# sungnyun/dualhyp

Measured on AMD Instinct MI355X. Metric: corrected utterances/sec (TinyLlama-1.1B, 5+5 hyps, 512->64 tok), higher is better.
Workload: dtype bf16; 1 GPU; DualHyp inference, TinyLlama-1.1B bf16 + LoRA r16 (q,k,v,proj), batch 32/GPU synthetic 5+5-hyp prompts, 512-token prompt -> 64 generated tokens, greedy; batch_per_gpu=32, parallelism=replicas x1, batches_in_flight_per_gpu=64, schedule=merged, decode_rows_per_launch=2048

## Files before the change

### dualhyp_amd/_lib.py

```python
from __future__ import annotations

import ctypes as C
from pathlib import Path

_HERE = Path(__file__).resolve().parent
import os as _os
LIB_PATH = Path(_os.environ["DUALHYP_HIP_LIB"]) if _os.environ.get("DUALHYP_HIP_LIB") else _HERE / "lib" / "libdualhyp_hip.so"

P = C.c_void_p
I = C.c_int
I64 = C.c_int64
U64 = C.c_uint64
F = C.c_float


class LayerWeights(C.Structure):
    _fields_ = [(n, P) for n in ("norm_1", "norm_2", "attn_w", "attn_lora_a", "attn_lora_b", "proj_w",
                                 "proj_lora_a", "proj_lora_b", "fc_1", "fc_2", "mlp_proj",
                                 "attn_ws", "proj_ws", "fc_1_ws", "fc_2_ws", "mlp_proj_ws")]


class ModelDesc(C.Structure):
    _fields_ = [("n_layer", C.c_int32), ("n_head", C.c_int32), ("n_groups", C.c_int32), ("head_size", C.c_int32),
                ("n_embd", C.c_int32), ("intermediate", C.c_int32), ("vocab", C.c_int32), ("block_size", C.c_int32),
                ("norm_eps", F), ("lora_scale", F), ("wte", P), ("wte_rows", C.c_int32), ("ln_f", P),
                ("rope_cos", P), ("rope_sin", P), ("lm_head", P), ("adapter_scale", P), ("adapter_bias", P),
                ("h_layers", C.POINTER(LayerWeights)), ("lm_head_ws", P)]


SIGNATURES = {
    "dh_abi_version": (I, []),
    "dh_set_tuning": (I, [I, I]),
    "dh_last_error": (C.c_char_p, []),
    "dh_device_info": (I, [C.c_char_p, I, C.POINTER(I), C.POINTER(I64)]),
    "dh_embed_bf16": (I, [P, P, P, I, I, I, P]),
    "dh_rmsnorm_bf16": (I, [P, P, P, P, P, I, I, F, P, P]),
    "dh_qkv_rope_cache_bf16": (I, [P, P, P, P, P, P, P, P, P, P, I, I, I, I, I, P]),
    "dh_linear_bf16": (I, [P, P, P, I, I, I, I, P, P, I, P, F, I, I, P, P, P, P]),
    "dh_linear_qkv_rope_cache_bf16": (I, [P, P, I, I, P, I, P, F, P, P, P, P, P, P, P, I, I, I, I, P]),
    "dh_linear_lora_bf16": (I, [P, P, P, I, I, I, P, P, F, I, I, P, P, P]),
    "dh_linear_qkv_lora_rope_cache_bf16": (I, [P, P, I, I, P, P, F, P, P, P, P, P, P, P, I, I, I, I, P, P]),
    "dh_linear_partial_bf16": (I, [P, P, P, P, I, I, I, I, I, P]),
    "dh_linear_chain_bf16": (I, [P, P, P, P, I, I, I, I, I, P]),
    "dh_linear_partial_pairs_bf16": (I, [P, P, P, P, I, I, I, I, I, P]),
    "dh_finish_norm_bf16": (I, [P, I, I, I, I, I, P, F, P, P, P, P, F, P, P]),
    "dh_attn_decode_fused_bf16": (I, [P, I, I, I, I, I, P, F, I, I, P, P, P, P, P, P, P, I, I, I, I, P]),
    "dh_attn_prefill_bf16": (I, [P, P, P, P, P, P, P, P, P, I, I, I, I, I, I, P]),
    "dh_dropout_bf16": (I, [P, P, P, I64, F, C.c_uint64, C.c_uint32, P, P]),
    "dh_swiglu_fwd_bf16": (I, [P, P, P, I64, P]),
    "dh_linear_swiglu_train_bf16": (I, [P, P, P, P, P, P, I, I, I, P]),
    "dh_linear_mul_bf16": (I, [P, P, P, I, I, I, P, P]),
    "dh_swiglu_bwd_bf16": (I, [P, P, P, P, I, I, P]),
    "dh_rmsnorm_bwd_bf16": (I, [P, P, P, P, P, I, I, F, P]),
    "dh_qkv_rope_bwd_bf16": (I, [P, P, P, P, P, P, P, I, I, I, I, P]),
    "dh_tn_accum_f32": (I, [P, I, P, I, P, I, I, I, I, F, I, P, P]),
    "dh_tn_accum_work_bytes": (I64, [I, I, I]),
    "dh_tn_accum_seg_f32": (I, [P, I, P, I, P, I, I, I, I, I, F, I, P, P]),
    "dh_rowdot_f32": (I, [P, P, P, I64, I, P]),
    "dh_transpose_pad_bf16": (I, [P, P, P, P, P, I, I, I, I, P]),
    "dh_transpose_frag_bf16": (I, [P, P, P, I, I, I, P]),
    "dh_attn_bwd_transposes": (I, [I, I, I, I]),
    "dh_attn_bwd_bf16": (I, [P, P, P, P, P, P, P, P, P, P, P, P, P, P, P, I, I, I, I, I, I, P]),
    "dh_attn_decode_work_bytes": (I64, [I, I, I, I]),
    "dh_attn_decode_bf16": (I, [P, P, P, P, P, P, P, I, I, I, I, I, P]),
    "dh_sample_bf16": (I, [P, I, P, I, P, P, I, F, I, I64, U64, I, P]),
    "dh_sample_rows_bf16": (I, [P, I, P, I, P, P, P, P, I, I, I, F, I, I64, U64, P]),
    "dh_quant_rows_fp8": (I, [P, P, P, I, I, P]),
    "dh_rmsnorm_quant_fp8": (I, [P, P, P, P, P, I, I, F, P, P]),
    "dh_linear_fp8": (I, [P, P, P, P, P, I, I, I, I, P, P, P, P, P, P]),
    "dh_linear_fp8_ex": (I, [P, P, P, P, P, I, I, I, I, P, P, P, P, P, I, P]),
    "dh_linear_fp8_f32": (I, [P, P, P, P, P, I, I, I, P]),
    "dh_engine_create": (I, [C.POINTER(ModelDesc), I, I, I, C.POINTER(P)]),
    "dh_engine_destroy": (None, [P]),
    "dh_engine_device_bytes": (I64, [P]),
    "dh_im2col3_bf16": (I, [P, P, I, I, I, I, I, P]),
    "dh_pool_head_bf16": (I, [P, P, P, P, I, I, I, I, P]),
    "dh_pool_head_bwd_bf16": (I, [P, P, P, P, P, I, I, I, I, P]),
    "dh_col2im3_bf16": (I, [P, P, P, P, I, I, I, I, P]),
    "dh_cross_entropy_fwd": (I, [P, I, P, P, P, I, I, P]),
    "dh_cross_entropy_bwd": (I, [P, I, P, P, P, P, I, I, P]),
    "dh_engine_forward": (I, [P, P, C.POINTER(C.c_int32), C.POINTER(C.c_int32), I, P, P, P]),
    "dh_engine_forward_at": (I, [P, P, C.POINTER(C.c_int32), C.POINTER(C.c_int32), I, I, P, P, P]),
    "dh_engine_forward_slots": (I, [P, P, C.POINTER(C.c_int32), C.POINTER(C.c_int32), C.POINTER(C.c_int32), I, I, P, P, P]),
    "dh_engine_set_cpu_rsqrt_emulation": (I, [P, I, I]),
    "dh_engine_decode": (I, [P, P, I, P, P, I, I, F, I, I64, U64, I, P]),
    "dh_engine_decode_rows": (I, [P, P, I, P, P, P, I, I, P, P, I, I, F, I, I64, U64, P]),
    "dh_engine_read": (I, [P, I, I, P, I64, P]),
    "dh_engine_set_timing": (I, [P, I]),
    "dh_engine_get_timing": (I, [P, I, C.POINTER(C.c_double), C.POINTER(I64)]),
}

_lib = None


class DualHypHipError(RuntimeError):
    pass


def load() -> C.CDLL:
    global _lib
    if _lib is not None:
        return _lib
    if not LIB_PATH.exists():
        raise DualHypHipError(
            f"{LIB_PATH} not found: the HIP library is not built. Run `python __graft_entry__.py` "
            "(hipcc --offload-arch=gfx950). There is no CPU fallback for the product path.")
    lib = C.CDLL(str(LIB_PATH))
    for name, (res, args) in SIGNATURES.items():
        try:
            fn = getattr(lib, name)
        except AttributeError as e:
            raise DualHypHipError(f"libdualhyp_hip.so does not export {name}") from e
        fn.restype = res
        fn.argtypes = args
    if lib.dh_abi_version() != 6:
        raise DualHypHipError("libdualhyp_hip.so ABI version mismatch")
    _lib = lib
    return lib


def check(rc: int) -> None:
    if rc != 0:
        msg = load().dh_last_error().decode(errors="replace")
        raise DualHypHipError(msg or f"libdualhyp_hip call failed with code {rc}")
```

### dualhyp_amd/csrc/decode_fused.hip

```cpp
#include "common.h"

namespace {

constexpr int DCOLS = 16;
constexpr int MAXP = 16;

template <int HS, int PMAX, int NW>
__global__ __launch_bounds__(NW * 64, NW == 16 ? 1 : (NW == 6 ? 3 : (HS == 64 ? 4 : 2))) void attn_decode_fused_kernel(
    const float* __restrict__ qkv32, int n_part, int pairs, int n_seq, int ldq, int qkv_dim,
    const bf16_t* __restrict__ lora_b, float lora_scale, int split0, int split1,
    const bf16_t* __restrict__ cos, const bf16_t* __restrict__ sin, const int32_t* __restrict__ seq_slot,
    const int32_t* __restrict__ kv_len, bf16_t* __restrict__ k_cache, bf16_t* __restrict__ vT_cache,
    bf16_t* __restrict__ y, int n_head, int n_groups, int s_max, float scale) {
    constexpr int KS = HS / 16, DT = HS / 32, HALF = HS / 2;
    extern __shared__ __attribute__((aligned(16))) char smem[];
    const int pair = blockIdx.x, seq = pair / n_groups, g = pair % n_groups;
    const int q_per_kv = n_head / n_groups;
    const int tid = threadIdx.x, lane = tid & 63, wave = tid >> 6;
    const int lr = lane & 31, lh = lane >> 5;
    const int slot = seq_slot[seq];
    const int len = kv_len[seq], pos = len - 1;
    bf16_t* sQ = reinterpret_cast<bf16_t*>(smem);
    float* sKn = reinterpret_cast<float*>(smem + 16 * HS * 2);
    float* sVn = sKn + HS;
    float* sXa = sVn + HS;
    float* sSn = sXa + 48;
    float* sPm = sSn + 16;
    float* sPl = sPm + NW * DCOLS;
    float* sPo = sPl + NW * DCOLS;
    constexpr int NT_ = NW * 64;

    constexpr int PF = NW == 6 ? 2 : 1;
    struct VF { bf16x8 v; };
    struct Tile { bf16x8 kf[KS]; VF vf[DT][2]; };
    Tile tl[PF];
    const bf16_t* kbase = k_cache + ((size_t)slot * n_groups + g) * s_max * HS;
    const bf16_t* vbase = vT_cache + ((size_t)slot * n_groups + g) * HS * s_max;
    const int n_tiles = (pos + 31) / 32;
    auto load_tile = [&](Tile& T, int t) {
#pragma unroll
        for (int ks = 0; ks < KS; ++ks)
            T.kf[ks] = __builtin_nontemporal_load(reinterpret_cast<const bf16x8*>(kbase + kfrag_blk<HS>(t, ks) + lane * 8));
#pragma unroll
        for (int dt = 0; dt < DT; ++dt)
#pragma unroll
            for (int s2 = 0; s2 < 2; ++s2)
                T.vf[dt][s2].v = __builtin_nontemporal_load(reinterpret_cast<const bf16x8*>(vbase + vfrag_blk<HS>(t, dt, s2) + lane * 8));
    };
#pragma unroll
    for (int p = 0; p < PF; ++p)
        if (wave + NW * p < n_tiles) load_tile(tl[p], wave + NW * p);

    const float* row0 = qkv32 + (size_t)seq * ldq;
    const size_t pstride = (size_t)n_seq * ldq;
    auto psum = [&](int c) {
        float v[PMAX];
#pragma unroll
        for (int p = 0; p < PMAX; ++p) v[p] = p < n_part ? row0[p * pstride + c] : 0.f;
        float s = 0.f;
        if (pairs) {
#pragma unroll
            for (int p = 0; p < PMAX; p += 2) s += v[p] + v[p + 1];
        } else {
#pragma unroll
            for (int p = 0; p < PMAX; ++p) s += v[p];
        }
        return s;
    };
    if (lora_b != nullptr && tid < 48) sXa[tid] = rbf(psum(qkv_dim + tid));
    for (int i = tid; i < 16 * HS; i += NT_) sQ[i] = 0;
    __syncthreads();

    auto finish = [&](int c) -> float {
        float o = rbf(psum(c));
        if (lora_b != nullptr) {
            const int seg = (c >= split0) + (c >= split1);
            const uint4* b4 = reinterpret_cast<const uint4*>(lora_b + (size_t)c * 16);
            float l = 0.f;
#pragma unroll
            for (int h = 0; h < 2; ++h) {
                const uint4 bv = b4[h];
                const bf16_t* bp = reinterpret_cast<const bf16_t*>(&bv);
#pragma unroll
                for (int e = 0; e < 8; ++e) l = fmaf(sXa[seg * 16 + h * 8 + e], bf2f(bp[e]), l);
            }
            o = rbf(o + rbf(rbf(l) * lora_scale));
        }
        return o;
    };
    const int gbase = g * (q_per_kv + 2) * HS;
    bf16_t* kdst = k_cache + ((size_t)slot * n_groups + g) * s_max * HS;
    bf16_t* vdst = vT_cache + ((size_t)slot * n_groups + g) * HS * s_max;
    const int n_rope = (q_per_kv + 1) * HALF;
    for (int it = tid; it < n_rope + HS; it += NT_) {
        if (it < n_rope) {
            const int j = it / HALF, i = it % HALF;
            const float x1 = finish(gbase + j * HS + i), x2 = finish(gbase + j * HS + HALF + i);
            const bf16_t* cp = cos + (size_t)pos * HS;
            const bf16_t* sp = sin + (size_t)pos * HS;
            const bf16_t o1 = f2bf(rbf(x1 * bf2f(cp[i])) + rbf(-x2 * bf2f(sp[i])));
            const bf16_t o2 = f2bf(rbf(x2 * bf2f(cp[HALF + i])) + rbf(x1 * bf2f(sp[HALF + i])));
            if (j < q_per_kv) {
                sQ[j * HS + i] = o1;
                sQ[j * HS + HALF + i] = o2;
            } else {
                sKn[i] = bf2f(o1);
                sKn[HALF + i] = bf2f(o2);
                kdst[kfrag_off<HS>(pos, i)] = o1;
                kdst[kfrag_off<HS>(pos, HALF + i)] = o2;
            }
        } else {
            const int e = it - n_rope;
            const bf16_t v = f2bf(finish(gbase + (q_per_kv + 1) * HS + e));
            sVn[e] = bf2f(v);
            vdst[vfrag_off<HS>(pos, e)] = v;
        }
    }
    __syncthreads();

    for (int h = wave; h < q_per_kv; h += NW) {
        float p = 0.f;
        for (int e = lane; e < HS; e += 64) p += bf2f(sQ[h * HS + e]) * sKn[e];
        p = wave_sum(p);
        if (lane == 0) sSn[h] = p * scale;
    }

    bf16x8 qf[KS];
#pragma unroll
    for (int ks = 0; ks < KS; ++ks) qf[ks] = *reinterpret_cast<const bf16x8*>(sQ + (lr & 15) * HS + ks * 16 + lh * 8);
    if (lr >= 16) {
#pragma unroll
        for (int ks = 0; ks < KS; ++ks) qf[ks] = bf16x8{0, 0, 0, 0, 0, 0, 0, 0};
    }
    f32x16 o[DT];
#pragma unroll
    for (int dt = 0; dt < DT; ++dt)
#pragma unroll
        for (int r = 0; r < 16; ++r) o[dt][r] = 0.f;
    float m_run = -INFINITY, l_run = 0.f;
    auto compute_tile = [&](const Tile& T, int t) {
        const int key0 = t * 32;
        f32x16 st;
#pragma unroll
        for (int r = 0; r < 16; ++r) st[r] = 0.f;
#pragma unroll
        for (int ks = 0; ks < KS; ++ks) st = __builtin_amdgcn_mfma_f32_32x32x16_bf16(T.kf[ks], qf[ks], st, 0, 0, 0);
        float m_t = -INFINITY;
#pragma unroll
        for (int r = 0; r < 16; ++r) {
            const int key_abs = key0 + (r & 3) + 8 * (r >> 2) + 4 * lh;
            float sc = st[r] * scale;
            sc = key_abs < pos ? sc : -INFINITY;
            st[r] = sc;
            m_t = fmaxf(m_t, sc);
        }
        m_t = fmaxf(m_t, __shfl_xor(m_t, 32, 64));
        const float m_new = fmaxf(m_run, m_t);
        const float alpha = __expf(m_run - m_new);
        m_run = m_new;
        float psm = 0.f;
#pragma unroll
        for (int r = 0; r < 16; ++r) {
            const float p = __expf(st[r] - m_new);
            st[r] = p;
            psm += p;
        }
        l_run = l_run * alpha + psm;
#pragma unroll
        for (int s2 = 0; s2 < 2; ++s2) {
            union { bf16x8 v; uint32_t u[4]; } pf;
#pragma unroll
            for (int j = 0; j < 4; ++j) pf.u[j] = pack2bf(st[8 * s2 + 2 * j], st[8 * s2 + 2 * j + 1]);
#pragma unroll
            for (int dt = 0; dt < DT; ++dt) {
                if (s2 == 0) {
#pragma unroll
                    for (int r = 0; r < 16; ++r) o[dt][r] *= alpha;
                }
                o[dt] = __builtin_amdgcn_mfma_f32_32x32x16_bf16(T.vf[dt][s2].v, pf.v, o[dt], 0, 0, 0);
            }
        }
    };
    for (int base = wave; base < n_tiles; base += NW * PF) {
#pragma unroll
        for (int p = 0; p < PF; ++p) {
            if (base + NW * p < n_tiles) compute_tile(tl[p], base + NW * p);
            if (base + NW * (PF + p) < n_tiles) load_tile(tl[p], base + NW * (PF + p));
        }
    }
    const float l_tot = l_run + __shfl_xor(l_run, 32, 64);
    if (lr < q_per_kv) {
        if (lh == 0) {
            sPm[wave * DCOLS + lr] = m_run;
            sPl[wave * DCOLS + lr] = l_tot;
        }
#pragma unroll
        for (int dt = 0; dt < DT; ++dt)
#pragma unroll
            for (int r = 0; r < 16; ++r) {
                const int d = dt * 32 + (r & 3) + 8 * (r >> 2) + 4 * lh;
                sPo[(wave * HS + d) * DCOLS + lr] = o[dt][r];
            }
    }
    __syncthreads();
    for (int it = tid; it < q_per_kv * HS; it += NT_) {
        const int h = it / HS, d = it % HS;
        const float sn = sSn[h];
        float M = sn;
#pragma unroll
        for (int w = 0; w < NW; ++w) M = fmaxf(M, sPm[w * DCOLS + h]);
        const float pn = __expf(sn - M);
        float L = pn, O = rbf(pn) * sVn[d];
#pragma unroll
        for (int w = 0; w < NW; ++w) {
            const float mw = sPm[w * DCOLS + h];
            const float f = (mw == -INFINITY) ? 0.f : __expf(mw - M);
            L += sPl[w * DCOLS + h] * f;
            O += sPo[(w * HS + d) * DCOLS + h] * f;
        }
        y[(size_t)seq * n_head * HS + (g * q_per_kv + h) * HS + d] = f2bf(O / L);
    }
}

#ifndef DH_ATTN_WAVES64
#define DH_ATTN_WAVES64 8
#endif
template <int HS>
constexpr int attn_fused_waves() { return HS == 64 ? DH_ATTN_WAVES64 : 8; }
template <int HS>
constexpr size_t attn_fused_lds() {
    constexpr int NW = attn_fused_waves<HS>();
    return 16 * HS * 2 + (HS + HS + 48 + 16 + NW * DCOLS + NW * DCOLS + NW * HS * DCOLS) * sizeof(float);
}

template <int MAXC>
__global__ __launch_bounds__(256) void finish_norm_kernel(const float* __restrict__ h32, int n_part, int pairs, int rows, int ldh,
                                                          const bf16_t* __restrict__ lora_b, float lora_scale,
                                                          const bf16_t* __restrict__ x_resid,
                                                          const bf16_t* __restrict__ w_norm, bf16_t* __restrict__ x_out,
                                                          bf16_t* __restrict__ xn_out, int d, float eps,
                                                          const uint8_t* __restrict__ row_tail) {
    __shared__ float sXa[16];
    __shared__ float sRed[4];
    const int row = blockIdx.x, tid = threadIdx.x, lane = tid & 63, wave = tid >> 6;
    const float* hrow = h32 + (size_t)row * ldh;
    const size_t pstride = (size_t)rows * ldh;
    if (lora_b != nullptr && tid < 16) {
        float pv[MAXP];
#pragma unroll
        for (int p = 0; p < MAXP; ++p) pv[p] = p < n_part ? hrow[p * pstride + d + tid] : 0.f;
        float s = 0.f;
        if (pairs) {
#pragma unroll
            for (int p = 0; p < MAXP; p += 2) s += pv[p] + pv[p + 1];
        } else {
#pragma unroll
            for (int p = 0; p < MAXP; ++p) s += pv[p];
        }
        sXa[tid] = rbf(s);
    }
    __syncthreads();
    float v[MAXC][8];
    float ss = 0.f;
#pragma unroll
    for (int i = 0; i < MAXC; ++i) {
        const int c0 = (tid + i * 256) * 8;
        if (c0 < d) {
            float acc[8];
#pragma unroll
            for (int e = 0; e < 8; ++e) acc[e] = 0.f;
            for (int p0 = 0; p0 < n_part; p0 += 4) {
                float4 a0[4], a1[4];
#pragma unroll
                for (int q = 0; q < 4; ++q) {
                    const int p = p0 + q < n_part ? p0 + q : p0;
                    a0[q] = *reinterpret_cast<const float4*>(hrow + p * pstride + c0);
                    a1[q] = *reinterpret_cast<const float4*>(hrow + p * pstride + c0 + 4);
                }
                if (pairs) {
#pragma unroll
                    for (int q = 0; q < 4; q += 2) {
                        if (p0 + q < n_part) {
                            const bool two = p0 + q + 1 < n_part;
                            const float4 b0 = two ? a0[q + 1] : float4{0.f, 0.f, 0.f, 0.f}, b1 = two ? a1[q + 1] : float4{0.f, 0.f, 0.f, 0.f};
                            acc[0] += a0[q].x + b0.x; acc[1] += a0[q].y + b0.y; acc[2] += a0[q].z + b0.z; acc[3] += a0[q].w + b0.w;
                            acc[4] += a1[q].x + b1.x; acc[5] += a1[q].y + b1.y; acc[6] += a1[q].z + b1.z; acc[7] += a1[q].w + b1.w;
                        }
                    }
                } else {
#pragma unroll
                for (int q = 0; q < 4; ++q) {
                    if (p0 + q < n_part) {
                        acc[0] += a0[q].x; acc[1] += a0[q].y; acc[2] += a0[q].z; acc[3] += a0[q].w;
                        acc[4] += a1[q].x; acc[5] += a1[q].y; acc[6] += a1[q].z; acc[7] += a1[q].w;
                    }
                }
                }
            }
            const uint4 xr = *reinterpret_cast<const uint4*>(x_resid + (size_t)row * d + c0);
            const bf16_t* xp = reinterpret_cast<const bf16_t*>(&xr);
            uint4 xo;
            bf16_t* xop = reinterpret_cast<bf16_t*>(&xo);
#pragma unroll
            for (int e = 0; e < 8; ++e) {
                float o = rbf(acc[e]);
                if (lora_b != nullptr) {
                    const uint4* b4 = reinterpret_cast<const uint4*>(lora_b + (size_t)(c0 + e) * 16);
                    float l = 0.f;
#pragma unroll
                    for (int h = 0; h < 2; ++h) {
                        const uint4 bv = b4[h];
                        const bf16_t* bp = reinterpret_cast<const bf16_t*>(&bv);
#pragma unroll
                        for (int k = 0; k < 8; ++k) l = fmaf(sXa[h * 8 + k], bf2f(bp[k]), l);
                    }
                    o = rbf(o + rbf(rbf(l) * lora_scale));
                }
                xop[e] = f2bf(bf2f(xp[e]) + o);
                v[i][e] = bf2f(xop[e]);
                ss += rbf(v[i][e] * v[i][e]);
            }
            *reinterpret_cast<uint4*>(x_out + (size_t)row * d + c0) = xo;
        }
    }
    ss = wave_sum(ss);
    if (lane == 0) sRed[wave] = ss;
    __syncthreads();
    ss = sRed[0] + sRed[1] + sRed[2] + sRed[3];
    const float ms = rbf(ss / (float)d);
    const float t = rbf(ms + eps);
    const bool tail = row_tail != nullptr && row_tail[row] != 0;
    const float r = tail ? rbf(1.0f / rbf(sqrtf(t))) : rbf(1.0f / sqrtf(t));
#pragma unroll
    for (int i = 0; i < MAXC; ++i) {
        const int c0 = (tid + i * 256) * 8;
        if (c0 < d) {
            const uint4 wu = *reinterpret_cast<const uint4*>(w_norm + c0);
            const bf16_t* wp = reinterpret_cast<const bf16_t*>(&wu);
            uint4 o;
            bf16_t* op = reinterpret_cast<bf16_t*>(&o);
#pragma unroll
            for (int e = 0; e < 8; ++e) op[e] = f2bf(bf2f(wp[e]) * rbf(v[i][e] * r));
            *reinterpret_cast<uint4*>(xn_out + (size_t)row * d + c0) = o;
        }
    }
}

}

extern "C" int dh_attn_decode_fused_bf16(const float* qkv32, int n_part, int pairs, int n_seq, int qkv_dim, int n_ext,
                                         const dh_bf16* lora_b, float lora_scale, int split0, int split1,
                                         const dh_bf16* cos, const dh_bf16* sin, const int32_t* seq_slot,
                                         const int32_t* kv_len, dh_bf16* k_cache, dh_bf16* vT_cache, dh_bf16* y,
                                         int n_head, int n_groups, int hs, int s_max, void* stream) {
    DH_CHECK(qkv32 && cos && sin && seq_slot && kv_len && k_cache && vT_cache && y, "dh_attn_decode_fused_bf16: null argument");
    DH_CHECK(n_groups > 0 && n_head % n_groups == 0 && n_head / n_groups <= DCOLS, "dh_attn_decode_fused_bf16: bad head counts");
    DH_CHECK(hs == 64 || hs == 96 || hs == 128, "dh_attn_decode_fused_bf16: head_size %d unsupported", hs);
    DH_CHECK(s_max % 64 == 0 && n_part >= 1 && n_part <= MAXP, "dh_attn_decode_fused_bf16: bad s_max / n_part");
    DH_CHECK(qkv_dim == (n_head + 2 * n_groups) * hs, "dh_attn_decode_fused_bf16: qkv_dim mismatch");
    DH_CHECK(lora_b == nullptr || n_ext >= 48, "dh_attn_decode_fused_bf16: LoRA needs the 48 x·A^T columns");
    if (n_seq <= 0) return 0;
    const float scale = 1.0f / sqrtf((float)hs);
    hipStream_t s = (hipStream_t)stream;
    dim3 grid(n_seq * n_groups);
#define ATT_LAUNCH(HSV, PM)                                                                                           \
    hipLaunchKernelGGL((attn_decode_fused_kernel<HSV, PM, attn_fused_waves<HSV>()>), grid, dim3(64 * attn_fused_waves<HSV>()), attn_fused_lds<HSV>(), s, qkv32, n_part, pairs, n_seq,  \
                       qkv_dim + n_ext, qkv_dim, lora_b, lora_scale, split0, split1, cos, sin, seq_slot, kv_len, k_cache,  \
                       vT_cache, y, n_head, n_groups, s_max, scale)
    if (hs == 64) {
        DH_MAX_LDS_ONCE((attn_decode_fused_kernel<64, 2, attn_fused_waves<64>()>), attn_fused_lds<64>());
        DH_MAX_LDS_ONCE((attn_decode_fused_kernel<64, 8, attn_fused_waves<64>()>), attn_fused_lds<64>());
        DH_MAX_LDS_ONCE((attn_decode_fused_kernel<64, 16, attn_fused_waves<64>()>), attn_fused_lds<64>());
        if (n_part <= 2) ATT_LAUNCH(64, 2);
        else if (n_part <= 8) ATT_LAUNCH(64, 8);
        else ATT_LAUNCH(64, 16);
    } else if (hs == 96) {
        DH_MAX_LDS_ONCE((attn_decode_fused_kernel<96, 2, 8>), attn_fused_lds<96>());
        DH_MAX_LDS_ONCE((attn_decode_fused_kernel<96, 8, 8>), attn_fused_lds<96>());
        DH_MAX_LDS_ONCE((attn_decode_fused_kernel<96, 16, 8>), attn_fused_lds<96>());
        if (n_part <= 2) ATT_LAUNCH(96, 2);
        else if (n_part <= 8) ATT_LAUNCH(96, 8);
        else ATT_LAUNCH(96, 16);
    } else {
        DH_MAX_LDS_ONCE((attn_decode_fused_kernel<128, 2, 8>), attn_fused_lds<128>());
        DH_MAX_LDS_ONCE((attn_decode_fused_kernel<128, 8, 8>), attn_fused_lds<128>());
        DH_MAX_LDS_ONCE((attn_decode_fused_kernel<128, 16, 8>), attn_fused_lds<128>());
        if (n_part <= 2) ATT_LAUNCH(128, 2);
        else if (n_part <= 8) ATT_LAUNCH(128, 8);
        else ATT_LAUNCH(128, 16);
    }
#undef ATT_LAUNCH
    DH_LAUNCH_CHECK();
    return 0;
}

extern "C" int dh_finish_norm_bf16(const float* h32, int n_part, int pairs, int rows, int d, int n_ext, const dh_bf16* lora_b,
                                   float lora_scale, const dh_bf16* x_resid, const dh_bf16* w_norm, dh_bf16* x_out,
                                   dh_bf16* xn_out, float eps, const uint8_t* row_tail, void* stream) {
    DH_CHECK(h32 && x_resid && w_norm && x_out && xn_out, "dh_finish_norm_bf16: null argument");
    DH_CHECK(d % 8 == 0 && d <= 8192 && n_part >= 1 && n_part <= MAXP, "dh_finish_norm_bf16: unsupported d=%d", d);
    DH_CHECK(lora_b == nullptr || n_ext >= 16, "dh_finish_norm_bf16: LoRA needs the 16 x·A^T columns");
    DH_CHECK((d + n_ext) % 4 == 0, "dh_finish_norm_bf16: row stride must be a multiple of 4 floats");
    if (rows <= 0) return 0;
    hipStream_t s = (hipStream_t)stream;
    dim3 grid(rows), block(256);
    const int ldh = d + n_ext;
#define LAUNCH(MAXC) hipLaunchKernelGGL((finish_norm_kernel<MAXC>), grid, block, 0, s, h32, n_part, pairs, rows, ldh, lora_b, \
                                        lora_scale, x_resid, w_norm, x_out, xn_out, d, eps, row_tail)
    if (d <= 2048) { LAUNCH(1); }
    else if (d <= 4096) { LAUNCH(2); }
    else { LAUNCH(4); }
#undef LAUNCH
    DH_LAUNCH_CHECK();
    return 0;
}
```

### dualhyp_amd/csrc/engine.hip

```cpp
#include <vector>

#include "common.h"
#include "gemm.h"

int dh_sample_impl(const dh_bf16* logits, int vocab, int64_t* tokens, int tok_ld, int32_t* length, int32_t* done,
                   int n_seq, float temperature, int top_k, int64_t eos_id, uint64_t seed, int step,
                   const int32_t* step_dev, void* stream);
int dh_sample_rows_impl(const dh_bf16* logits, int vocab, int64_t* tokens, int tok_ld, int32_t* length, int32_t* done,
                        const int32_t* limit, const int32_t* row_seq, int n_rows, int n_seq, int max_new, float temperature,
                        int top_k, int64_t eos_id, uint64_t seed, void* stream);

namespace {

struct Timing {
    bool on = false;
    std::vector<std::pair<hipEvent_t, hipEvent_t>> ev[4];
    std::vector<hipEvent_t> pool;
};

}

constexpr int MAX_DECODE_ROWS = 2048;
int g_decode_tiled_rows = 0;
int g_short_kps = 8;
int g_fuse_qkv_rope = 1;
int g_prune_last_layer = 1;

struct dh_engine {
    dh_model_desc d;
    std::vector<dh_layer_weights> layers;
    int max_batch = 0, s_max = 0, max_tokens = 0;
    int qkv_dim = 0, kv_dim = 0;
    bf16_t *kc = nullptr, *vtc = nullptr;
    bf16_t *x = nullptr, *xn = nullptr, *qkv = nullptr, *qrot = nullptr, *att = nullptr, *xa = nullptr,
           *act = nullptr, *xlast = nullptr, *logits = nullptr;
    int32_t *tok_slot = nullptr, *tok_pos = nullptr, *seq_meta = nullptr;
    int32_t *last_row = nullptr, *step_dev = nullptr;
    int32_t* slot_list = nullptr;
    int32_t* last_meta = nullptr;
    bf16_t *att_last = nullptr, *xn_last = nullptr, *act_last = nullptr;
    uint8_t *row_tail = nullptr, *last_tail = nullptr, *ones = nullptr;
    int rsqrt_vec = 0, rsqrt_whole = 0;
    int64_t* dec_ids = nullptr;
    void* dec_work = nullptr;
    float* part32 = nullptr;
    bool fp8 = false;
    uint8_t* xq = nullptr;
    float* xscale = nullptr;
    int32_t* h_stage = nullptr;
    size_t cache_layer_elems = 0;
    int64_t dev_bytes = 0;
    hipStream_t gstream = nullptr;
    hipEvent_t ev_in = nullptr, ev_out = nullptr, ev_stage = nullptr;
    struct GKey {
        int64_t* tokens; int tok_ld; int32_t *length, *done; int n_seq, top_k; float temp; int64_t eos; uint64_t seed; int rsqrt_vec, tiled_rows;
        const int32_t *limit, *row_seq, *row_slot; int n_all, max_new;
        bool operator==(const GKey& k) const {
            return tokens == k.tokens && tok_ld == k.tok_ld && length == k.length && done == k.done && n_seq == k.n_seq &&
                   top_k == k.top_k && temp == k.temp && eos == k.eos && seed == k.seed && rsqrt_vec == k.rsqrt_vec &&
                   tiled_rows == k.tiled_rows && limit == k.limit && row_seq == k.row_seq && row_slot == k.row_slot &&
                   n_all == k.n_all && max_new == k.max_new;
        }
    };
    struct GEntry { GKey key; hipGraphExec_t exec; uint64_t used; };
    std::vector<GEntry> graphs;
    uint64_t graph_clock = 0;
    int last_ntok = 0;
    int slot_base = 0;
    const int32_t* seq_slot = nullptr;
    bool capturing = false;
    bool phase_decode = false;
    bool decode_tiled = false;
    Timing tm;
};

namespace {

template <typename T>
int dmalloc(dh_engine* e, T** p, size_t n) {
    DH_HIP(hipMalloc((void**)p, n * sizeof(T)));
    e->dev_bytes += (int64_t)(n * sizeof(T));
    return 0;
}

__global__ void decode_prep_kernel(const int64_t* __restrict__ tokens, int tok_ld, const int32_t* __restrict__ length,
                                   int64_t* __restrict__ ids, int32_t* __restrict__ tok_slot,
                                   int32_t* __restrict__ tok_pos, int32_t* __restrict__ kv_len, int32_t* step_dev,
                                   int n_seq, int s_max) {
    const int i = blockIdx.x * blockDim.x + threadIdx.x;
    if (i < n_seq) {
        int n = length[i];
        n = n < 1 ? 1 : (n > s_max ? s_max : n);
        ids[i] = tokens[(size_t)i * tok_ld + n - 1];
        tok_slot[i] = i;
        tok_pos[i] = n - 1;
        kv_len[i] = n;
    }
    if (i == 0) *step_dev += 1;
}

__global__ void decode_prep_rows_kernel(const int64_t* __restrict__ tokens, int tok_ld, const int32_t* __restrict__ length,
                                        const int32_t* __restrict__ row_seq, const int32_t* __restrict__ row_slot,
                                        int64_t* __restrict__ ids, int32_t* __restrict__ tok_slot, int32_t* __restrict__ tok_pos,
                                        int32_t* __restrict__ kv_len, int n_rows, int n_all, int max_batch, int s_max) {
    const int r = blockIdx.x * blockDim.x + threadIdx.x;
    if (r < n_rows) {
        int u = row_seq[r], slot = row_slot[r];
        u = u < 0 || u >= n_all ? 0 : u;
        slot = slot < 0 || slot >= max_batch ? 0 : slot;
        int n = length[u];
        const int cap = s_max < tok_ld ? s_max : tok_ld;
        n = n < 1 ? 1 : (n > cap ? cap : n);
        ids[r] = tokens[(size_t)u * tok_ld + n - 1];
        tok_slot[r] = slot;
        tok_pos[r] = n - 1;
        kv_len[r] = n;
    }
}

__global__ void set_i32_kernel(int32_t* p, int32_t v) { *p = v; }
__global__ void iota_i32_kernel(int32_t* p, int n) {
    const int i = blockIdx.x * blockDim.x + threadIdx.x;
    if (i < n) p[i] = i;
}

__global__ void gather_rows_kernel(const bf16_t* __restrict__ src, const int32_t* __restrict__ rows,
                                   bf16_t* __restrict__ dst, int n, int d) {
    const int wave = (blockIdx.x * blockDim.x + threadIdx.x) >> 6, lane = threadIdx.x & 63;
    if (wave >= n) return;
    const uint4* s = reinterpret_cast<const uint4*>(src + (size_t)rows[wave] * d);
    uint4* t = reinterpret_cast<uint4*>(dst + (size_t)wave * d);
    for (int c = lane; c < d / 8; c += 64) t[c] = s[c];
}

struct TimeScope {
    dh_engine* e; int which; hipStream_t s; hipEvent_t a = nullptr, b = nullptr;
    TimeScope(dh_engine* e_, int w, hipStream_t s_) : e(e_), which(w), s(s_) {
        if (!e->tm.on || e->capturing) return;
        hipEventCreate(&a); hipEventCreate(&b);
        hipEventRecord(a, s);
    }
    ~TimeScope() {
        if (!a) return;
        hipEventRecord(b, s);
        e->tm.ev[which].push_back({a, b});
    }
};

int linear(dh_engine* e, const bf16_t* x, const bf16_t* w, bf16_t* y, int M, int N, int K, int epi,
           const bf16_t* w2, const bf16_t* xa, int xa_ld, const bf16_t* lb, int s0, int s1, const bf16_t* va,
           const bf16_t* vb, const bf16_t* resid, hipStream_t s, bool timed) {
    const int kernel = e->phase_decode && !e->decode_tiled ? 2 : 1;
    if (timed) {
        TimeScope t(e, e->phase_decode ? 1 : 0, s);
        return dh_linear_impl(x, w, y, M, N, K, epi, w2, xa, xa_ld, lb, e->d.lora_scale, s0, s1, va, vb, resid, kernel, s);
    }
    return dh_linear_impl(x, w, y, M, N, K, epi, w2, xa, xa_ld, lb, e->d.lora_scale, s0, s1, va, vb, resid, kernel, s);
}

int run_layers(dh_engine* e, const int64_t* ids, int n_tok, int n_seq, int max_q_len, bool decode,
               const uint8_t* tail_flags, hipStream_t s, bool prune_last = false) {
    const uint8_t* rt = e->rsqrt_vec > 0 ? tail_flags : nullptr;
    e->phase_decode = decode;
    const dh_model_desc& D = e->d;
    const int d = D.n_embd, I = D.intermediate, hs = D.head_size, H = D.n_head, G = D.n_groups;
    const int32_t* seq_slot = e->seq_slot;
    int32_t* q_start = e->seq_meta + e->max_batch;
    int32_t* q_len = e->seq_meta + 2 * e->max_batch;
    int32_t* kv_pos0 = e->seq_meta + 3 * e->max_batch;
    int rc;
    if ((rc = dh_embed_bf16(ids, D.wte, e->x, n_tok, d, D.wte_rows, s))) return rc;
    for (int l = 0; l < D.n_layer; ++l) {
        const dh_layer_weights& W = e->layers[l];
        bf16_t* kc = e->kc + (size_t)l * e->cache_layer_elems;
        bf16_t* vtc = e->vtc + (size_t)l * e->cache_layer_elems;
        if ((rc = dh_rmsnorm_bf16(e->x, nullptr, W.norm_1, e->xn, nullptr, n_tok, d, D.norm_eps, rt, s))) return rc;
        const bool fuse_qkv = !decode && g_fuse_qkv_rope && hs != 96 && dh_linear_is_big(n_tok, e->qkv_dim, DH_EPI_LORA);
        if (W.attn_lora_a && !fuse_qkv)
            if ((rc = linear(e, e->xn, W.attn_lora_a, e->xa, n_tok, 48, d, DH_EPI_PLAIN, nullptr, nullptr, 0, nullptr, 0, 0,
                             nullptr, nullptr, nullptr, s, false))) return rc;
        if (fuse_qkv) {
            TimeScope t(e, 0, s);
            if (W.attn_lora_a) {
                if ((rc = dh_linear_qkv_lora_rope_cache_bf16(e->xn, W.attn_w, n_tok, d, W.attn_lora_a, W.attn_lora_b, D.lora_scale,
                                                             D.rope_cos, D.rope_sin, e->tok_slot, e->tok_pos, e->qrot, kc, vtc, H, G,
                                                             hs, e->s_max, e->xa, s))) return rc;
            } else if ((rc = dh_linear_qkv_rope_cache_bf16(e->xn, W.attn_w, n_tok, d, nullptr, 48, nullptr, D.lora_scale, D.rope_cos,
                                                           D.rope_sin, e->tok_slot, e->tok_pos, e->qrot, kc, vtc, H, G, hs,
                                                           e->s_max, s))) return rc;
        } else {
        if (W.attn_lora_a) {
            if ((rc = linear(e, e->xn, W.attn_w, e->qkv, n_tok, e->qkv_dim, d, DH_EPI_LORA, nullptr, e->xa, 48,
                             W.attn_lora_b, d, d + e->kv_dim, nullptr, nullptr, nullptr, s, true))) return rc;
        } else {
            if ((rc = linear(e, e->xn, W.attn_w, e->qkv, n_tok, e->qkv_dim, d, DH_EPI_PLAIN, nullptr, nullptr, 0, nullptr,
                             0, 0, nullptr, nullptr, nullptr, s, true))) return rc;
        }
        if ((rc = dh_qkv_rope_cache_bf16(e->qkv, D.rope_cos, D.rope_sin, e->tok_slot, e->tok_pos, e->qrot, kc, vtc, nullptr,
                                         nullptr, n_tok, H, G, hs, e->s_max, s))) return rc;
        }
        if (prune_last && l == D.n_layer - 1) {
            const uint8_t* rtl = e->rsqrt_vec > 0 ? e->last_tail : nullptr;
            {
                TimeScope t(e, 2, s);
                if ((rc = dh_attn_prefill_bf16(e->qrot, kc, vtc, seq_slot, e->last_row, e->last_meta, e->last_meta + e->max_batch,
                                               e->att, nullptr, n_seq, 1, H, G, hs, e->s_max, s))) return rc;
            }
            hipLaunchKernelGGL(gather_rows_kernel, dim3(cdiv(n_seq, 4)), dim3(256), 0, s, e->att, e->last_row, e->att_last, n_seq, d);
            hipLaunchKernelGGL(gather_rows_kernel, dim3(cdiv(n_seq, 4)), dim3(256), 0, s, e->x, e->last_row, e->xlast, n_seq, d);
            DH_LAUNCH_CHECK();
            if (W.proj_lora_a) {
                if ((rc = dh_linear_lora_impl(e->att_last, W.proj_w, e->xlast, n_seq, d, d, W.proj_lora_a, W.proj_lora_b, D.lora_scale, d, d,
                                              e->xlast, e->xa, 1, s))) return rc;
            } else {
                if ((rc = linear(e, e->att_last, W.proj_w, e->xlast, n_seq, d, d, DH_EPI_PLAIN, nullptr, nullptr, 0, nullptr, 0, 0,
                                 nullptr, nullptr, e->xlast, s, false))) return rc;
            }
            if ((rc = dh_rmsnorm_bf16(e->xlast, nullptr, W.norm_2, e->xn_last, nullptr, n_seq, d, D.norm_eps, rtl, s))) return rc;
            if ((rc = linear(e, e->xn_last, W.fc_1, e->act_last, n_seq, I, d, DH_EPI_SWIGLU, W.fc_2, nullptr, 0, nullptr, 0, 0, nullptr,
                             nullptr, nullptr, s, false))) return rc;
            if ((rc = linear(e, e->act_last, W.mlp_proj, e->xlast, n_seq, d, I, DH_EPI_PLAIN, nullptr, nullptr, 0, nullptr, 0, 0, nullptr,
                             nullptr, e->xlast, s, false))) return rc;
            break;
        }
        if (decode) {
            TimeScope t(e, 3, s);
            if ((rc = dh_attn_decode_bf16(e->qrot, kc, vtc, seq_slot, kv_pos0, e->att, e->dec_work, n_seq, H, G, hs,
                                          e->s_max, s))) return rc;
        } else {
            TimeScope t(e, 2, s);
            if ((rc = dh_attn_prefill_bf16(e->qrot, kc, vtc, seq_slot, q_start, q_len, kv_pos0, e->att, nullptr, n_seq,
                                           max_q_len, H, G, hs, e->s_max, s))) return rc;
        }
        if (W.proj_lora_a) {
            TimeScope t(e, e->phase_decode ? 1 : 0, s);
            if ((rc = dh_linear_lora_impl(e->att, W.proj_w, e->x, n_tok, d, d, W.proj_lora_a, W.proj_lora_b, D.lora_scale, d, d, e->x,
                                          e->xa, e->phase_decode && !e->decode_tiled ? 2 : 1, s))) return rc;
        } else {
            if ((rc = linear(e, e->att, W.proj_w, e->x, n_tok, d, d, DH_EPI_PLAIN, nullptr, nullptr, 0, nullptr, 0, 0,
                             nullptr, nullptr, e->x, s, true))) return rc;
        }
        if ((rc = dh_rmsnorm_bf16(e->x, nullptr, W.norm_2, e->xn, nullptr, n_tok, d, D.norm_eps, rt, s))) return rc;
        if ((rc = linear(e, e->xn, W.fc_1, e->act, n_tok, I, d, DH_EPI_SWIGLU, W.fc_2, nullptr, 0, nullptr, 0, 0, nullptr,
                         nullptr, nullptr, s, true))) return rc;
        if ((rc = linear(e, e->act, W.mlp_proj, e->x, n_tok, d, I, DH_EPI_PLAIN, nullptr, nullptr, 0, nullptr, 0, 0, nullptr,
                         nullptr, e->x, s, true))) return rc;
    }
    return 0;
}

inline int fp8_kernel(bool decode, int rows) { return decode && rows <= 128 ? 2 : 1; }

int run_layers_fp8(dh_engine* e, const int64_t* ids, int n_tok, int n_seq, int max_q_len, bool decode,
                   const uint8_t* tail_flags, hipStream_t s, bool prune_last = false) {
    const uint8_t* rt = e->rsqrt_vec > 0 ? tail_flags : nullptr;
    e->phase_decode = decode;
    const dh_model_desc& D = e->d;
    const int d = D.n_embd, I = D.intermediate, hs = D.head_size, H = D.n_head, G = D.n_groups;
    const int32_t* seq_slot = e->seq_slot;
    int32_t* q_start = e->seq_meta + e->max_batch;
    int32_t* q_len = e->seq_meta + 2 * e->max_batch;
    int32_t* kv_pos0 = e->seq_meta + 3 * e->max_batch;
    int rc;
    auto lin = [&](const bf16_t* w, const float* ws, bf16_t* y, int N, int K, int epi, const bf16_t* w2, const float* w2s,
                   const bf16_t* res) {
        return dh_linear_fp8_ex(e->xq, e->xscale, reinterpret_cast<const uint8_t*>(w), ws, y, n_tok, N, K, epi,
                                reinterpret_cast<const uint8_t*>(w2), w2s, nullptr, nullptr, res, fp8_kernel(decode, n_tok), s);
    };
    if ((rc = dh_embed_bf16(ids, D.wte, e->x, n_tok, d, D.wte_rows, s))) return rc;
    for (int l = 0; l < D.n_layer; ++l) {
        const dh_layer_weights& W = e->layers[l];
        bf16_t* kc = e->kc + (size_t)l * e->cache_layer_elems;
        bf16_t* vtc = e->vtc + (size_t)l * e->cache_layer_elems;
        if ((rc = dh_rmsnorm_quant_fp8(e->x, W.norm_1, nullptr, e->xq, e->xscale, n_tok, d, D.norm_eps, rt, s))) return rc;
        if (decode && n_tok <= 128) {
            {
                TimeScope t(e, 1, s);
                if ((rc = dh_linear_fp8_f32(e->xq, e->xscale, reinterpret_cast<const uint8_t*>(W.attn_w), W.attn_ws, e->part32,
                                            n_tok, e->qkv_dim, d, s))) return rc;
            }
            TimeScope t(e, 3, s);
            if ((rc = dh_attn_decode_fused_bf16(e->part32, 1, 0, n_seq, e->qkv_dim, 0, nullptr, 0.f, e->qkv_dim, e->qkv_dim,
                                                D.rope_cos, D.rope_sin, seq_slot, kv_pos0, kc, vtc, e->att, H, G, hs,
                                                e->s_max, s))) return rc;
        } else {
        {
            TimeScope t(e, decode ? 1 : 0, s);
            if ((rc = lin(W.attn_w, W.attn_ws, e->qkv, e->qkv_dim, d, DH_EPI_PLAIN, nullptr, nullptr, nullptr))) return rc;
        }
        if ((rc = dh_qkv_rope_cache_bf16(e->qkv, D.rope_cos, D.rope_sin, e->tok_slot, e->tok_pos, e->qrot, kc, vtc, nullptr,
                                         nullptr, n_tok, H, G, hs, e->s_max, s))) return rc;
        if (prune_last && l == D.n_layer - 1) {
            const uint8_t* rtl = e->rsqrt_vec > 0 ? e->last_tail : nullptr;
            auto lin_last = [&](const bf16_t* w, const float* ws, bf16_t* y, int N, int K, int epi, const bf16_t* w2, const float* w2s,
                                const bf16_t* res) {
                return dh_linear_fp8_ex(e->xq, e->xscale, reinterpret_cast<const uint8_t*>(w), ws, y, n_seq, N, K, epi,
                                        reinterpret_cast<const uint8_t*>(w2), w2s, nullptr, nullptr, res, fp8_kernel(false, n_seq), s);
            };
            {
                TimeScope t(e, 2, s);
                if ((rc = dh_attn_prefill_bf16(e->qrot, kc, vtc, seq_slot, e->last_row, e->last_meta, e->last_meta + e->max_batch,
                                               e->att, nullptr, n_seq, 1, H, G, hs, e->s_max, s))) return rc;
            }
            hipLaunchKernelGGL(gather_rows_kernel, dim3(cdiv(n_seq, 4)), dim3(256), 0, s, e->att, e->last_row, e->att_last, n_seq, d);
            hipLaunchKernelGGL(gather_rows_kernel, dim3(cdiv(n_seq, 4)), dim3(256), 0, s, e->x, e->last_row, e->xlast, n_seq, d);
            DH_LAUNCH_CHECK();
            if ((rc = dh_quant_rows_fp8(e->att_last, e->xq, e->xscale, n_seq, d, s))) return rc;
            if ((rc = lin_last(W.proj_w, W.proj_ws, e->xlast, d, d, DH_EPI_PLAIN, nullptr, nullptr, e->xlast))) return rc;
            if ((rc = dh_rmsnorm_quant_fp8(e->xlast, W.norm_2, nullptr, e->xq, e->xscale, n_seq, d, D.norm_eps, rtl, s))) return rc;
            if ((rc = lin_last(W.fc_1, W.fc_1_ws, e->act_last, I, d, DH_EPI_SWIGLU, W.fc_2, W.fc_2_ws, nullptr))) return rc;
            if ((rc = dh_quant_rows_fp8(e->act_last, e->xq, e->xscale, n_seq, I, s))) return rc;
            if ((rc = lin_last(W.mlp_proj, W.mlp_proj_ws, e->xlast, d, I, DH_EPI_PLAIN, nullptr, nullptr, e->xlast))) return rc;
            break;
        }
        if (decode) {
            TimeScope t(e, 3, s);
            if ((rc = dh_attn_decode_bf16(e->qrot, kc, vtc, seq_slot, kv_pos0, e->att, e->dec_work, n_seq, H, G, hs,
                                          e->s_max, s))) return rc;
        } else {
            TimeScope t(e, 2, s);
            if ((rc = dh_attn_prefill_bf16(e->qrot, kc, vtc, seq_slot, q_start, q_len, kv_pos0, e->att, nullptr, n_seq,
                                           max_q_len, H, G, hs, e->s_max, s))) return rc;
        }
        }
        if ((rc = dh_quant_rows_fp8(e->att, e->xq, e->xscale, n_tok, d, s))) return rc;
        {
            TimeScope t(e, decode ? 1 : 0, s);
            if ((rc = lin(W.proj_w, W.proj_ws, e->x, d, d, DH_EPI_PLAIN, nullptr, nullptr, e->x))) return rc;
        }
        if ((rc = dh_rmsnorm_quant_fp8(e->x, W.norm_2, nullptr, e->xq, e->xscale, n_tok, d, D.norm_eps, rt, s))) return rc;
        {
            TimeScope t(e, decode ? 1 : 0, s);
            if ((rc = lin(W.fc_1, W.fc_1_ws, e->act, I, d, DH_EPI_SWIGLU, W.fc_2, W.fc_2_ws, nullptr))) return rc;
        }
        if ((rc = dh_quant_rows_fp8(e->act, e->xq, e->xscale, n_tok, I, s))) return rc;
        {
            TimeScope t(e, decode ? 1 : 0, s);
            if ((rc = lin(W.mlp_proj, W.mlp_proj_ws, e->x, d, I, DH_EPI_PLAIN, nullptr, nullptr, e->x))) return rc;
        }
    }
    return 0;
}

int head_fp8(dh_engine* e, const bf16_t* xrows, int rows, bf16_t* logits, const uint8_t* rt, hipStream_t s) {
    const dh_model_desc& D = e->d;
    int rc;
    if ((rc = dh_rmsnorm_quant_fp8(xrows, D.ln_f, e->xn, e->xq, e->xscale, rows, D.n_embd, D.norm_eps,
                                   e->rsqrt_vec > 0 ? rt : nullptr, s))) return rc;
    TimeScope t(e, e->phase_decode ? 1 : 0, s);
    return dh_linear_fp8_ex(e->xq, e->xscale, reinterpret_cast<const uint8_t*>(D.lm_head), D.lm_head_ws, logits, rows, D.vocab,
                            D.n_embd, DH_EPI_ADAPTER, nullptr, nullptr, D.adapter_scale, D.adapter_bias, nullptr,
                            fp8_kernel(e->phase_decode, rows), s);
}

int pick_ksplit(int tiles, int nks) {
    (void)tiles;
    if (nks <= 128) return g_short_kps == 16 && nks % 16 == 0 ? nks / 16 : (nks + 7) / 8;
    if (nks <= 256) return (nks + 15) / 16;
    int ks = 1;
    while (ks < 4 && nks / (16 * ks) >= 2) ks *= 2;
    return ks;
}

int run_layers_decode(dh_engine* e, const int64_t* ids, int n_seq, const uint8_t* tail_flags, hipStream_t s) {
    const dh_model_desc& D = e->d;
    const int d = D.n_embd, I = D.intermediate, hs = D.head_size, H = D.n_head, G = D.n_groups;
    const uint8_t* rt = e->rsqrt_vec > 0 ? tail_flags : nullptr;
    const int32_t* seq_slot = e->seq_slot;
    const int32_t* kv_len = e->seq_meta + 3 * e->max_batch;
    e->phase_decode = true;
    int rc;
    if ((rc = dh_embed_bf16(ids, D.wte, e->x, n_seq, d, D.wte_rows, s))) return rc;
    if ((rc = dh_rmsnorm_bf16(e->x, nullptr, e->layers[0].norm_1, e->xn, nullptr, n_seq, d, D.norm_eps, rt, s))) return rc;
    for (int l = 0; l < D.n_layer; ++l) {
        const dh_layer_weights& W = e->layers[l];
        bf16_t* kc = e->kc + (size_t)l * e->cache_layer_elems;
        bf16_t* vtc = e->vtc + (size_t)l * e->cache_layer_elems;
        auto partial = [&](const bf16_t* xin, const bf16_t* w, const bf16_t* wext, int N, int ext, int K, int ks, int& np, int& pairs) {
            if (dh_chain_ok(n_seq, N, ext, K, ks)) { np = 1; pairs = 0; return dh_linear_chain_bf16(xin, w, wext, e->part32, n_seq, N, ext, K, ks, s); }
            if (dh_pairs_ok(n_seq, N, ext, K, ks)) { np = (ks + 1) / 2; pairs = 0; return dh_linear_partial_pairs_bf16(xin, w, wext, e->part32, n_seq, N, ext, K, ks, s); }
            np = ks; pairs = 1;
            return dh_linear_partial_bf16(xin, w, wext, e->part32, n_seq, N, ext, K, ks, s);
        };
        int np, pairs;
        const int ext1 = W.attn_lora_a ? 48 : 0;
        if ((rc = partial(e->xn, W.attn_w, W.attn_lora_a, e->qkv_dim, ext1, d, pick_ksplit((e->qkv_dim + ext1) / 16, d / 32), np, pairs))) return rc;
        if ((rc = dh_attn_decode_fused_bf16(e->part32, np, pairs, n_seq, e->qkv_dim, ext1, W.attn_lora_b, D.lora_scale, d,
                                            d + e->kv_dim, D.rope_cos, D.rope_sin, seq_slot, kv_len, kc, vtc, e->att, H, G,
                                            hs, e->s_max, s))) return rc;
        const int ext2 = W.proj_lora_a ? 16 : 0;
        if ((rc = partial(e->att, W.proj_w, W.proj_lora_a, d, ext2, d, pick_ksplit((d + ext2) / 16, d / 32), np, pairs))) return rc;
        if ((rc = dh_finish_norm_bf16(e->part32, np, pairs, n_seq, d, ext2, W.proj_lora_b, D.lora_scale, e->x, W.norm_2, e->x,
                                      e->xn, D.norm_eps, rt, s))) return rc;
        if ((rc = linear(e, e->xn, W.fc_1, e->act, n_seq, I, d, DH_EPI_SWIGLU, W.fc_2, nullptr, 0, nullptr, 0, 0, nullptr,
                         nullptr, nullptr, s, false))) return rc;
        if ((rc = partial(e->act, W.mlp_proj, nullptr, d, 0, I, pick_ksplit(d / 16, I / 32), np, pairs))) return rc;
        const bf16_t* next_norm = l + 1 < D.n_layer ? e->layers[l + 1].norm_1 : D.ln_f;
        if ((rc = dh_finish_norm_bf16(e->part32, np, pairs, n_seq, d, 0, nullptr, 0.f, e->x, next_norm, e->x, e->xn,
                                      D.norm_eps, rt, s))) return rc;
    }
    return 0;
}

int head_normed(dh_engine* e, int rows, bf16_t* logits, hipStream_t s) {
    const dh_model_desc& D = e->d;
    return linear(e, e->xn, D.lm_head, logits, rows, D.vocab, D.n_embd, DH_EPI_ADAPTER, nullptr, nullptr, 0, nullptr, 0, 0,
                  D.adapter_scale, D.adapter_bias, nullptr, s, true);
}

int head(dh_engine* e, const bf16_t* xrows, int rows, bf16_t* logits, const uint8_t* rt, hipStream_t s) {
    const dh_model_desc& D = e->d;
    int rc;
    if ((rc = dh_rmsnorm_bf16(xrows, nullptr, D.ln_f, e->xn, nullptr, rows, D.n_embd, D.norm_eps,
                              e->rsqrt_vec > 0 ? rt : nullptr, s))) return rc;
    return linear(e, e->xn, D.lm_head, logits, rows, D.vocab, D.n_embd, DH_EPI_ADAPTER, nullptr, nullptr, 0, nullptr, 0, 0,
                  D.adapter_scale, D.adapter_bias, nullptr, s, true);
}

int decode_step(dh_engine* e, int64_t* tokens, int tok_ld, int32_t* length, int32_t* done, int n_seq, float temperature,
                int top_k, int64_t eos_id, uint64_t seed, hipStream_t s);
int engine_init(dh_engine* e, const dh_model_desc* desc, int max_batch, int s_max, int max_tokens);

}

extern "C" int dh_engine_create(const dh_model_desc* desc, int max_batch, int s_max, int max_tokens, dh_engine** out) {
    DH_CHECK(desc && out, "dh_engine_create: null argument");
    DH_CHECK(desc->head_size == 64 || desc->head_size == 96 || desc->head_size == 128, "dh_engine_create: head_size %d unsupported", desc->head_size);
    DH_CHECK(desc->n_head % desc->n_groups == 0, "dh_engine_create: n_head %% n_groups != 0");
    DH_CHECK(desc->n_embd == desc->n_head * desc->head_size, "dh_engine_create: n_embd != n_head*head_size");
    DH_CHECK(desc->n_embd % 64 == 0 && desc->intermediate % 64 == 0 && desc->vocab % 8 == 0, "dh_engine_create: dims must be multiples of 64");
    DH_CHECK(s_max > 0 && s_max % 64 == 0 && s_max <= (desc->block_size + 63) / 64 * 64, "dh_engine_create: s_max=%d must be a multiple of 64 and <= block_size rounded up", s_max);
    DH_CHECK(max_batch > 0 && max_tokens >= max_batch, "dh_engine_create: bad batch/token capacity");
    DH_CHECK(desc->rope_cos && desc->rope_sin && desc->wte && desc->ln_f && desc->lm_head && desc->h_layers, "dh_engine_create: null weight pointer");
    dh_engine* e = new dh_engine();
    const int rc = engine_init(e, desc, max_batch, s_max, max_tokens);
    if (rc) { dh_engine_destroy(e); return rc; }
    *out = e;
    return 0;
}

namespace {

int engine_init(dh_engine* e, const dh_model_desc* desc, int max_batch, int s_max, int max_tokens) {
    e->d = *desc;
    e->layers.assign(desc->h_layers, desc->h_layers + desc->n_layer);
    e->d.h_layers = nullptr;
    e->max_batch = max_batch; e->s_max = s_max; e->max_tokens = max_tokens;
    const int d = desc->n_embd, hs = desc->head_size, G = desc->n_groups, H = desc->n_head;
    e->kv_dim = G * hs;
    e->qkv_dim = (H + 2 * G) * hs;
    e->fp8 = e->layers[0].attn_ws != nullptr;
    if (e->fp8) {
        for (const auto& L : e->layers)
            DH_CHECK(L.attn_ws && L.proj_ws && L.fc_1_ws && L.fc_2_ws && L.mlp_proj_ws && !L.attn_lora_a && !L.proj_lora_a,
                     "dh_engine_create: fp8 mode needs every channel-scale pointer and merged LoRA (no lora_a/lora_b)");
        DH_CHECK(desc->lm_head_ws != nullptr, "dh_engine_create: fp8 mode needs lm_head_ws");
        DH_CHECK(d % 128 == 0 && desc->intermediate % 128 == 0, "dh_engine_create: fp8 mode needs n_embd and intermediate %% 128 == 0");
    }
    e->cache_layer_elems = (size_t)max_batch * G * s_max * hs;
    {
        size_t free_b = 0, total_b = 0;
        DH_HIP(hipMemGetInfo(&free_b, &total_b));
        const size_t kv_bytes = 2 * e->cache_layer_elems * desc->n_layer * sizeof(bf16_t);
        DH_CHECK(kv_bytes <= free_b,
                 "dh_engine_create: the KV cache of %d sequences x %d positions x %d layers needs %.1f GiB and %.1f GiB are free: "
                 "lower the decode batch (--decode_batch)", max_batch, s_max, desc->n_layer, kv_bytes / 1073741824.0,
                 free_b / 1073741824.0);
    }
    const size_t T = max_tokens;
    int rc = 0;
    rc |= dmalloc(e, &e->kc, e->cache_layer_elems * desc->n_layer);
    rc |= dmalloc(e, &e->vtc, e->cache_layer_elems * desc->n_layer);
    rc |= dmalloc(e, &e->x, T * d);
    rc |= dmalloc(e, &e->xn, T * d);
    rc |= dmalloc(e, &e->qkv, T * e->qkv_dim);
    rc |= dmalloc(e, &e->qrot, T * d);
    rc |= dmalloc(e, &e->att, T * d);
    rc |= dmalloc(e, &e->xa, T * 48);
    rc |= dmalloc(e, &e->act, T * desc->intermediate);
    rc |= dmalloc(e, &e->xlast, (size_t)max_batch * d);
    rc |= dmalloc(e, &e->logits, (size_t)max_batch * desc->vocab);
    rc |= dmalloc(e, &e->tok_slot, T);
    rc |= dmalloc(e, &e->tok_pos, T);
    rc |= dmalloc(e, &e->seq_meta, (size_t)4 * max_batch);
    rc |= dmalloc(e, &e->last_row, (size_t)max_batch);
    rc |= dmalloc(e, &e->last_meta, (size_t)2 * max_batch);
    rc |= dmalloc(e, &e->att_last, (size_t)max_batch * d);
    rc |= dmalloc(e, &e->xn_last, (size_t)max_batch * d);
    rc |= dmalloc(e, &e->act_last, (size_t)max_batch * desc->intermediate);
    rc |= dmalloc(e, &e->step_dev, 1);
    rc |= dmalloc(e, &e->slot_list, (size_t)max_batch);
    rc |= dmalloc(e, &e->dec_ids, (size_t)max_batch);
    rc |= dmalloc(e, &e->part32, (size_t)16 * (max_batch < 32 ? 32 : (max_batch < MAX_DECODE_ROWS ? max_batch : MAX_DECODE_ROWS)) * (e->qkv_dim + 48));
    if (e->fp8) {
        rc |= dmalloc(e, &e->xq, T * (size_t)(desc->intermediate > d ? desc->intermediate : d));
        rc |= dmalloc(e, &e->xscale, T);
    }
    rc |= dmalloc(e, &e->row_tail, T);
    rc |= dmalloc(e, &e->last_tail, (size_t)max_batch);
    rc |= dmalloc(e, &e->ones, (size_t)max_batch);
    const int64_t wb = dh_attn_decode_work_bytes(max_batch, H, hs, s_max);
    if (!rc) { hipError_t he = hipMalloc(&e->dec_work, wb); if (he != hipSuccess) rc = 2; e->dev_bytes += wb; }
    if (rc) { dh_set_error("dh_engine_create: device allocation failed (%s)", dh_last_error()); return 2; }
    DH_HIP(hipMemset(e->kc, 0, e->cache_layer_elems * desc->n_layer * sizeof(bf16_t)));
    DH_HIP(hipMemset(e->vtc, 0, e->cache_layer_elems * desc->n_layer * sizeof(bf16_t)));
    DH_HIP(hipMemset(e->step_dev, 0, sizeof(int32_t)));
    DH_HIP(hipMemset(e->ones, 1, (size_t)max_batch));
    DH_HIP(hipHostMalloc((void**)&e->h_stage, (3 * T + 8 * (size_t)max_batch) * sizeof(int32_t)));
    DH_HIP(hipStreamCreateWithFlags(&e->gstream, hipStreamNonBlocking));
    DH_HIP(hipEventCreateWithFlags(&e->ev_in, hipEventDisableTiming));
    DH_HIP(hipEventCreateWithFlags(&e->ev_out, hipEventDisableTiming));
    DH_HIP(hipEventCreateWithFlags(&e->ev_stage, hipEventDisableTiming));
    hipLaunchKernelGGL(iota_i32_kernel, dim3(cdiv(max_batch, 64)), dim3(64), 0, 0, e->seq_meta, max_batch);
    DH_HIP(hipDeviceSynchronize());
    return 0;
}

}

extern "C" void dh_engine_destroy(dh_engine* e) {
    if (!e) return;
    for (auto& g : e->graphs) hipGraphExecDestroy(g.exec);
    void* ptrs[] = {e->kc, e->vtc, e->x, e->xn, e->qkv, e->qrot, e->att, e->xa, e->act, e->xlast, e->logits,
                    e->tok_slot, e->tok_pos, e->seq_meta, e->last_row, e->last_meta, e->att_last, e->xn_last, e->act_last, e->step_dev, e->slot_list, e->dec_ids, e->dec_work,
                    e->row_tail, e->last_tail, e->ones, e->part32, e->xq, e->xscale};
    for (void* p : ptrs)
        if (p) hipFree(p);
    if (e->h_stage) hipHostFree(e->h_stage);
    if (e->gstream) hipStreamDestroy(e->gstream);
    if (e->ev_in) hipEventDestroy(e->ev_in);
    if (e->ev_out) hipEventDestroy(e->ev_out);
    if (e->ev_stage) hipEventDestroy(e->ev_stage);
    for (auto& v : e->tm.ev)
        for (auto& p : v) { hipEventDestroy(p.first); hipEventDestroy(p.second); }
    delete e;
}

extern "C" int64_t dh_engine_device_bytes(const dh_engine* e) { return e ? e->dev_bytes : 0; }
extern "C" int dh_engine_read(dh_engine* e, int what, int layer, void* dst, int64_t n_bytes, void* stream) {
    DH_CHECK(e && dst && n_bytes >= 0, "dh_engine_read: bad argument");
    const void* src = nullptr;
    int64_t avail = 0;
    const int64_t cache_bytes = (int64_t)e->cache_layer_elems * sizeof(bf16_t);
    switch (what) {
        case 0: src = e->xn; avail = (int64_t)e->max_tokens * e->d.n_embd * 2; break;
        case 3: src = e->x; avail = (int64_t)e->max_tokens * e->d.n_embd * 2; break;
        case 1: case 2:
            DH_CHECK(layer >= 0 && layer < e->d.n_layer, "dh_engine_read: layer %d out of range", layer);
            src = (what == 1 ? e->kc : e->vtc) + (size_t)layer * e->cache_layer_elems;
            avail = cache_bytes;
            break;
        default: DH_CHECK(false, "dh_engine_read: unknown selector %d", what);
    }
    DH_CHECK(n_bytes <= avail, "dh_engine_read: %lld bytes requested, %lld available", (long long)n_bytes, (long long)avail);
    DH_HIP(hipMemcpyAsync(dst, src, n_bytes, hipMemcpyDeviceToDevice, (hipStream_t)stream));
    return 0;
}

extern "C" int dh_engine_forward(dh_engine* e, const int64_t* ids, const int32_t* h_seq_len, const int32_t* h_pos0,
                                 int n_seq, dh_bf16* logits_all, dh_bf16* logits_last, void* stream) {
    return dh_engine_forward_at(e, ids, h_seq_len, h_pos0, n_seq, 0, logits_all, logits_last, stream);
}

namespace {
int forward_impl(dh_engine* e, const int64_t* ids, const int32_t* h_seq_len, const int32_t* h_pos0, const int32_t* h_slots,
                 int n_seq, int slot_base, bool prompt_phase, dh_bf16* logits_all, dh_bf16* logits_last, void* stream);
}

extern "C" int dh_engine_forward_at(dh_engine* e, const int64_t* ids, const int32_t* h_seq_len, const int32_t* h_pos0,
                                    int n_seq, int slot_base, dh_bf16* logits_all, dh_bf16* logits_last, void* stream) {
    DH_CHECK(e && ids && h_seq_len && h_pos0, "dh_engine_forward: null argument");
    DH_CHECK(n_seq > 0 && slot_base >= 0 && slot_base + n_seq <= e->max_batch,
             "dh_engine_forward: sequences [%d, %d) exceed max_batch=%d", slot_base, slot_base + n_seq, e->max_batch);
    return forward_impl(e, ids, h_seq_len, h_pos0, nullptr, n_seq, slot_base, false, logits_all, logits_last, stream);
}

extern "C" int dh_engine_forward_slots(dh_engine* e, const int64_t* ids, const int32_t* h_seq_len, const int32_t* h_pos0,
                                       const int32_t* h_slot, int n_seq, int prompt_phase, dh_bf16* logits_all, dh_bf16* logits_last,
                                       void* stream) {
    DH_CHECK(e && ids && h_seq_len && h_pos0 && h_slot, "dh_engine_forward_slots: null argument");
    DH_CHECK(n_seq > 0 && n_seq <= e->max_batch, "dh_engine_forward_slots: n_seq=%d exceeds max_batch=%d", n_seq, e->max_batch);
    std::vector<char> taken(e->max_batch, 0);
    for (int i = 0; i < n_seq; ++i) {
        DH_CHECK(h_slot[i] >= 0 && h_slot[i] < e->max_batch, "dh_engine_forward_slots: sequence %d names slot %d of %d", i, h_slot[i], e->max_batch);
        DH_CHECK(!taken[h_slot[i]], "dh_engine_forward_slots: slot %d is named twice", h_slot[i]);
        taken[h_slot[i]] = 1;
    }
    return forward_impl(e, ids, h_seq_len, h_pos0, h_slot, n_seq, 0, prompt_phase != 0, logits_all, logits_last, stream);
}

namespace {

int forward_impl(dh_engine* e, const int64_t* ids, const int32_t* h_seq_len, const int32_t* h_pos0, const int32_t* h_slots,
                 int n_seq, int slot_base, bool prompt_phase, dh_bf16* logits_all, dh_bf16* logits_last, void* stream) {
    e->slot_base = slot_base;
    e->seq_slot = h_slots ? e->slot_list : e->seq_meta + slot_base;
    hipStream_t s = (hipStream_t)stream;
    int n_tok = 0, max_q = 0;
    for (int i = 0; i < n_seq; ++i) {
        DH_CHECK(h_seq_len[i] > 0 && h_pos0[i] >= 0, "dh_engine_forward: sequence %d has length %d at position %d", i, h_seq_len[i], h_pos0[i]);
        DH_CHECK(h_pos0[i] + h_seq_len[i] <= e->s_max, "Cannot forward sequence %d: %d tokens at position %d exceed the KV cache length %d",
                 i, h_seq_len[i], h_pos0[i], e->s_max);
        n_tok += h_seq_len[i];
        max_q = h_seq_len[i] > max_q ? h_seq_len[i] : max_q;
    }
    const bool step = max_q == 1 && !prompt_phase;
    DH_CHECK(n_tok <= e->max_tokens, "dh_engine_forward: %d tokens exceed the workspace capacity %d", n_tok, e->max_tokens);
    const int B = e->max_batch;
    int32_t* hs_ = e->h_stage;
    DH_HIP(hipEventSynchronize(e->ev_stage));
    int32_t *h_slot = hs_, *h_pos = hs_ + e->max_tokens, *h_meta = hs_ + 2 * (size_t)e->max_tokens;
    int t = 0;
    for (int i = 0; i < n_seq; ++i) {
        const int slot = h_slots ? h_slots[i] : slot_base + i;
        h_meta[i] = slot;
        h_meta[B + i] = t;
        h_meta[2 * B + i] = h_seq_len[i];
        h_meta[3 * B + i] = step ? h_pos0[i] + 1 : h_pos0[i];
        for (int j = 0; j < h_seq_len[i]; ++j, ++t) { h_slot[t] = slot; h_pos[t] = h_pos0[i] + j; }
        h_meta[4 * B + i] = t - 1;
    }
    uint8_t* h_tail = reinterpret_cast<uint8_t*>(hs_ + 2 * (size_t)e->max_tokens + 5 * (size_t)B);
    uint8_t* h_last_tail = h_tail + e->max_tokens;
    if (e->rsqrt_vec > 0) {
        const int V = e->rsqrt_vec;
        int r = 0;
        for (int i = 0; i < n_seq; ++i) {
            for (int j = 0; j < h_seq_len[i]; ++j, ++r)
                h_tail[r] = e->rsqrt_whole ? (r >= n_tok / V * V) : (j >= h_seq_len[i] / V * V);
            h_last_tail[i] = h_tail[r - 1];
        }
        DH_HIP(hipMemcpyAsync(e->row_tail, h_tail, n_tok, hipMemcpyHostToDevice, s));
        DH_HIP(hipMemcpyAsync(e->last_tail, h_last_tail, n_seq, hipMemcpyHostToDevice, s));
    }
    DH_HIP(hipMemcpyAsync(e->tok_slot, h_slot, n_tok * sizeof(int32_t), hipMemcpyHostToDevice, s));
    DH_HIP(hipMemcpyAsync(e->tok_pos, h_pos, n_tok * sizeof(int32_t), hipMemcpyHostToDevice, s));
    if (h_slots) DH_HIP(hipMemcpyAsync(e->slot_list, h_meta, n_seq * sizeof(int32_t), hipMemcpyHostToDevice, s));
    DH_HIP(hipMemcpyAsync(e->seq_meta + B, h_meta + B, 3 * B * sizeof(int32_t), hipMemcpyHostToDevice, s));
    DH_HIP(hipMemcpyAsync(e->last_row, h_meta + 4 * B, B * sizeof(int32_t), hipMemcpyHostToDevice, s));
    const bool prune_last = g_prune_last_layer && max_q > 1 && logits_all == nullptr && logits_last != nullptr;
    if (prune_last) {
        int32_t* h_lm = hs_ + 3 * (size_t)e->max_tokens + 6 * (size_t)B;
        for (int i = 0; i < n_seq; ++i) { h_lm[i] = 1; h_lm[B + i] = h_pos0[i] + h_seq_len[i] - 1; }
        DH_HIP(hipMemcpyAsync(e->last_meta, h_lm, 2 * B * sizeof(int32_t), hipMemcpyHostToDevice, s));
    }
    DH_HIP(hipEventRecord(e->ev_stage, s));
    int rc;
    e->decode_tiled = step && g_decode_tiled_rows > 0 && n_seq >= g_decode_tiled_rows;
    if (e->fp8) {
        if ((rc = run_layers_fp8(e, ids, n_tok, n_seq, max_q, step, e->row_tail, s, prune_last))) return rc;
        e->last_ntok = n_tok;
        if (prune_last) return head_fp8(e, e->xlast, n_seq, logits_last, e->last_tail, s);
        if (logits_all && (rc = head_fp8(e, e->x, n_tok, logits_all, e->row_tail, s))) return rc;
        if (logits_last) {
            hipLaunchKernelGGL(gather_rows_kernel, dim3(cdiv(n_seq, 4)), dim3(256), 0, s, e->x, e->last_row, e->xlast, n_seq,
                               e->d.n_embd);
            DH_LAUNCH_CHECK();
            if ((rc = head_fp8(e, e->xlast, n_seq, logits_last, e->last_tail, s))) return rc;
        }
        return 0;
    }
    const bool fast = step && n_seq <= MAX_DECODE_ROWS && e->d.n_embd % 16 == 0 && !e->decode_tiled;
    if (fast) {
        if ((rc = run_layers_decode(e, ids, n_seq, e->row_tail, s))) return rc;
        e->last_ntok = n_tok;
        if (logits_all && (rc = head_normed(e, n_seq, logits_all, s))) return rc;
        if (logits_last && (rc = head_normed(e, n_seq, logits_last, s))) return rc;
        return 0;
    }
    if ((rc = run_layers(e, ids, n_tok, n_seq, max_q, step, e->row_tail, s, prune_last))) return rc;
    e->last_ntok = n_tok;
    if (prune_last) return head(e, e->xlast, n_seq, logits_last, e->last_tail, s);
    if (logits_all) {
        if ((rc = head(e, e->x, n_tok, logits_all, e->row_tail, s))) return rc;
    }
    if (logits_last) {
        hipLaunchKernelGGL(gather_rows_kernel, dim3(cdiv(n_seq, 4)), dim3(256), 0, s, e->x, e->last_row, e->xlast, n_seq,
                           e->d.n_embd);
        DH_LAUNCH_CHECK();
        if (logits_all) {
        }
        if ((rc = head(e, e->xlast, n_seq, logits_last, e->last_tail, s))) return rc;
    }
    return 0;
}

int decode_forward(dh_engine* e, int n_seq, hipStream_t s) {
    int rc;
    e->decode_tiled = g_decode_tiled_rows > 0 && n_seq >= g_decode_tiled_rows;
    if (e->fp8) {
        if ((rc = run_layers_fp8(e, e->dec_ids, n_seq, n_seq, 1, true, e->ones, s))) return rc;
        if ((rc = head_fp8(e, e->x, n_seq, e->logits, e->ones, s))) return rc;
    } else if (n_seq <= MAX_DECODE_ROWS && !e->decode_tiled) {
        if ((rc = run_layers_decode(e, e->dec_ids, n_seq, e->ones, s))) return rc;
        if ((rc = head_normed(e, n_seq, e->logits, s))) return rc;
    } else {
        if ((rc = run_layers(e, e->dec_ids, n_seq, n_seq, 1, true, e->ones, s))) return rc;
        if ((rc = head(e, e->x, n_seq, e->logits, e->ones, s))) return rc;
    }
    return 0;
}

int decode_step(dh_engine* e, int64_t* tokens, int tok_ld, int32_t* length, int32_t* done, int n_seq, float temperature,
                int top_k, int64_t eos_id, uint64_t seed, hipStream_t s) {
    int32_t* kv_len = e->seq_meta + 3 * e->max_batch;
    hipLaunchKernelGGL(decode_prep_kernel, dim3(cdiv(n_seq, 64)), dim3(64), 0, s, tokens, tok_ld, length, e->dec_ids,
                       e->tok_slot, e->tok_pos, kv_len, e->step_dev, n_seq, e->s_max);
    DH_LAUNCH_CHECK();
    int rc;
    if ((rc = decode_forward(e, n_seq, s))) return rc;
    return dh_sample_impl(e->logits, e->d.vocab, tokens, tok_ld, length, done, n_seq, temperature, top_k, eos_id,
                          seed, 0, e->step_dev, s);
}

int decode_rows_step(dh_engine* e, const dh_engine::GKey& k, hipStream_t s) {
    int32_t* kv_len = e->seq_meta + 3 * e->max_batch;
    hipLaunchKernelGGL(decode_prep_rows_kernel, dim3(cdiv(k.n_seq, 64)), dim3(64), 0, s, k.tokens, k.tok_ld, k.length, k.row_seq,
                       k.row_slot, e->dec_ids, e->tok_slot, e->tok_pos, kv_len, k.n_seq, k.n_all, e->max_batch, e->s_max);
    DH_LAUNCH_CHECK();
    int rc;
    if ((rc = decode_forward(e, k.n_seq, s))) return rc;
    return dh_sample_rows_impl(e->logits, e->d.vocab, k.tokens, k.tok_ld, k.length, k.done, k.limit, k.row_seq, k.n_seq, k.n_all,
                               k.max_new, k.temp, k.top_k, k.eos, k.seed, s);
}

int launch_steps(dh_engine* e, const dh_engine::GKey& key, int n_steps, hipStream_t s) {
    const bool rows = key.row_seq != nullptr;
    hipGraphExec_t gexec = nullptr;
    for (auto& g : e->graphs) {
        if (g.key == key) {
            gexec = g.exec;
            g.used = ++e->graph_clock;
            break;
        }
    }
    DH_HIP(hipEventRecord(e->ev_in, s));
    DH_HIP(hipStreamWaitEvent(e->gstream, e->ev_in, 0));
    if (!gexec) {
        hipGraph_t graph = nullptr;
        DH_HIP(hipStreamBeginCapture(e->gstream, hipStreamCaptureModeThreadLocal));
        e->capturing = true;
        int rc = rows ? decode_rows_step(e, key, e->gstream)
                      : decode_step(e, key.tokens, key.tok_ld, key.length, key.done, key.n_seq, key.temp, key.top_k, key.eos, key.seed, e->gstream);
        e->capturing = false;
        hipError_t ce = hipStreamEndCapture(e->gstream, &graph);
        if (rc) { if (graph) hipGraphDestroy(graph); return rc; }
        DH_CHECK(ce == hipSuccess && graph, "dh_engine_decode: graph capture failed: %s", hipGetErrorString(ce));
        hipError_t ie = hipGraphInstantiate(&gexec, graph, nullptr, nullptr, 0);
        hipGraphDestroy(graph);
        DH_CHECK(ie == hipSuccess, "dh_engine_decode: hipGraphInstantiate failed: %s", hipGetErrorString(ie));
        if (e->graphs.size() >= 8) {
            size_t lru = 0;
            for (size_t i = 1; i < e->graphs.size(); ++i)
                if (e->graphs[i].used < e->graphs[lru].used) lru = i;
            DH_HIP(hipStreamSynchronize(e->gstream));
            hipGraphExecDestroy(e->graphs[lru].exec);
            e->graphs.erase(e->graphs.begin() + lru);
        }
        e->graphs.push_back({key, gexec, ++e->graph_clock});
    }
    for (int i = 0; i < n_steps; ++i) DH_HIP(hipGraphLaunch(gexec, e->gstream));
    DH_HIP(hipEventRecord(e->ev_out, e->gstream));
    DH_HIP(hipStreamWaitEvent(s, e->ev_out, 0));
    return 0;
}

}

extern "C" int dh_engine_decode(dh_engine* e, int64_t* tokens, int tok_ld, int32_t* length, int32_t* done, int n_seq,
                                int n_steps, float temperature, int top_k, int64_t eos_id, uint64_t seed,
                                int first_step, void* stream) {
    DH_CHECK(e && tokens && length && done, "dh_engine_decode: null argument");
    DH_CHECK(n_seq > 0 && n_seq <= e->max_batch, "dh_engine_decode: n_seq=%d exceeds max_batch=%d", n_seq, e->max_batch);
    DH_CHECK(temperature > 0.f && top_k >= 0, "dh_engine_decode: bad sampling parameters");
    if (n_steps <= 0) return 0;
    e->slot_base = 0;
    e->seq_slot = e->seq_meta;
    hipStream_t s = (hipStream_t)stream;
    hipLaunchKernelGGL(set_i32_kernel, dim3(1), dim3(1), 0, s, e->step_dev, (int32_t)first_step);
    DH_LAUNCH_CHECK();
    const dh_engine::GKey key{tokens, tok_ld, length, done, n_seq, top_k, temperature, eos_id, seed, e->rsqrt_vec, g_decode_tiled_rows,
                              nullptr, nullptr, nullptr, 0, 0};
    return launch_steps(e, key, n_steps, s);
}

extern "C" int dh_engine_decode_rows(dh_engine* e, int64_t* tokens, int tok_ld, int32_t* length, int32_t* done, const int32_t* limit,
                                     int n_seq, int max_new_tokens, const int32_t* row_seq, const int32_t* row_slot, int n_rows,
                                     int n_steps, float temperature, int top_k, int64_t eos_id, uint64_t seed, void* stream) {
    DH_CHECK(e && tokens && length && done && limit && row_seq && row_slot, "dh_engine_decode_rows: null argument");
    DH_CHECK(n_rows > 0 && n_rows <= e->max_batch, "dh_engine_decode_rows: n_rows=%d exceeds max_batch=%d", n_rows, e->max_batch);
    DH_CHECK(n_seq > 0 && tok_ld > 0 && max_new_tokens > 0, "dh_engine_decode_rows: bad shape");
    DH_CHECK(temperature > 0.f && top_k >= 0, "dh_engine_decode_rows: bad sampling parameters");
    if (n_steps <= 0) return 0;
    e->slot_base = 0;
    e->seq_slot = row_slot;
    const dh_engine::GKey key{tokens, tok_ld, length, done, n_rows, top_k, temperature, eos_id, seed, e->rsqrt_vec, g_decode_tiled_rows,
                              limit, row_seq, row_slot, n_seq, max_new_tokens};
    return launch_steps(e, key, n_steps, (hipStream_t)stream);
}

extern "C" int dh_engine_set_cpu_rsqrt_emulation(dh_engine* e, int vec_width, int whole_call) {
    DH_CHECK(e && vec_width >= 0, "dh_engine_set_cpu_rsqrt_emulation: bad argument");
    e->rsqrt_vec = vec_width;
    e->rsqrt_whole = whole_call != 0;
    return 0;
}

extern "C" int dh_engine_set_timing(dh_engine* e, int on) {
    DH_CHECK(e, "dh_engine_set_timing: null engine");
    e->tm.on = on != 0;
    for (auto& v : e->tm.ev) {
        for (auto& p : v) { hipEventDestroy(p.first); hipEventDestroy(p.second); }
        v.clear();
    }
    return 0;
}

extern "C" int dh_engine_get_timing(dh_engine* e, int which, double* h_ms, int64_t* h_launches) {
    DH_CHECK(e && which >= 0 && which < 4 && h_ms && h_launches, "dh_engine_get_timing: bad argument");
    DH_HIP(hipDeviceSynchronize());
    double tot = 0;
    for (auto& p : e->tm.ev[which]) {
        float ms = 0;
        DH_HIP(hipEventElapsedTime(&ms, p.first, p.second));
        tot += ms;
    }
    *h_ms = tot;
    *h_launches = (int64_t)e->tm.ev[which].size();
    return 0;
}
```

### dualhyp_amd/csrc/gemm.h

```cpp
#pragma once
#include "common.h"

struct GemmArgs {
    const bf16_t* x;
    const bf16_t* w;
    const bf16_t* w2;
    bf16_t* y;
    const bf16_t* xa;
    const bf16_t* lora_a;
    const bf16_t* lora_b;
    const bf16_t* vec_a;
    const bf16_t* vec_b;
    const bf16_t* resid;
    int M, N, K;
    int xa_ld, split0, split1;
    float lora_scale;
    int nb_n, nb_m;
    int gm;
    int fast_epi;
    int resid_mul;
    const bf16_t* rope_cos;
    const bf16_t* rope_sin;
    const int32_t* tok_slot;
    const int32_t* tok_pos;
    bf16_t* q_out;
    bf16_t* k_cache;
    bf16_t* vT_cache;
    int n_head, n_groups, hs, s_max;
};

constexpr int DH_EPI_QKV = 4;



int dh_linear_skinny(const GemmArgs& a, int epilogue, hipStream_t s);
bool dh_linear_skinny_n_ok(int M, int N, int K, const void* x, const void* w, const void* y);
int dh_linear_skinny_n(const dh_bf16* x, const dh_bf16* w, dh_bf16* y, int M, int N, int K, hipStream_t s);
bool dh_linear_k64_ok(int M, int N, int K, const void* x, const void* w, const void* y, const void* mul);
int dh_linear_k64(const dh_bf16* x, const dh_bf16* w, const dh_bf16* mul, dh_bf16* y, int M, int N, hipStream_t s);
bool dh_linear_256_xa_ok(const GemmArgs& a, int epilogue);

bool dh_linear_mid_ok(const GemmArgs& a, int epilogue);
int dh_linear_mid(const GemmArgs& a, int epilogue, hipStream_t s);
extern int g_mid;

bool dh_linear_dt_ok(const GemmArgs& a, int epilogue, int seg);
int dh_linear_dt(const GemmArgs& a, int epilogue, int seg, hipStream_t s);
bool dh_chain_ok(int M, int n_main, int n_ext, int K, int ksplit);
bool dh_pairs_ok(int M, int n_main, int n_ext, int K, int ksplit);
int dh_pairs_tiled(const bf16_t* x, const bf16_t* w, const bf16_t* w_ext, float* y32, int M, int n_main, int n_ext, int K,
                   int kps, hipStream_t s);
int dh_chain_tiled(const bf16_t* x, const bf16_t* w, const bf16_t* w_ext, float* y32, int M, int n_main, int n_ext, int K,
                   int kps, hipStream_t s);
extern int g_dt_min_rows, g_chain_min_rows;

bool dh_linear_is_big(int M, int N, int epilogue);

int dh_linear_256(GemmArgs a, int epilogue, hipStream_t s);
extern int g_linear_phase;
extern int g_gemm_gm;
extern int g_gemm_variant;

int dh_linear_lora_impl(const dh_bf16* x, const dh_bf16* w, dh_bf16* y, int M, int N, int K, const dh_bf16* lora_a, const dh_bf16* lora_b,
                        float lora_scale, int split0, int split1, const dh_bf16* resid, dh_bf16* xa_work, int kernel, hipStream_t s);
int dh_linear_impl(const dh_bf16* x, const dh_bf16* w, dh_bf16* y, int M, int N, int K, int epilogue,
                   const dh_bf16* w2, const dh_bf16* xa, int xa_ld, const dh_bf16* lora_b, float lora_scale,
                   int split0, int split1, const dh_bf16* vec_a, const dh_bf16* vec_b, const dh_bf16* resid,
                   int kernel, hipStream_t s);
```

### dualhyp_amd/csrc/gemm_skinny.hip

```cpp
#include "common.h"
#include "gemm.h"

namespace {

constexpr int ROWS = 16;
constexpr int NW = 8;
constexpr int CH = 8;

template <int EPI, bool RESID>
__global__ __launch_bounds__(512, 2) void gemm_skinny_kernel(GemmArgs a) {
    __shared__ __attribute__((aligned(16))) float part[NW][32][ROWS];
    __shared__ __attribute__((aligned(16))) float part2[EPI == DH_EPI_SWIGLU ? NW : 1][32][ROWS];
    const int tid = threadIdx.x, lane = tid & 63, wave = tid >> 6;
    const int n0 = blockIdx.x * ROWS;
    const int lrow = lane & 15, kg = lane >> 4;
    constexpr bool SW = EPI == DH_EPI_SWIGLU;
    constexpr int CHK = SW ? CH / 2 : CH;
    const int kw = wave, kstride = NW;
    int n = n0 + lrow;
    n = n < a.N ? n : a.N - 1;
    const bf16_t* wrow = a.w + (size_t)n * a.K + kg * 8;
    const bf16_t* wrow2 = SW ? a.w2 + (size_t)n * a.K + kg * 8 : nullptr;
    int m_lo = lrow, m_hi = 16 + lrow;
    m_lo = m_lo < a.M ? m_lo : a.M - 1;
    m_hi = m_hi < a.M ? m_hi : a.M - 1;
    const bf16_t* xlo = a.x + (size_t)m_lo * a.K + kg * 8;
    const bf16_t* xhi = a.x + (size_t)m_hi * a.K + kg * 8;

    f32x4 acc_lo = {0.f, 0.f, 0.f, 0.f}, acc_hi = {0.f, 0.f, 0.f, 0.f};
    f32x4 acc2_lo = {0.f, 0.f, 0.f, 0.f}, acc2_hi = {0.f, 0.f, 0.f, 0.f};
    const int nks = a.K / 32;
    for (int ks0 = kw; ks0 < nks; ks0 += kstride * CHK) {
        bf16x8 wf[CHK], wf2[CHK], xl[CHK], xh[CHK];
#pragma unroll
        for (int c = 0; c < CHK; ++c) {
            const int ks = ks0 + c * kstride;
            if (ks < nks) {
                wf[c] = __builtin_nontemporal_load(reinterpret_cast<const bf16x8*>(wrow + ks * 32));
                if (SW) wf2[c] = __builtin_nontemporal_load(reinterpret_cast<const bf16x8*>(wrow2 + ks * 32));
                xl[c] = *reinterpret_cast<const bf16x8*>(xlo + ks * 32);
                xh[c] = *reinterpret_cast<const bf16x8*>(xhi + ks * 32);
            }
        }
#pragma unroll
        for (int c = 0; c < CHK; ++c) {
            const int ks = ks0 + c * kstride;
            if (ks < nks) {
                acc_lo = __builtin_amdgcn_mfma_f32_16x16x32_bf16(wf[c], xl[c], acc_lo, 0, 0, 0);
                acc_hi = __builtin_amdgcn_mfma_f32_16x16x32_bf16(wf[c], xh[c], acc_hi, 0, 0, 0);
                if (SW) {
                    acc2_lo = __builtin_amdgcn_mfma_f32_16x16x32_bf16(wf2[c], xl[c], acc2_lo, 0, 0, 0);
                    acc2_hi = __builtin_amdgcn_mfma_f32_16x16x32_bf16(wf2[c], xh[c], acc2_hi, 0, 0, 0);
                }
            }
        }
    }
    *reinterpret_cast<f32x4*>(&part[wave][lrow][kg * 4]) = acc_lo;
    *reinterpret_cast<f32x4*>(&part[wave][16 + lrow][kg * 4]) = acc_hi;
    if (SW) {
        *reinterpret_cast<f32x4*>(&part2[wave][lrow][kg * 4]) = acc2_lo;
        *reinterpret_cast<f32x4*>(&part2[wave][16 + lrow][kg * 4]) = acc2_hi;
    }
    __syncthreads();

    const int tn = tid & 15, tm = tid >> 4;
    const int nn = n0 + tn;
    if (tm >= a.M || nn >= a.N) return;
    const float* p = &part[0][0][0] + tm * ROWS + tn;
    float o;
    if (EPI == DH_EPI_SWIGLU) {
        float g = 0.f, u = 0.f;
        const float* p2 = &part2[0][0][0] + tm * ROWS + tn;
#pragma unroll
        for (int w = 0; w < NW; ++w) {
            g += p[w * 32 * ROWS];
            u += p2[w * 32 * ROWS];
        }
        g = rbf(g);
        u = rbf(u);
        o = rbf(silu_fast(g)) * u;
    } else {
        float s = 0.f;
#pragma unroll
        for (int w = 0; w < NW; ++w) s += p[w * 32 * ROWS];
        o = rbf(s);
        if (EPI == DH_EPI_LORA) {
            const int seg = (nn >= a.split0) + (nn >= a.split1);
            const uint4* xa4 = reinterpret_cast<const uint4*>(a.xa + (size_t)tm * a.xa_ld + seg * 16);
            const uint4* lb4 = reinterpret_cast<const uint4*>(a.lora_b + (size_t)nn * 16);
            float l = 0.f;
#pragma unroll
            for (int h = 0; h < 2; ++h) {
                const uint4 xv = xa4[h], bv = lb4[h];
                const bf16_t* xp = reinterpret_cast<const bf16_t*>(&xv);
                const bf16_t* bp = reinterpret_cast<const bf16_t*>(&bv);
#pragma unroll
                for (int e = 0; e < 8; ++e) l = fmaf(bf2f(xp[e]), bf2f(bp[e]), l);
            }
            o = rbf(o + rbf(rbf(l) * a.lora_scale));
        }
        if (EPI == DH_EPI_ADAPTER) o = rbf(bf2f(a.vec_a[nn]) * rbf(o + bf2f(a.vec_b[nn])));
        if (RESID) o = bf2f(a.resid[(size_t)tm * a.N + nn]) + o;
    }
    a.y[(size_t)tm * a.N + nn] = f2bf(o);
}

__global__ __launch_bounds__(512, 1) void swiglu_skinny2_kernel(GemmArgs a) {
    extern __shared__ __attribute__((aligned(16))) float part2x[];
    const int tid = threadIdx.x, lane = tid & 63, wave = tid >> 6;
    const int n0 = blockIdx.x * 32;
    const int lrow = lane & 15, kg = lane >> 4;
    int na = n0 + lrow, nb = n0 + 16 + lrow;
    na = na < a.N ? na : a.N - 1;
    nb = nb < a.N ? nb : a.N - 1;
    const bf16_t* w1a = a.w + (size_t)na * a.K + kg * 8;
    const bf16_t* w1b = a.w + (size_t)nb * a.K + kg * 8;
    const bf16_t* w2a = a.w2 + (size_t)na * a.K + kg * 8;
    const bf16_t* w2b = a.w2 + (size_t)nb * a.K + kg * 8;
    int m_lo = lrow, m_hi = 16 + lrow;
    m_lo = m_lo < a.M ? m_lo : a.M - 1;
    m_hi = m_hi < a.M ? m_hi : a.M - 1;
    const bf16_t* xlo = a.x + (size_t)m_lo * a.K + kg * 8;
    const bf16_t* xhi = a.x + (size_t)m_hi * a.K + kg * 8;
    f32x4 acc[2][2][2];
#pragma unroll
    for (int f = 0; f < 2; ++f)
#pragma unroll
        for (int t = 0; t < 2; ++t)
#pragma unroll
            for (int h = 0; h < 2; ++h) acc[f][t][h] = f32x4{0.f, 0.f, 0.f, 0.f};
    constexpr int C2 = 4;
    const int nks = a.K / 32;
    for (int ks0 = wave; ks0 < nks; ks0 += NW * C2) {
        bf16x8 f1a[C2], f1b[C2], f2a[C2], f2b[C2], xl[C2], xh[C2];
#pragma unroll
        for (int c = 0; c < C2; ++c) {
            const int ks = ks0 + c * NW;
            if (ks < nks) {
                f1a[c] = __builtin_nontemporal_load(reinterpret_cast<const bf16x8*>(w1a + ks * 32));
                f1b[c] = __builtin_nontemporal_load(reinterpret_cast<const bf16x8*>(w1b + ks * 32));
                f2a[c] = __builtin_nontemporal_load(reinterpret_cast<const bf16x8*>(w2a + ks * 32));
                f2b[c] = __builtin_nontemporal_load(reinterpret_cast<const bf16x8*>(w2b + ks * 32));
                xl[c] = *reinterpret_cast<const bf16x8*>(xlo + ks * 32);
                xh[c] = *reinterpret_cast<const bf16x8*>(xhi + ks * 32);
            }
        }
#pragma unroll
        for (int c = 0; c < C2; ++c) {
            const int ks = ks0 + c * NW;
            if (ks < nks) {
                acc[0][0][0] = __builtin_amdgcn_mfma_f32_16x16x32_bf16(f1a[c], xl[c], acc[0][0][0], 0, 0, 0);
                acc[0][0][1] = __builtin_amdgcn_mfma_f32_16x16x32_bf16(f1a[c], xh[c], acc[0][0][1], 0, 0, 0);
                acc[0][1][0] = __builtin_amdgcn_mfma_f32_16x16x32_bf16(f1b[c], xl[c], acc[0][1][0], 0, 0, 0);
                acc[0][1][1] = __builtin_amdgcn_mfma_f32_16x16x32_bf16(f1b[c], xh[c], acc[0][1][1], 0, 0, 0);
                acc[1][0][0] = __builtin_amdgcn_mfma_f32_16x16x32_bf16(f2a[c], xl[c], acc[1][0][0], 0, 0, 0);
                acc[1][0][1] = __builtin_amdgcn_mfma_f32_16x16x32_bf16(f2a[c], xh[c], acc[1][0][1], 0, 0, 0);
                acc[1][1][0] = __builtin_amdgcn_mfma_f32_16x16x32_bf16(f2b[c], xl[c], acc[1][1][0], 0, 0, 0);
                acc[1][1][1] = __builtin_amdgcn_mfma_f32_16x16x32_bf16(f2b[c], xh[c], acc[1][1][1], 0, 0, 0);
            }
        }
    }
#pragma unroll
    for (int f = 0; f < 2; ++f)
#pragma unroll
        for (int t = 0; t < 2; ++t)
#pragma unroll
            for (int h = 0; h < 2; ++h)
                *reinterpret_cast<f32x4*>(&part2x[(((f * NW + wave) * 32) + 16 * h + lrow) * 32 + 16 * t + kg * 4]) = acc[f][t][h];
    __syncthreads();
    for (int it = tid; it < 32 * 32; it += 512) {
        const int tn = it & 31, tm = it >> 5, nn = n0 + tn;
        if (tm >= a.M || nn >= a.N) continue;
        float g = 0.f, u = 0.f;
#pragma unroll
        for (int w = 0; w < NW; ++w) {
            g += part2x[((0 * NW + w) * 32 + tm) * 32 + tn];
            u += part2x[((1 * NW + w) * 32 + tm) * 32 + tn];
        }
        g = rbf(g);
        u = rbf(u);
        a.y[(size_t)tm * a.N + nn] = f2bf(rbf(silu_fast(g)) * u);
    }
}

int g_swiglu2 = 1;

__global__ __launch_bounds__(512, 2) void gemm_skinny_partial_kernel(const bf16_t* __restrict__ x,
                                                                   const bf16_t* __restrict__ w,
                                                                   const bf16_t* __restrict__ w_ext,
                                                                   float* __restrict__ y32, int M, int m_total,
                                                                   int n_main, int N, int K) {
    __shared__ __attribute__((aligned(16))) float part[NW][32][ROWS];
    const int tid = threadIdx.x, lane = tid & 63, wave = tid >> 6;
    const int n0 = blockIdx.x * ROWS, ksplit = gridDim.y;
    const int lrow = lane & 15, kg = lane >> 4;
    int n = n0 + lrow;
    n = n < N ? n : N - 1;
    const bf16_t* wrow = (n < n_main ? w + (size_t)n * K : w_ext + (size_t)(n - n_main) * K) + kg * 8;
    int m_lo = lrow, m_hi = 16 + lrow;
    m_lo = m_lo < M ? m_lo : M - 1;
    m_hi = m_hi < M ? m_hi : M - 1;
    const bf16_t* xlo = x + (size_t)m_lo * K + kg * 8;
    const bf16_t* xhi = x + (size_t)m_hi * K + kg * 8;
    f32x4 acc_lo = {0.f, 0.f, 0.f, 0.f}, acc_hi = {0.f, 0.f, 0.f, 0.f};
    const int nks = K / 32, kstride = NW * ksplit;
    for (int ks0 = blockIdx.y * NW + wave; ks0 < nks; ks0 += kstride * CH) {
        bf16x8 wf[CH], xl[CH], xh[CH];
#pragma unroll
        for (int c = 0; c < CH; ++c) {
            const int ks = ks0 + c * kstride;
            if (ks < nks) {
                wf[c] = __builtin_nontemporal_load(reinterpret_cast<const bf16x8*>(wrow + ks * 32));
                xl[c] = *reinterpret_cast<const bf16x8*>(xlo + ks * 32);
                xh[c] = *reinterpret_cast<const bf16x8*>(xhi + ks * 32);
            }
        }
#pragma unroll
        for (int c = 0; c < CH; ++c) {
            const int ks = ks0 + c * kstride;
            if (ks < nks) {
                acc_lo = __builtin_amdgcn_mfma_f32_16x16x32_bf16(wf[c], xl[c], acc_lo, 0, 0, 0);
                acc_hi = __builtin_amdgcn_mfma_f32_16x16x32_bf16(wf[c], xh[c], acc_hi, 0, 0, 0);
            }
        }
    }
    *reinterpret_cast<f32x4*>(&part[wave][lrow][kg * 4]) = acc_lo;
    *reinterpret_cast<f32x4*>(&part[wave][16 + lrow][kg * 4]) = acc_hi;
    __syncthreads();
    const int tn = tid & 15, tm = tid >> 4, nn = n0 + tn;
    if (tm >= M || nn >= N) return;
    const float* p = &part[0][0][0] + tm * ROWS + tn;
    float s = 0.f;
#pragma unroll
    for (int wv = 0; wv < NW; ++wv) s += p[wv * 32 * ROWS];
    y32[((size_t)blockIdx.y * m_total + tm) * N + nn] = s;
}

#ifdef DH_ROWS_NT_STORE
#define PSTORE(p, v) __builtin_nontemporal_store(v, reinterpret_cast<f32x4*>(p))
#else
#define PSTORE(p, v) (*reinterpret_cast<f32x4*>(p) = (v))
#endif
#ifdef DH_ROWS_STAMPS
__device__ unsigned long long g_rows_stamps[1024 * 8];
#define ROWS_STAMP(i) do { if (threadIdx.x == 0) { const int _b = blockIdx.x + gridDim.x * (blockIdx.y + gridDim.y * blockIdx.z); \
    if (_b < 1024) g_rows_stamps[_b * 8 + (i)] = __builtin_amdgcn_s_memrealtime(); } } while (0)
extern "C" int dh_debug_rows_stamps(unsigned long long* out) {
    return hipMemcpyFromSymbol(out, HIP_SYMBOL(g_rows_stamps), sizeof(g_rows_stamps)) == hipSuccess ? 0 : 1;
}
#else
#define ROWS_STAMP(i)
#endif

template <int KPS, int NG, int NGL, int CT>
__global__ __launch_bounds__(512, NG == 1 ? 2 : 1) void gemm_skinny_rows_kernel(const bf16_t* __restrict__ x,
                                                                              const bf16_t* __restrict__ w,
                                                                              const bf16_t* __restrict__ w_ext,
                                                                              float* __restrict__ y32, int M, int n_main,
                                                                              int N, int K) {
    constexpr int RB = KPS * 64;
    constexpr int RND = NGL * 32 * RB;
    constexpr int LPR = RB / 16;
    constexpr int XI = RND / 1024 / 8;
    constexpr int NR = (NG + NGL - 1) / NGL;
    static_assert(KPS % 2 == 0 && RND % 8192 == 0, "a line holds two k-steps; a round is a whole number of requests per wave");
    extern __shared__ __attribute__((aligned(16))) char sx[];
    const int tid = threadIdx.x, lane = tid & 63, wave = tid >> 6;
    const int lrow = lane & 15, kg = lane >> 4;
    const int n0 = blockIdx.x * (128 * CT) + wave * (16 * CT);
    const int m0 = blockIdx.z * (NG * 32);
    const int ks_begin = blockIdx.y * KPS;
    ROWS_STAMP(0);
    i32x4 raw[CT][KPS / 2][2];
#pragma unroll
    for (int ct = 0; ct < CT; ++ct)
#pragma unroll
        for (int h = 0; h < 2; ++h) {
            int n = n0 + ct * 16 + h * 8 + (lane >> 3);
            n = n < N ? n : N - 1;
            const bf16_t* wrow = (n < n_main ? w + (size_t)n * K : w_ext + (size_t)(n - n_main) * K) + ks_begin * 32 + (lane & 7) * 8;
#pragma unroll
            for (int c2 = 0; c2 < KPS / 2; ++c2) raw[ct][c2][h] = __builtin_nontemporal_load(reinterpret_cast<const i32x4*>(wrow + c2 * 64));
        }
    const int xrow_in = lane / LPR, xpos = lane % LPR;
    auto issue_x = [&](int r) __attribute__((always_inline)) {
        char* buf = sx + (r & 1) * RND;
#pragma unroll
        for (int i = 0; i < XI; ++i) {
            const int q = wave + 8 * i;
            const int row = q * (64 / LPR) + xrow_in;
            int m = m0 + r * (NGL * 32) + row;
            m = m < M ? m : M - 1;
            const int chunk = xpos ^ (row & 15);
            glds16(x + (size_t)m * K + ks_begin * 32 + chunk * 8, buf + q * 1024);
        }
    };
    const int rounds = min(NR, (M - m0 + NGL * 32 - 1) / (NGL * 32));
    issue_x(0);
    bf16x8 wf[CT][KPS];
    {
        const int fidx = frag_src_lane(lane) * 4;
#pragma unroll
        for (int ct = 0; ct < CT; ++ct)
#pragma unroll
            for (int c2 = 0; c2 < KPS / 2; ++c2) lines_to_frags(raw[ct][c2][0], raw[ct][c2][1], fidx, wf[ct][2 * c2], wf[ct][2 * c2 + 1]);
    }
    ROWS_STAMP(1);
    asm volatile("s_waitcnt vmcnt(0)" ::: "memory");
    __builtin_amdgcn_s_barrier();
    ROWS_STAMP(2);
    float* out = y32 + (size_t)blockIdx.y * M * N;
#pragma unroll
    for (int r = 0; r < NR; ++r) {
        if (r >= rounds) break;
        if (r + 1 < rounds) issue_x(r + 1);
        const char* buf = sx + (r & 1) * RND;
        f32x4 acc_lo[NGL][CT], acc_hi[NGL][CT];
#pragma unroll
        for (int g = 0; g < NGL; ++g) {
#pragma unroll
            for (int ct = 0; ct < CT; ++ct) acc_lo[g][ct] = acc_hi[g][ct] = f32x4{0.f, 0.f, 0.f, 0.f};
            if (r * NGL + g < NG && m0 + (r * NGL + g) * 32 < M) {
#pragma unroll
                for (int c = 0; c < KPS; ++c) {
                    const int co = ((c * 4 + kg) ^ lrow) << 4;
                    const bf16x8 xl = *reinterpret_cast<const bf16x8*>(buf + (g * 32 + lrow) * RB + co);
                    const bf16x8 xh = *reinterpret_cast<const bf16x8*>(buf + (g * 32 + 16 + lrow) * RB + co);
#pragma unroll
                    for (int ct = 0; ct < CT; ++ct) {
                        acc_lo[g][ct] = __builtin_amdgcn_mfma_f32_16x16x32_bf16(wf[ct][c], xl, acc_lo[g][ct], 0, 0, 0);
                        acc_hi[g][ct] = __builtin_amdgcn_mfma_f32_16x16x32_bf16(wf[ct][c], xh, acc_hi[g][ct], 0, 0, 0);
                    }
                }
            }
        }
        if (r + 1 < rounds) {
            asm volatile("s_waitcnt vmcnt(0)" ::: "memory");
            __builtin_amdgcn_s_barrier();
        }
        ROWS_STAMP(r == 0 ? 3 : 5);
#pragma unroll
        for (int g = 0; g < NGL; ++g) {
            const int mg = m0 + (r * NGL + g) * 32;
            if (r * NGL + g >= NG || mg >= M) break;
            if (CT >= 2 && n0 + 16 * CT <= N) {
                const int lidx = line_src_lane(lane) * 4;
#pragma unroll
                for (int cp = 0; cp + 1 < CT; cp += 2) {
                    float* o = out + n0 + cp * 16 + (lane & 7) * 4;
#pragma unroll
                    for (int h = 0; h < 2; ++h) {
                        f32x4 r0, r1;
                        tiles_to_lines(h ? acc_hi[g][cp] : acc_lo[g][cp], h ? acc_hi[g][cp + 1] : acc_lo[g][cp + 1], lidx, r0, r1);
                        const int m_a = mg + h * 16 + (lane >> 3), m_b = m_a + 8;
                        if (m_a < M) PSTORE(o + (size_t)m_a * N, r0);
                        if (m_b < M) PSTORE(o + (size_t)m_b * N, r1);
                    }
                }
            } else {
#pragma unroll
                for (int ct = 0; ct < CT; ++ct) {
                    const int nn = n0 + ct * 16 + kg * 4;
                    if (nn < N) {
                        if (mg + lrow < M) *reinterpret_cast<f32x4*>(out + (size_t)(mg + lrow) * N + nn) = acc_lo[g][ct];
                        if (mg + 16 + lrow < M) *reinterpret_cast<f32x4*>(out + (size_t)(mg + 16 + lrow) * N + nn) = acc_hi[g][ct];
                    }
                }
            }
        }
    }
    ROWS_STAMP(6);
}

int g_rows_ng = 0;
int g_rows_ct = 0;

template <int KPS, int NG, int CT>
int launch_rows(const bf16_t* x, const bf16_t* w, const bf16_t* w_ext, float* y32, int M, int n_main, int N, int K,
                int ksplit, hipStream_t s) {
    constexpr int NGL = NG == 1 ? 1 : (KPS == 8 ? (NG >= 4 ? 4 : 2) : 2);
    constexpr int lds = 2 * NGL * 32 * KPS * 64;
    static_assert(lds <= 160 * 1024, "x rounds do not fit in LDS");
    if (lds > 48 * 1024) DH_MAX_LDS_ONCE((gemm_skinny_rows_kernel<KPS, NG, NGL, CT>), lds);
    dim3 grid(cdiv(N, 128 * CT), ksplit, cdiv(M, NG * 32)), block(512);
    hipLaunchKernelGGL((gemm_skinny_rows_kernel<KPS, NG, NGL, CT>), grid, block, lds, s, x, w, w_ext, y32, M, n_main, N, K);
    DH_LAUNCH_CHECK();
    return 0;
}

template <int KPS>
int launch_rows_ng(const bf16_t* x, const bf16_t* w, const bf16_t* w_ext, float* y32, int M, int n_main, int N, int K,
                   int ksplit, hipStream_t s) {
    if (M <= 32) return launch_rows<KPS, 1, 1>(x, w, w_ext, y32, M, n_main, N, K, ksplit, s);
    if (M <= 64) return launch_rows<KPS, 2, 1>(x, w, w_ext, y32, M, n_main, N, K, ksplit, s);
    if (M <= 128) return launch_rows<KPS, 4, 1>(x, w, w_ext, y32, M, n_main, N, K, ksplit, s);
    constexpr int CTMAX = KPS == 8 ? 4 : 2;
    const int ct = g_rows_ct ? g_rows_ct : (M <= 256 ? 1 : 2);
    if (ct >= 4 && CTMAX >= 4) return launch_rows<KPS, 8, CTMAX>(x, w, w_ext, y32, M, n_main, N, K, ksplit, s);
    if (ct >= 2) {
        auto cost = [&](int ng) {
            const int blocks = cdiv(N, 256) * ksplit * cdiv(M, ng * 32);
            return cdiv(blocks, 256) * (5 + 2 * ng);
        };
        const bool ten = g_rows_ng ? g_rows_ng == 10 : cost(10) < cost(8);
        if (ten) return launch_rows<KPS, 10, 2>(x, w, w_ext, y32, M, n_main, N, K, ksplit, s);
        return launch_rows<KPS, 8, 2>(x, w, w_ext, y32, M, n_main, N, K, ksplit, s);
    }
    return launch_rows<KPS, 8, 1>(x, w, w_ext, y32, M, n_main, N, K, ksplit, s);
}

int g_skinny_variant = 1;

template <int EPI>
int launch(const GemmArgs& a, hipStream_t s) {
    dim3 grid(cdiv(a.N, ROWS)), block(512);
    if (a.resid)
        hipLaunchKernelGGL((gemm_skinny_kernel<EPI, true>), grid, block, 0, s, a);
    else
        hipLaunchKernelGGL((gemm_skinny_kernel<EPI, false>), grid, block, 0, s, a);
    DH_LAUNCH_CHECK();
    return 0;
}

template <int NT>
__global__ __launch_bounds__(256, 2) void gemm_skinny_n_kernel(const bf16_t* __restrict__ x, const bf16_t* __restrict__ w,
                                                               bf16_t* __restrict__ y, int M, int K, int ldy) {
    constexpr int RB = 64, NST = 4, XB = RB * 128, WB = NT * 16 * 128, STAGE = XB + WB;
    constexpr int WPW = (2 * NT + 3) / 4, NPW = 2 + WPW;
    extern __shared__ __attribute__((aligned(16))) char sn_smem[];
    const int lane = threadIdx.x & 63, wave = __builtin_amdgcn_readfirstlane(threadIdx.x >> 6);
    const int m0 = blockIdx.x * RB;
    uint32_t xo[2], wo[WPW];
    int wp[WPW];
#pragma unroll
    for (int i = 0; i < 2; ++i) {
        const int r = 8 * (2 * wave + i) + (lane >> 3);
        const int row = min(m0 + r, M - 1);
        xo[i] = ((uint32_t)row * (uint32_t)K + (uint32_t)(((lane & 7) ^ ((r >> 1) & 7)) * 8)) * 2u;
    }
#pragma unroll
    for (int i = 0; i < WPW; ++i) {
        wp[i] = min(wave + 4 * i, 2 * NT - 1);
        const int r = 8 * wp[i] + (lane >> 3);
        wo[i] = ((uint32_t)r * (uint32_t)K + (uint32_t)(((lane & 7) ^ ((r >> 1) & 7)) * 8)) * 2u;
    }
    auto issue = [&](int st) __attribute__((always_inline)) {
        char* base = sn_smem + (st % NST) * STAGE;
        const bf16_t* xs = x + (size_t)st * 64;
        const bf16_t* ws = w + (size_t)st * 64;
#pragma unroll
        for (int i = 0; i < 2; ++i) glds16_saddr(xs, xo[i], base + (2 * wave + i) * 1024);
#pragma unroll
        for (int i = 0; i < WPW; ++i) glds16_saddr(ws, wo[i], base + XB + wp[i] * 1024);
    };
    const int nst = K / 64;
    f32x4 acc[NT];
#pragma unroll
    for (int t = 0; t < NT; ++t) acc[t] = f32x4{0.f, 0.f, 0.f, 0.f};
    const int frow = lane & 15, kg = lane >> 4;
    const int xr = 16 * wave + frow;
#pragma unroll 1
    for (int st = 0; st < NST - 1 && st < nst; ++st) issue(st);
#pragma unroll 1
    for (int st = 0; st < nst; ++st) {
        if (st + NST - 2 < nst) asm volatile("s_waitcnt vmcnt(%0)" ::"n"((NST - 2) * NPW) : "memory");
        else asm volatile("s_waitcnt vmcnt(0)" ::: "memory");
        __syncthreads();
        if (st + NST - 1 < nst) issue(st + NST - 1);
        const char* base = sn_smem + (st % NST) * STAGE;
#pragma unroll
        for (int kh = 0; kh < 2; ++kh) {
            const int c = 4 * kh + kg;
            const bf16x8 bf = *reinterpret_cast<const bf16x8*>(base + xr * 128 + ((c ^ ((xr >> 1) & 7)) << 4));
#pragma unroll
            for (int t = 0; t < NT; ++t) {
                const int wr = 16 * t + frow;
                const bf16x8 af = *reinterpret_cast<const bf16x8*>(base + XB + wr * 128 + ((c ^ ((wr >> 1) & 7)) << 4));
                acc[t] = __builtin_amdgcn_mfma_f32_16x16x32_bf16(af, bf, acc[t], 0, 0, 0);
            }
        }
    }
    const int m = m0 + xr;
    if (m < M) {
#pragma unroll
        for (int t = 0; t < NT; ++t)
            *reinterpret_cast<uint2*>(y + (size_t)m * ldy + 16 * t + 4 * kg) = make_uint2(pack2bf(acc[t][0], acc[t][1]), pack2bf(acc[t][2], acc[t][3]));
    }
}

template <bool MUL>
__global__ __launch_bounds__(256, 4) void gemm_k64_kernel(const bf16_t* __restrict__ x, const bf16_t* __restrict__ w,
                                                          const bf16_t* __restrict__ mul, bf16_t* __restrict__ y, int M, int N) {
    constexpr int RB = 64, CB = 256, XB = RB * 128, WB = CB * 128;
    __shared__ __attribute__((aligned(16))) char k64_smem[XB + WB];
    const int lane = threadIdx.x & 63, wave = __builtin_amdgcn_readfirstlane(threadIdx.x >> 6);
    const int m0 = blockIdx.y * RB, n0 = blockIdx.x * CB;
#pragma unroll
    for (int i = 0; i < 2; ++i) {
        const int r = 8 * (2 * wave + i) + (lane >> 3);
        const int row = min(m0 + r, M - 1);
        glds16_saddr(x, ((uint32_t)row * 64u + (uint32_t)(((lane & 7) ^ ((r >> 1) & 7)) * 8)) * 2u, k64_smem + (2 * wave + i) * 1024);
    }
#pragma unroll
    for (int i = 0; i < 8; ++i) {
        const int r = 8 * (8 * wave + i) + (lane >> 3);
        const int row = min(n0 + r, N - 1);
        glds16_saddr(w, ((uint32_t)row * 64u + (uint32_t)(((lane & 7) ^ ((r >> 1) & 7)) * 8)) * 2u, k64_smem + XB + (8 * wave + i) * 1024);
    }
    asm volatile("s_waitcnt vmcnt(0)" ::: "memory");
    __syncthreads();
    const int frow = lane & 15, kg = lane >> 4;
    const int xr = 16 * wave + frow, m = m0 + xr;
    bf16x8 bf[2];
#pragma unroll
    for (int kh = 0; kh < 2; ++kh) bf[kh] = *reinterpret_cast<const bf16x8*>(k64_smem + xr * 128 + (((4 * kh + kg) ^ ((xr >> 1) & 7)) << 4));
    const bool m_ok = m < M;
    const int cpair = (kg & 1) * 16 + (kg >> 1) * 8;
#pragma unroll
    for (int tp = 0; tp < CB / 32; ++tp) {
        f32x4 acc[2];
#pragma unroll
        for (int h = 0; h < 2; ++h) {
            const int wr = 32 * tp + 16 * h + frow;
            acc[h] = f32x4{0.f, 0.f, 0.f, 0.f};
#pragma unroll
            for (int kh = 0; kh < 2; ++kh) {
                const bf16x8 af = *reinterpret_cast<const bf16x8*>(k64_smem + XB + wr * 128 + (((4 * kh + kg) ^ ((wr >> 1) & 7)) << 4));
                acc[h] = __builtin_amdgcn_mfma_f32_16x16x32_bf16(af, bf[kh], acc[h], 0, 0, 0);
            }
        }
        const uint2 ta = make_uint2(pack2bf(acc[0][0], acc[0][1]), pack2bf(acc[0][2], acc[0][3]));
        const uint2 tb = make_uint2(pack2bf(acc[1][0], acc[1][1]), pack2bf(acc[1][2], acc[1][3]));
        const auto rx = __builtin_amdgcn_permlane16_swap(ta.x, tb.x, false, false);
        const auto ry = __builtin_amdgcn_permlane16_swap(ta.y, tb.y, false, false);
        uint4 out = make_uint4(rx[0], ry[0], rx[1], ry[1]);
        const int n = n0 + 32 * tp + cpair;
        if (m_ok && n + 8 <= N) {
            if (MUL) {
                const uint4 mv = *reinterpret_cast<const uint4*>(mul + (size_t)m * N + n);
                auto mul2 = [](uint32_t y2, uint32_t r2) __attribute__((always_inline)) -> uint32_t {
                    return pack2bf(bf2f((bf16_t)(r2 & 0xffffu)) * bf2f((bf16_t)(y2 & 0xffffu)), bf2f((bf16_t)(r2 >> 16)) * bf2f((bf16_t)(y2 >> 16)));
                };
                out = make_uint4(mul2(out.x, mv.x), mul2(out.y, mv.y), mul2(out.z, mv.z), mul2(out.w, mv.w));
            }
            *reinterpret_cast<uint4*>(y + (size_t)m * N + n) = out;
        }
    }
}

}

extern "C" int dh_linear_partial_bf16(const dh_bf16* x, const dh_bf16* w, const dh_bf16* w_ext, float* y32, int M,
                                      int n_main, int n_ext, int K, int ksplit, void* stream) {
    DH_CHECK(x && w && y32 && M >= 1 && M <= 4096, "dh_linear_partial_bf16: need 1 <= M <= 4096 (got %d)", M);
    DH_CHECK(K % 32 == 0 && n_main % ROWS == 0 && n_ext % ROWS == 0 && n_main > 0 && n_ext >= 0,
             "dh_linear_partial_bf16: K %% 32 and row counts %% 16 must be 0");
    DH_CHECK(n_ext == 0 || w_ext, "dh_linear_partial_bf16: null w_ext");
    DH_CHECK(ksplit >= 1 && ksplit <= 16, "dh_linear_partial_bf16: ksplit must be 1..16");
    const int N = n_main + n_ext;
    const int nks = K / 32;
    const int kps = (nks + ksplit - 1) / ksplit;
    hipStream_t s = (hipStream_t)stream;
    if (g_skinny_variant == 1 && (kps == 8 || kps == 16) && ksplit * kps == nks && N % 4 == 0) {
        if (kps == 8) return launch_rows_ng<8>(x, w, w_ext ? w_ext : w, y32, M, n_main, N, K, ksplit, s);
        return launch_rows_ng<16>(x, w, w_ext ? w_ext : w, y32, M, n_main, N, K, ksplit, s);
    }
    DH_CHECK(ksplit <= 8, "dh_linear_partial_bf16: ksplit must be 1..8 for this shape");
    for (int m0 = 0; m0 < M; m0 += 32) {
        const int mm = M - m0 < 32 ? M - m0 : 32;
        hipLaunchKernelGGL(gemm_skinny_partial_kernel, dim3(N / ROWS, ksplit), dim3(512), 0, s, x + (size_t)m0 * K, w,
                           w_ext ? w_ext : w, y32 + (size_t)m0 * N, mm, M, n_main, N, K);
    }
    DH_LAUNCH_CHECK();
    return 0;
}

bool dh_chain_ok(int M, int n_main, int n_ext, int K, int ksplit) {
    const int nks = K / 32, kps = (nks + ksplit - 1) / ksplit, N = n_main + n_ext;
    return g_skinny_variant == 1 && M >= g_chain_min_rows && K % 64 == 0 && (kps == 8 || kps == 16) && (ksplit - 1) * kps < nks &&
           N % 4 == 0 && n_main % ROWS == 0 && n_ext % ROWS == 0;
}

int g_pairs_min_rows = 288;
bool dh_pairs_ok(int M, int n_main, int n_ext, int K, int ksplit) {
    const int nks = K / 32, kps = (nks + ksplit - 1) / ksplit, N = n_main + n_ext;
    return g_skinny_variant == 1 && M >= g_pairs_min_rows && K % 64 == 0 && (kps == 8 || kps == 16) && ksplit * kps == nks &&
           N % 4 == 0 && n_main % ROWS == 0 && n_ext % ROWS == 0;
}

extern "C" int dh_linear_partial_pairs_bf16(const dh_bf16* x, const dh_bf16* w, const dh_bf16* w_ext, float* y32, int M,
                                            int n_main, int n_ext, int K, int ksplit, void* stream) {
    DH_CHECK(x && w && y32 && M >= 1 && ksplit >= 1 && ksplit <= 16 && (n_ext == 0 || w_ext), "dh_linear_partial_pairs_bf16: bad argument");
    const int nks = K / 32, kps = (nks + ksplit - 1) / ksplit;
    DH_CHECK(K % 64 == 0 && (kps == 8 || kps == 16) && ksplit * kps == nks && (n_main + n_ext) % 4 == 0 && n_main % ROWS == 0 &&
             n_ext % ROWS == 0, "dh_linear_partial_pairs_bf16: unsupported shape N=%d+%d K=%d ksplit=%d (K %% 64 == 0, whole K-slices of 8 or 16 k-steps)",
             n_main, n_ext, K, ksplit);
    return dh_pairs_tiled(x, w, w_ext, y32, M, n_main, n_ext, K, kps, (hipStream_t)stream);
}

extern "C" int dh_linear_chain_bf16(const dh_bf16* x, const dh_bf16* w, const dh_bf16* w_ext, float* y32, int M, int n_main,
                                    int n_ext, int K, int ksplit, void* stream) {
    DH_CHECK(x && w && y32 && M >= 1 && ksplit >= 1 && (n_ext == 0 || w_ext), "dh_linear_chain_bf16: bad argument");
    DH_CHECK(dh_chain_ok(M, n_main, n_ext, K, ksplit),
             "dh_linear_chain_bf16: unsupported shape M=%d N=%d+%d K=%d ksplit=%d (needs >= %d rows, K %% 64 == 0, K-slices of 8 or 16 k-steps)",
             M, n_main, n_ext, K, ksplit, g_chain_min_rows);
    const int kps = (K / 32 + ksplit - 1) / ksplit;
    return dh_chain_tiled(x, w, w_ext, y32, M, n_main, n_ext, K, kps, (hipStream_t)stream);
}

int g_skinny_n = 1;
bool dh_linear_skinny_n_ok(int M, int N, int K, const void* x, const void* w, const void* y) {
    return g_skinny_n && N >= 16 && N <= 64 && N % 16 == 0 && M >= 512 && K >= 64 && K % 64 == 0 && (size_t)M * K * 2 < (1ull << 32) &&
           (((uintptr_t)x | (uintptr_t)w) & 15) == 0 && ((uintptr_t)y & 7) == 0;
}
int dh_linear_skinny_n(const dh_bf16* x, const dh_bf16* w, dh_bf16* y, int M, int N, int K, hipStream_t s) {
    const dim3 grid(cdiv(M, 64)), block(256);
    const int nt = N / 16, lds = 4 * (64 * 128 + nt * 16 * 128);
    switch (nt) {
        case 1: hipLaunchKernelGGL((gemm_skinny_n_kernel<1>), grid, block, lds, s, x, w, y, M, K, N); break;
        case 2: hipLaunchKernelGGL((gemm_skinny_n_kernel<2>), grid, block, lds, s, x, w, y, M, K, N); break;
        case 3: hipLaunchKernelGGL((gemm_skinny_n_kernel<3>), grid, block, lds, s, x, w, y, M, K, N); break;
        default: hipLaunchKernelGGL((gemm_skinny_n_kernel<4>), grid, block, lds, s, x, w, y, M, K, N); break;
    }
    DH_LAUNCH_CHECK();
    return 0;
}

bool dh_linear_k64_ok(int M, int N, int K, const void* x, const void* w, const void* y, const void* mul) {
    return g_skinny_n && K == 64 && N >= 256 && N % 8 == 0 && M >= 512 && (size_t)M * 128 < (1ull << 32) && (size_t)N * 128 < (1ull << 32) &&
           (((uintptr_t)x | (uintptr_t)w | (uintptr_t)y | (uintptr_t)mul) & 15) == 0;
}
int dh_linear_k64(const dh_bf16* x, const dh_bf16* w, const dh_bf16* mul, dh_bf16* y, int M, int N, hipStream_t s) {
    const dim3 grid(cdiv(N, 256), cdiv(M, 64)), block(256);
    if (mul) hipLaunchKernelGGL((gemm_k64_kernel<true>), grid, block, 0, s, x, w, mul, y, M, N);
    else hipLaunchKernelGGL((gemm_k64_kernel<false>), grid, block, 0, s, x, w, mul, y, M, N);
    DH_LAUNCH_CHECK();
    return 0;
}

extern "C" int dh_set_tuning(int key, int value) {
    if (key == 0) { g_skinny_variant = value; return 0; }
    if (key == 1) { g_gemm_variant = value; return 0; }
    if (key == 2) { g_swiglu2 = value; return 0; }
    if (key == 3) { g_mid = value; return 0; }
    if (key == 4) { g_linear_phase = value; return 0; }
    if (key == 5 && value >= 0) { g_gemm_gm = value; return 0; }
    if (key == 6 && value >= 1) { g_dt_min_rows = value; return 0; }
    if (key == 7 && value >= 1) { g_chain_min_rows = value; return 0; }
    if (key == 8) { extern int g_dt_stages; g_dt_stages = value; return 0; }
    if (key == 9) { extern int g_gemm128_stages; g_gemm128_stages = value; return 0; }
    if (key == 10 && value >= 0) { extern int g_decode_tiled_rows; g_decode_tiled_rows = value; return 0; }
    if (key == 11 && value >= 0) { g_rows_ct = value; return 0; }
    if (key == 12) { extern int g_fuse_qkv_rope; g_fuse_qkv_rope = value; return 0; }
    if (key == 14 && (value == 0 || value == 8 || value == 10)) { g_rows_ng = value; return 0; }
    if (key == 16 && (value == 8 || value == 16)) { extern int g_short_kps; g_short_kps = value; return 0; }
    if (key == 15) { extern int g_dt_wide; g_dt_wide = value; return 0; }
    if (key == 13) { extern int g_mid_wlds; g_mid_wlds = value; return 0; }
    if (key == 17 && (value == 0 || value == 2 || value == 4)) { extern int g_pairs_wn; g_pairs_wn = value; return 0; }
    if (key == 18 && value >= 1) { g_pairs_min_rows = value; return 0; }
    if (key == 21) { extern int g_pairs_wt; g_pairs_wt = value != 0; return 0; }
    if (key == 19 && (value == 0 || value == 128 || value == 256)) { extern int g_fp8_tile; g_fp8_tile = value; return 0; }
    if (key == 20 && value >= 0 && value <= 64) { extern int g_fp8_gm; g_fp8_gm = value; return 0; }
    if (key == 22 && value >= 0 && value <= 2) { extern int g_w4_persist; g_w4_persist = value; return 0; }
    if (key == 23) { extern int g_prune_last_layer; g_prune_last_layer = value != 0; return 0; }
    if (key == 24) { extern int g_w4_fast_epi; g_w4_fast_epi = value; return 0; }
    if (key == 25) { extern int g_w4_persist_qkv; g_w4_persist_qkv = value != 0; return 0; }
    if (key == 26) { extern int g_tn_mfma; g_tn_mfma = value != 0; return 0; }
    if (key == 31) { g_skinny_n = value != 0; return 0; }
    if (key == 30) { extern int g_w4_persist_lora; g_w4_persist_lora = value != 0; return 0; }
    if (key == 29) { extern int g_attn_bwd_dkdv_img; g_attn_bwd_dkdv_img = value != 0; return 0; }
    if (key == 28) { extern int g_tail_split; g_tail_split = value != 0; return 0; }
    if (key == 27) { extern int g_attn_bwd_dq_group; g_attn_bwd_dq_group = value != 0; return 0; }
    dh_set_error("dh_set_tuning: unknown key %d", key);
    return 1;
}

int dh_linear_skinny(const GemmArgs& a, int epilogue, hipStream_t s) {
    if (epilogue == DH_EPI_SWIGLU && g_swiglu2 && a.N % 32 == 0) {
        DH_MAX_LDS_ONCE(swiglu_skinny2_kernel, 64 * 1024);
        hipLaunchKernelGGL(swiglu_skinny2_kernel, dim3(a.N / 32), dim3(512), 64 * 1024, s, a);
        DH_LAUNCH_CHECK();
        return 0;
    }
    switch (epilogue) {
        case DH_EPI_PLAIN: return launch<DH_EPI_PLAIN>(a, s);
        case DH_EPI_LORA: return launch<DH_EPI_LORA>(a, s);
        case DH_EPI_SWIGLU: return launch<DH_EPI_SWIGLU>(a, s);
        case DH_EPI_ADAPTER: return launch<DH_EPI_ADAPTER>(a, s);
    }
    dh_set_error("dh_linear_bf16: unknown epilogue %d", epilogue);
    return 1;
}
```

### dualhyp_amd/ops.py

```python
from __future__ import annotations

import os
from typing import Sequence, Optional, Tuple

import torch

from . import _lib
from ._lib import check

EPI_PLAIN, EPI_LORA, EPI_SWIGLU, EPI_ADAPTER = 0, 1, 2, 3


def _p(t: Optional[torch.Tensor]):
    return None if t is None else t.data_ptr()


def _stream() -> int:
    return torch.cuda.current_stream().cuda_stream


def _dev(t: torch.Tensor, dtype=torch.bfloat16, name="tensor") -> torch.Tensor:
    if not t.is_cuda:
        raise _lib.DualHypHipError(f"{name} must live on the GPU: the HIP path has no CPU fallback")
    if t.dtype != dtype:
        raise TypeError(f"{name} must be {dtype}, got {t.dtype}")
    return t if t.is_contiguous() else t.contiguous()


class _Keep(list):

    def __call__(self, t: Optional[torch.Tensor], dtype=torch.bfloat16, name: str = "tensor"):
        if t is None:
            return None
        t = _dev(t, dtype, name)
        self.append(t)
        return t.data_ptr()


def embed(ids: torch.Tensor, wte: torch.Tensor) -> torch.Tensor:
    ids = _dev(ids.reshape(-1), torch.int64, "ids")
    wte = _dev(wte, name="wte")
    out = torch.empty((ids.numel(), wte.size(1)), dtype=torch.bfloat16, device=wte.device)
    check(_lib.load().dh_embed_bf16(_p(ids), _p(wte), _p(out), ids.numel(), wte.size(1), wte.size(0), _stream()))
    return out


def rmsnorm(x: torch.Tensor, w: torch.Tensor, eps: float, resid: Optional[torch.Tensor] = None,
            return_sum: bool = False, row_tail: Optional[torch.Tensor] = None):
    x = _dev(x, name="x")
    w = _dev(w, name="weight")
    d = x.size(-1)
    rows = x.numel() // d
    out = torch.empty_like(x)
    s = torch.empty_like(x) if (resid is not None and return_sum) else None
    if resid is not None:
        resid = _dev(resid, name="resid")
    if row_tail is not None:
        row_tail = _dev(row_tail.reshape(-1), torch.uint8, "row_tail")
        assert row_tail.numel() == rows
    check(_lib.load().dh_rmsnorm_bf16(_p(x), _p(resid), _p(w), _p(out), _p(s), rows, d, float(eps), _p(row_tail),
                                      _stream()))
    return (out, s) if return_sum else out


def linear(x: torch.Tensor, w: torch.Tensor, *, epilogue: int = EPI_PLAIN, w2: Optional[torch.Tensor] = None,
           xa: Optional[torch.Tensor] = None, lora_b: Optional[torch.Tensor] = None, lora_scale: float = 1.0,
           splits: Optional[Tuple[int, int]] = None, scale: Optional[torch.Tensor] = None,
           bias: Optional[torch.Tensor] = None, resid: Optional[torch.Tensor] = None,
           out: Optional[torch.Tensor] = None) -> torch.Tensor:
    x = _dev(x, name="x")
    w = _dev(w, name="w")
    K = x.size(-1)
    M = x.numel() // K
    N = w.size(0)
    assert w.size(1) == K, f"weight is {tuple(w.shape)}, input feature size {K}"
    y = out if out is not None else torch.empty((*x.shape[:-1], N), dtype=torch.bfloat16, device=x.device)
    s0, s1 = splits if splits is not None else (N, N)
    xa_ld = 0
    if xa is not None:
        xa = _dev(xa, name="xa")
        xa_ld = xa.size(-1)
    for t, nm in ((w2, "w2"), (lora_b, "lora_b"), (scale, "scale"), (bias, "bias"), (resid, "resid")):
        if t is not None:
            _dev(t, name=nm)
            assert t.is_contiguous(), f"{nm} must be contiguous"
    check(_lib.load().dh_linear_bf16(_p(x), _p(w), _p(y), M, N, K, epilogue, _p(w2), _p(xa), xa_ld, _p(lora_b),
                                     float(lora_scale), s0, s1, _p(scale), _p(bias), _p(resid), _stream()))
    return y


def qkv_rope_cache(qkv: torch.Tensor, cos: torch.Tensor, sin: torch.Tensor, tok_slot: torch.Tensor,
                   tok_pos: torch.Tensor, k_cache: torch.Tensor, vT_cache: torch.Tensor, n_head: int,
                   n_groups: int, k_out: Optional[torch.Tensor] = None, v_out: Optional[torch.Tensor] = None) -> torch.Tensor:
    k = _Keep()
    qkv = _dev(qkv, name="qkv")
    hs = k_cache.size(-1)
    s_max = k_cache.size(-2)
    n_tok = qkv.numel() // ((n_head + 2 * n_groups) * hs)
    q = torch.empty((n_tok, n_head, hs), dtype=torch.bfloat16, device=qkv.device)
    check(_lib.load().dh_qkv_rope_cache_bf16(_p(qkv), k(cos), k(sin), k(tok_slot, torch.int32),
                                             k(tok_pos, torch.int32), _p(q), _p(k_cache), _p(vT_cache), _p(k_out),
                                             _p(v_out), n_tok, n_head, n_groups, hs, s_max, _stream()))
    return q


def linear_qkv_rope_cache(x: torch.Tensor, w: torch.Tensor, cos: torch.Tensor, sin: torch.Tensor, tok_slot: torch.Tensor,
                          tok_pos: torch.Tensor, k_cache: torch.Tensor, vT_cache: torch.Tensor, n_head: int, n_groups: int,
                          xa: Optional[torch.Tensor] = None, lora_b: Optional[torch.Tensor] = None,
                          lora_scale: float = 1.0) -> torch.Tensor:
    k = _Keep()
    x = _dev(x, name="x")
    K = x.size(-1)
    M = x.numel() // K
    hs, s_max = k_cache.size(-1), k_cache.size(-2)
    q = torch.empty((M, n_head, hs), dtype=torch.bfloat16, device=x.device)
    check(_lib.load().dh_linear_qkv_rope_cache_bf16(_p(x), k(w, name="w"), M, K, k(xa, name="xa"), 0 if xa is None else xa.size(-1),
                                                    k(lora_b, name="lora_b"), float(lora_scale), k(cos), k(sin),
                                                    k(tok_slot, torch.int32), k(tok_pos, torch.int32), _p(q), _p(k_cache),
                                                    _p(vT_cache), n_head, n_groups, hs, s_max, _stream()))
    return q


def linear_lora(x: torch.Tensor, w: torch.Tensor, lora_a: torch.Tensor, lora_b: torch.Tensor, *, lora_scale: float = 1.0,
                splits: Optional[Tuple[int, int]] = None, resid: Optional[torch.Tensor] = None) -> torch.Tensor:
    x, w, lora_a, lora_b = _dev(x, name="x"), _dev(w, name="w"), _dev(lora_a, name="lora_a"), _dev(lora_b, name="lora_b")
    K = x.size(-1)
    M, N = x.numel() // K, w.size(0)
    s0, s1 = splits if splits is not None else (N, N)
    nseg = 1 + (s0 < N) + (s1 < N)
    assert lora_a.shape == (16 * nseg, K) and lora_b.shape == (N, 16), (lora_a.shape, lora_b.shape)
    if resid is not None:
        _dev(resid, name="resid")
    y = torch.empty((*x.shape[:-1], N), dtype=torch.bfloat16, device=x.device)
    work = torch.empty((M, 16 * nseg), dtype=torch.bfloat16, device=x.device)
    check(_lib.load().dh_linear_lora_bf16(_p(x), _p(w), _p(y), M, N, K, _p(lora_a), _p(lora_b), float(lora_scale), s0, s1, _p(resid),
                                          _p(work), _stream()))
    return y


def linear_qkv_lora_rope_cache(x: torch.Tensor, w: torch.Tensor, lora_a: torch.Tensor, lora_b: torch.Tensor, cos: torch.Tensor,
                               sin: torch.Tensor, tok_slot: torch.Tensor, tok_pos: torch.Tensor, k_cache: torch.Tensor,
                               vT_cache: torch.Tensor, n_head: int, n_groups: int, *, lora_scale: float = 1.0) -> torch.Tensor:
    k = _Keep()
    M, K = x.shape
    hs = k_cache.size(-1)
    q = torch.empty((M, n_head, hs), dtype=torch.bfloat16, device=x.device)
    work = torch.empty((M, 48), dtype=torch.bfloat16, device=x.device)
    i32 = torch.int32
    check(_lib.load().dh_linear_qkv_lora_rope_cache_bf16(k(x), k(w), M, K, k(lora_a), k(lora_b), float(lora_scale), k(cos), k(sin),
                                                         k(tok_slot, i32), k(tok_pos, i32), _p(q), _p(k_cache), _p(vT_cache), n_head,
                                                         n_groups, hs, k_cache.size(2), _p(work), _stream()))
    return q


def attn_prefill(q: torch.Tensor, k_cache: torch.Tensor, vT_cache: torch.Tensor, seq_slot: torch.Tensor,
                 q_start: torch.Tensor, q_len: torch.Tensor, kv_pos0: torch.Tensor, max_q_len: int,
                 lse: Optional[torch.Tensor] = None) -> torch.Tensor:
    k = _Keep()
    n_tok, n_head, hs = q.shape
    n_groups, s_max = k_cache.size(1), k_cache.size(2)
    y = torch.empty((n_tok, n_head * hs), dtype=torch.bfloat16, device=q.device)
    i32 = torch.int32
    check(_lib.load().dh_attn_prefill_bf16(k(q), _p(k_cache), _p(vT_cache), k(seq_slot, i32),
                                           k(q_start, i32), k(q_len, i32), k(kv_pos0, i32), _p(y), _p(lse),
                                           seq_slot.numel(), int(max_q_len), n_head, n_groups, hs, s_max, _stream()))
    return y


def attn_decode(q: torch.Tensor, k_cache: torch.Tensor, vT_cache: torch.Tensor, seq_slot: torch.Tensor,
                kv_len: torch.Tensor) -> torch.Tensor:
    k = _Keep()
    n_seq, n_head, hs = q.shape
    n_groups, s_max = k_cache.size(1), k_cache.size(2)
    lib = _lib.load()
    work = torch.empty(lib.dh_attn_decode_work_bytes(n_seq, n_head, hs, s_max), dtype=torch.uint8, device=q.device)
    y = torch.empty((n_seq, n_head * hs), dtype=torch.bfloat16, device=q.device)
    i32 = torch.int32
    check(lib.dh_attn_decode_bf16(k(q), _p(k_cache), _p(vT_cache), k(seq_slot, i32),
                                  k(kv_len, i32), _p(y), _p(work), n_seq, n_head, n_groups, hs, s_max, _stream()))
    return y


def sample(logits: torch.Tensor, tokens: torch.Tensor, length: torch.Tensor, done: torch.Tensor, *,
           temperature: float = 1.0, top_k: Optional[int] = None, eos_id: Optional[int] = None, seed: int = 0,
           step: int = 0) -> None:
    k = _Keep()
    logits = _dev(logits, name="logits")
    n_seq, vocab = logits.shape
    assert tokens.dtype == torch.int64 and tokens.is_contiguous() and tokens.size(0) == n_seq
    check(_lib.load().dh_sample_bf16(_p(logits), vocab, _p(tokens), tokens.size(1), k(length, torch.int32),
                                     k(done, torch.int32), n_seq, float(temperature),
                                     0 if top_k is None else int(top_k), -1 if eos_id is None else int(eos_id),
                                     int(seed) & ((1 << 64) - 1), int(step), _stream()))


def sample_rows(logits: torch.Tensor, tokens: torch.Tensor, length: torch.Tensor, done: torch.Tensor, limit: torch.Tensor,
                row_seq: torch.Tensor, max_new_tokens: int, *, temperature: float = 1.0, top_k: Optional[int] = None,
                eos_id: Optional[int] = None, seed: int = 0) -> None:
    k = _Keep()
    logits = _dev(logits, name="logits")
    n_rows, vocab = logits.shape
    n_seq = tokens.size(0)
    assert tokens.dtype == torch.int64 and tokens.is_contiguous() and row_seq.numel() == n_rows
    assert length.numel() == done.numel() == limit.numel() == n_seq
    check(_lib.load().dh_sample_rows_bf16(_p(logits), vocab, _p(tokens), tokens.size(1), k(length, torch.int32),
                                          k(done, torch.int32), k(limit, torch.int32), k(row_seq, torch.int32), n_rows, n_seq,
                                          int(max_new_tokens), float(temperature), 0 if top_k is None else int(top_k),
                                          -1 if eos_id is None else int(eos_id), int(seed) & ((1 << 64) - 1), _stream()))


def quant_rows_fp8(x: torch.Tensor) -> Tuple[torch.Tensor, torch.Tensor]:
    x = _dev(x, name="x")
    K = x.size(-1)
    rows = x.numel() // K
    q = torch.empty((rows, K), dtype=torch.uint8, device=x.device)
    s = torch.empty(rows, dtype=torch.float32, device=x.device)
    check(_lib.load().dh_quant_rows_fp8(_p(x), _p(q), _p(s), rows, K, _stream()))
    return q, s


def rmsnorm_quant_fp8(x: torch.Tensor, w: torch.Tensor, eps: float, row_tail: Optional[torch.Tensor] = None):
    k = _Keep()
    x = _dev(x, name="x")
    d = x.size(-1)
    rows = x.numel() // d
    xn = torch.empty_like(x)
    q = torch.empty((rows, d), dtype=torch.uint8, device=x.device)
    s = torch.empty(rows, dtype=torch.float32, device=x.device)
    check(_lib.load().dh_rmsnorm_quant_fp8(_p(x), k(w, name="weight"), _p(xn), _p(q), _p(s), rows, d, float(eps),
                                           k(row_tail, torch.uint8, "row_tail"), _stream()))
    return xn, q, s


def linear_fp8(xq: torch.Tensor, x_scale: torch.Tensor, wq: torch.Tensor, w_scale: torch.Tensor, *, epilogue: int = EPI_PLAIN,
               w2q: Optional[torch.Tensor] = None, w2_scale: Optional[torch.Tensor] = None, scale: Optional[torch.Tensor] = None,
               bias: Optional[torch.Tensor] = None, resid: Optional[torch.Tensor] = None, kernel: int = 0) -> torch.Tensor:
    k = _Keep()
    M, K = xq.shape
    N = wq.size(0)
    assert wq.size(1) == K and xq.dtype == torch.uint8 and wq.dtype == torch.uint8
    y = torch.empty((M, N), dtype=torch.bfloat16, device=xq.device)
    check(_lib.load().dh_linear_fp8_ex(k(xq, torch.uint8, "xq"), k(x_scale, torch.float32, "x_scale"), k(wq, torch.uint8, "wq"),
                                       k(w_scale, torch.float32, "w_scale"), _p(y), M, N, K, epilogue, k(w2q, torch.uint8, "w2q"),
                                       k(w2_scale, torch.float32, "w2_scale"), k(scale, name="scale"), k(bias, name="bias"),
                                       k(resid, name="resid"), int(kernel), _stream()))
    return y


def im2col3(x: torch.Tensor, ld: int, relu: bool = False) -> torch.Tensor:
    x = _dev(x, name="x")
    B, T, Cc = x.shape
    out = torch.empty((B * T, ld), dtype=torch.bfloat16, device=x.device)
    check(_lib.load().dh_im2col3_bf16(_p(x), _p(out), B, T, Cc, ld, int(relu), _stream()))
    return out


def pool_head(h: torch.Tensor, w: torch.Tensor, bias: torch.Tensor, pool: int) -> torch.Tensor:
    k = _Keep()
    h = _dev(h, name="h")
    B, T, H = h.shape
    out = torch.empty((B, (T + pool - 1) // pool, 3), dtype=torch.bfloat16, device=h.device)
    check(_lib.load().dh_pool_head_bf16(_p(h), k(w, name="w"), k(bias, name="bias"), _p(out), B, T, H, int(pool),
                                        _stream()))
    return out


def pool_head_bwd(h: torch.Tensor, w: torch.Tensor, dlogits: torch.Tensor, pool: int) -> Tuple[torch.Tensor, torch.Tensor]:
    k = _Keep()
    h = _dev(h, name="h")
    B, T, H = h.shape
    P = (T + pool - 1) // pool
    assert dlogits.shape == (B, P, 3)
    dh = torch.empty_like(h)
    pooled = torch.empty((B * P, H), dtype=torch.bfloat16, device=h.device)
    check(_lib.load().dh_pool_head_bwd_bf16(_p(h), k(w, name="w"), k(dlogits, torch.float32, "dlogits"), _p(dh), _p(pooled),
                                            B, T, H, int(pool), _stream()))
    return dh, pooled


def col2im3(dcol: torch.Tensor, B: int, T: int, C: int, pre: Optional[torch.Tensor] = None,
            mask: Optional[torch.Tensor] = None) -> torch.Tensor:
    k = _Keep()
    dcol = _dev(dcol, name="dcol")
    assert dcol.dim() == 2 and dcol.size(0) == B * T and dcol.size(1) >= 3 * C
    dx = torch.empty((B, T, C), dtype=torch.bfloat16, device=dcol.device)
    check(_lib.load().dh_col2im3_bf16(_p(dcol), k(pre, name="pre"), k(mask, name="mask"), _p(dx), B, T, C, dcol.size(1), _stream()))
    return dx


def cross_entropy_fwd(logits: torch.Tensor, targets: torch.Tensor) -> Tuple[torch.Tensor, torch.Tensor]:
    assert logits.dtype in (torch.bfloat16, torch.float32), f"logits must be bf16 or fp32, got {logits.dtype}"
    lg = _dev(logits.reshape(-1, logits.size(-1)), logits.dtype, "logits")
    tg = _dev(targets.reshape(-1), torch.int64, "targets")
    assert tg.numel() == lg.size(0), f"{tg.numel()} targets for {lg.size(0)} rows"
    loss = torch.empty(lg.size(0), dtype=torch.float32, device=lg.device)
    lse = torch.empty_like(loss)
    check(_lib.load().dh_cross_entropy_fwd(_p(lg), int(lg.dtype == torch.float32), _p(tg), _p(loss), _p(lse), lg.size(0),
                                           lg.size(1), _stream()))
    return loss, lse


def cross_entropy_bwd(logits: torch.Tensor, targets: torch.Tensor, lse: torch.Tensor, grad_row: torch.Tensor) -> torch.Tensor:
    k = _Keep()
    lg = _dev(logits.reshape(-1, logits.size(-1)), logits.dtype, "logits")
    tg = _dev(targets.reshape(-1), torch.int64, "targets")
    out = torch.empty_like(lg)
    check(_lib.load().dh_cross_entropy_bwd(_p(lg), int(lg.dtype == torch.float32), _p(tg), k(lse, torch.float32, "lse"),
                                           k(grad_row, torch.float32, "grad_row"), _p(out), lg.size(0), lg.size(1),
                                           _stream()))
    return out.view(logits.shape)


def linear_partial(x: torch.Tensor, w: torch.Tensor, w_ext: Optional[torch.Tensor] = None, ksplit: int = 1) -> torch.Tensor:
    x, w = _dev(x, name="x"), _dev(w, name="w")
    K = x.size(-1)
    M = x.numel() // K
    n_ext = 0 if w_ext is None else _dev(w_ext, name="w_ext").size(0)
    y = torch.empty((ksplit, M, w.size(0) + n_ext), dtype=torch.float32, device=x.device)
    check(_lib.load().dh_linear_partial_bf16(_p(x), _p(w), _p(w_ext), _p(y), M, w.size(0), n_ext, K, ksplit, _stream()))
    return y


def linear_partial_pairs(x: torch.Tensor, w: torch.Tensor, w_ext: Optional[torch.Tensor] = None, ksplit: int = 1) -> torch.Tensor:
    x, w = _dev(x, name="x"), _dev(w, name="w")
    K = x.size(-1)
    M = x.numel() // K
    n_ext = 0 if w_ext is None else _dev(w_ext, name="w_ext").size(0)
    y = torch.empty(((ksplit + 1) // 2, M, w.size(0) + n_ext), dtype=torch.float32, device=x.device)
    check(_lib.load().dh_linear_partial_pairs_bf16(_p(x), _p(w), _p(w_ext), _p(y), M, w.size(0), n_ext, K, ksplit, _stream()))
    return y


def combine_partials(parts: torch.Tensor, pairs: bool = True) -> torch.Tensor:
    if pairs:
        n = parts.size(0)
        parts = torch.stack([parts[i] + parts[i + 1] if i + 1 < n else parts[i] for i in range(0, n, 2)])
    out = parts[0].clone()
    for p in parts[1:]:
        out = out + p
    return out


def linear_chain(x: torch.Tensor, w: torch.Tensor, w_ext: Optional[torch.Tensor] = None, ksplit: int = 1) -> torch.Tensor:
    x, w = _dev(x, name="x"), _dev(w, name="w")
    K = x.size(-1)
    M = x.numel() // K
    n_ext = 0 if w_ext is None else _dev(w_ext, name="w_ext").size(0)
    y = torch.empty((M, w.size(0) + n_ext), dtype=torch.float32, device=x.device)
    check(_lib.load().dh_linear_chain_bf16(_p(x), _p(w), _p(w_ext), _p(y), M, w.size(0), n_ext, K, ksplit, _stream()))
    return y


def finish_norm(h32: torch.Tensor, d: int, x_resid: torch.Tensor, w_norm: torch.Tensor, eps: float,
                lora_b: Optional[torch.Tensor] = None, lora_scale: float = 1.0,
                row_tail: Optional[torch.Tensor] = None, pairs: bool = True) -> Tuple[torch.Tensor, torch.Tensor]:
    k = _Keep()
    n_part, rows, ld = h32.shape
    x_resid = _dev(x_resid, name="x_resid")
    x_out, xn_out = torch.empty_like(x_resid), torch.empty_like(x_resid)
    check(_lib.load().dh_finish_norm_bf16(_p(h32), n_part, int(pairs), rows, d, ld - d, _p(lora_b), float(lora_scale), _p(x_resid),
                                          k(w_norm), _p(x_out), _p(xn_out), float(eps), _p(row_tail), _stream()))
    return x_out, xn_out


def attn_decode_fused(qkv32: torch.Tensor, qkv_dim: int, lora_b: Optional[torch.Tensor], lora_scale: float,
                      splits: Tuple[int, int], cos: torch.Tensor, sin: torch.Tensor, seq_slot: torch.Tensor,
                      kv_len: torch.Tensor, k_cache: torch.Tensor, vT_cache: torch.Tensor, n_head: int,
                      pairs: bool = True) -> torch.Tensor:
    k = _Keep()
    n_part, n_seq, ld = qkv32.shape
    n_groups, s_max, hs = k_cache.size(1), k_cache.size(2), k_cache.size(3)
    y = torch.empty((n_seq, n_head * hs), dtype=torch.bfloat16, device=qkv32.device)
    i32 = torch.int32
    check(_lib.load().dh_attn_decode_fused_bf16(_p(qkv32), n_part, int(pairs), n_seq, qkv_dim, ld - qkv_dim, _p(lora_b),
                                                float(lora_scale), splits[0], splits[1], k(cos), k(sin),
                                                k(seq_slot, i32), k(kv_len, i32), _p(k_cache), _p(vT_cache),
                                                _p(y), n_head, n_groups, hs, s_max, _stream()))
    return y


def kcache_to_plain(kc: torch.Tensor) -> torch.Tensor:
    B, G, S, hs = kc.shape
    v = kc.reshape(B, G, S // 32, hs // 16, 2, 32, 8)
    return v.permute(0, 1, 2, 5, 3, 4, 6).reshape(B, G, S, hs)


def vcache_to_plain(vt: torch.Tensor) -> torch.Tensor:
    B, G, hs, S = vt.shape
    v = vt.reshape(B, G, S // 32, hs // 32, 2, 2, 32, 2, 4)
    return v.permute(0, 1, 3, 6, 2, 4, 7, 5, 8).reshape(B, G, hs, S)


def dropout(x: torch.Tensor, p: float, seed: int, call_id: int, step: Optional[torch.Tensor] = None):
    x = _dev(x, name="x")
    y, m = torch.empty_like(x), torch.empty_like(x)
    check(_lib.load().dh_dropout_bf16(_p(x), _p(y), _p(m), x.numel(), float(p), int(seed) & (2 ** 64 - 1), int(call_id) & 0xffffffff,
                                      _p(step) if step is not None else None, _stream()))
    return y, m


def swiglu_fwd(g: torch.Tensor, u: torch.Tensor) -> torch.Tensor:
    k = _Keep()
    act = torch.empty_like(g)
    check(_lib.load().dh_swiglu_fwd_bf16(k(g), k(u), _p(act), g.numel(), _stream()))
    return act


def linear_swiglu_train(x: torch.Tensor, w1: torch.Tensor, w2: torch.Tensor):
    k = _Keep()
    M, K = x.shape
    I = w1.size(0)
    act = torch.empty((M, I), dtype=torch.bfloat16, device=x.device)
    g, u = torch.empty_like(act), torch.empty_like(act)
    check(_lib.load().dh_linear_swiglu_train_bf16(k(x), k(w1), k(w2), _p(act), _p(g), _p(u), M, I, K, _stream()))
    return act, g, u


def linear_mul(x: torch.Tensor, w: torch.Tensor, mul: torch.Tensor) -> torch.Tensor:
    M, K = x.shape
    N = w.size(0)
    if (M >= 256 and N >= 256 and -(-M // 256) * -(-N // 256) >= 128 and mul.is_contiguous() and mul.shape == (M, N)
            and not os.environ.get("DUALHYP_NO_LINEAR_MUL")):
        k = _Keep()
        y = torch.empty((M, N), dtype=torch.bfloat16, device=x.device)
        check(_lib.load().dh_linear_mul_bf16(k(x), k(w), _p(y), M, N, K, k(mul), _stream()))
        return y
    return linear(x, w) * mul


def swiglu_bwd(dact: torch.Tensor, g: torch.Tensor, u: torch.Tensor) -> torch.Tensor:
    k = _Keep()
    rows, I = g.shape
    out = torch.empty((rows, 2 * I), dtype=torch.bfloat16, device=g.device)
    check(_lib.load().dh_swiglu_bwd_bf16(k(dact), k(g), k(u), _p(out), rows, I, _stream()))
    return out


def rmsnorm_bwd(dy: torch.Tensor, x: torch.Tensor, w: torch.Tensor, eps: float, dres: Optional[torch.Tensor] = None) -> torch.Tensor:
    k = _Keep()
    d = x.size(-1)
    dx = torch.empty_like(x)
    check(_lib.load().dh_rmsnorm_bwd_bf16(k(dy), k(x), k(w), k(dres, name="dres"), _p(dx), x.numel() // d, d,
                                          float(eps), _stream()))
    return dx


def qkv_rope_bwd(dq: torch.Tensor, dk: torch.Tensor, dv: torch.Tensor, cos: torch.Tensor, sin: torch.Tensor,
                 tok_pos: torch.Tensor) -> torch.Tensor:
    k = _Keep()
    n_tok, n_head, hs = dq.shape
    n_groups = dk.size(1)
    out = torch.empty((n_tok, (n_head + 2 * n_groups) * hs), dtype=torch.bfloat16, device=dq.device)
    check(_lib.load().dh_qkv_rope_bwd_bf16(k(dq), k(dk), k(dv), k(cos), k(sin),
                                           k(tok_pos, torch.int32), _p(out), n_tok, n_head, n_groups, hs, _stream()))
    return out


def tn_accum(a: torch.Tensor, b: torch.Tensor, out: torch.Tensor, scale: float = 1.0, accumulate: bool = True,
             splits: Optional[Tuple[int, int]] = None) -> None:
    assert a.stride(1) == 1 and b.stride(1) == 1 and out.dtype == torch.float32 and out.stride(1) == 1
    T, M = a.shape
    N = b.size(1) if splits is None else 16
    lib = _lib.load()
    wb = lib.dh_tn_accum_work_bytes(T, M, N)
    work = torch.empty(wb // 4, dtype=torch.float32, device=a.device) if wb else None
    if splits is not None:
        check(lib.dh_tn_accum_seg_f32(a.data_ptr(), a.stride(0), b.data_ptr(), b.stride(0), out.data_ptr(), out.stride(0),
                                      T, M, int(splits[0]), int(splits[1]), float(scale), int(accumulate), _p(work), _stream()))
        return
    check(lib.dh_tn_accum_f32(a.data_ptr(), a.stride(0), b.data_ptr(), b.stride(0), out.data_ptr(), out.stride(0),
                              T, M, N, float(scale), int(accumulate), _p(work), _stream()))


def attn_bwd_plan(q_start: torch.Tensor, q_len: torch.Tensor, n_tok: int, lens: Sequence[int]) -> dict:
    dev = q_len.device
    n_pad = sum(-(-n // 32) * 32 for n in lens)
    pads_dev = (q_len + 31) // 32 * 32
    pad_start = (torch.cumsum(pads_dev, 0) - pads_dev).to(torch.int32)
    tok_seq = torch.repeat_interleave(torch.arange(len(lens), dtype=torch.int64, device=dev), q_len.to(torch.int64), output_size=n_tok)
    tok = torch.arange(n_tok, dtype=torch.int64, device=dev)
    pp = pad_start.to(torch.int64)[tok_seq] + (tok - q_start.to(torch.int64)[tok_seq])
    pad_tok = torch.full((n_pad,), -1, dtype=torch.int32, device=dev)
    pad_tok[pp] = tok.to(torch.int32)
    return {"n_pad": n_pad, "pad_start": pad_start, "pad_tok": pad_tok, "n_seq": len(lens)}


def attn_bwd(q, k, v, out, dout, lse, q_start, q_len, max_q_len: int, lens: Optional[Sequence[int]] = None, plan: Optional[dict] = None):
    keep = _Keep()
    n_tok, H, hs = q.shape
    G = k.size(1)
    lib = _lib.load()
    dev = q.device
    if plan is None:
        if lens is None:
            lens = q_len.tolist()
        plan = attn_bwd_plan(q_start, q_len, n_tok, lens)
    n_pad, pad_start, pad_tok = plan["n_pad"], plan["pad_start"], plan["pad_tok"]
    dout = _dev(dout.reshape(n_tok, H, hs))
    dsum = torch.empty((n_tok, H), dtype=torch.float32, device=dev)
    check(lib.dh_rowdot_f32(_p(dout), keep(out.reshape(n_tok, H, hs)), _p(dsum), n_tok * H, hs, _stream()))

    def tpad(src, heads):
        dst = torch.empty((heads, hs, n_pad), dtype=torch.bfloat16, device=dev)
        check(lib.dh_transpose_frag_bf16(keep(src), _p(dst), _p(pad_tok), heads, hs, n_pad, _stream()))
        return dst
    need = lib.dh_attn_bwd_transposes(H, G, hs, n_pad)
    qT, doT = (tpad(q, H), tpad(dout, H)) if need & 1 else (None, None)
    kT = tpad(k, G)
    dq, dk, dv = torch.empty_like(q), torch.empty_like(k), torch.empty_like(v)
    check(lib.dh_attn_bwd_bf16(keep(q, name="q"), keep(k, name="k"), keep(v, name="v"), _p(dout), _p(qT), _p(doT), _p(kT), _p(lse), _p(dsum), _p(q_start),
                               _p(q_len), _p(pad_start), _p(dq), _p(dk), _p(dv), plan["n_seq"], int(max_q_len), H, G, hs,
                               n_pad, _stream()))
    return dq, dk, dv
```

### include/dualhyp_hip.h

```cpp
#ifndef DUALHYP_HIP_H
#define DUALHYP_HIP_H

#include <stdint.h>

#ifdef __cplusplus
extern "C" {
#endif

typedef uint16_t dh_bf16;

#define DH_ABI_VERSION 6

int dh_abi_version(void);
int dh_set_tuning(int key, int value);
const char* dh_last_error(void);
int dh_device_info(char* h_buf, int h_buf_len, int* h_num_cu, int64_t* h_hbm_bytes);


int dh_embed_bf16(const int64_t* ids, const dh_bf16* wte, dh_bf16* out, int n_tok, int d,
                  int vocab, void* stream);

int dh_rmsnorm_bf16(const dh_bf16* x, const dh_bf16* resid, const dh_bf16* w, dh_bf16* out,
                    dh_bf16* sum_out, int rows, int d, float eps, const uint8_t* row_tail,
                    void* stream);

int dh_qkv_rope_cache_bf16(const dh_bf16* qkv, const dh_bf16* cos, const dh_bf16* sin,
                           const int32_t* tok_slot, const int32_t* tok_pos, dh_bf16* q_out,
                           dh_bf16* k_cache, dh_bf16* vT_cache, dh_bf16* k_out, dh_bf16* v_out,
                           int n_tok, int n_head, int n_groups, int hs, int s_max, void* stream);


#define DH_EPI_PLAIN   0
#define DH_EPI_LORA    1
#define DH_EPI_SWIGLU  2
#define DH_EPI_ADAPTER 3

int dh_linear_bf16(const dh_bf16* x, const dh_bf16* w, dh_bf16* y, int M, int N, int K,
                   int epilogue, const dh_bf16* w2, const dh_bf16* xa, int xa_ld,
                   const dh_bf16* lora_b, float lora_scale, int split0, int split1,
                   const dh_bf16* vec_a, const dh_bf16* vec_b, const dh_bf16* resid,
                   void* stream);

int dh_linear_qkv_rope_cache_bf16(const dh_bf16* x, const dh_bf16* w, int M, int K, const dh_bf16* xa, int xa_ld,
                                  const dh_bf16* lora_b, float lora_scale, const dh_bf16* cos, const dh_bf16* sin,
                                  const int32_t* tok_slot, const int32_t* tok_pos, dh_bf16* q_out, dh_bf16* k_cache,
                                  dh_bf16* vT_cache, int n_head, int n_groups, int hs, int s_max, void* stream);

int dh_linear_lora_bf16(const dh_bf16* x, const dh_bf16* w, dh_bf16* y, int M, int N, int K, const dh_bf16* lora_a,
                        const dh_bf16* lora_b, float lora_scale, int split0, int split1, const dh_bf16* resid,
                        dh_bf16* xa_work, void* stream);
int dh_linear_qkv_lora_rope_cache_bf16(const dh_bf16* x, const dh_bf16* w, int M, int K, const dh_bf16* lora_a,
                                       const dh_bf16* lora_b, float lora_scale, const dh_bf16* cos, const dh_bf16* sin,
                                       const int32_t* tok_slot, const int32_t* tok_pos, dh_bf16* q_out, dh_bf16* k_cache,
                                       dh_bf16* vT_cache, int n_head, int n_groups, int hs, int s_max, dh_bf16* xa_work,
                                       void* stream);

int dh_linear_partial_bf16(const dh_bf16* x, const dh_bf16* w, const dh_bf16* w_ext, float* y32,
                           int M, int n_main, int n_ext, int K, int ksplit, void* stream);
int dh_linear_partial_pairs_bf16(const dh_bf16* x, const dh_bf16* w, const dh_bf16* w_ext, float* y32, int M,
                                 int n_main, int n_ext, int K, int ksplit, void* stream);
int dh_linear_chain_bf16(const dh_bf16* x, const dh_bf16* w, const dh_bf16* w_ext, float* y32, int M,
                         int n_main, int n_ext, int K, int ksplit, void* stream);

int dh_finish_norm_bf16(const float* h32, int n_part, int pairs, int rows, int d, int n_ext,
                        const dh_bf16* lora_b, float lora_scale, const dh_bf16* x_resid,
                        const dh_bf16* w_norm, dh_bf16* x_out, dh_bf16* xn_out, float eps,
                        const uint8_t* row_tail, void* stream);


int dh_attn_prefill_bf16(const dh_bf16* q, const dh_bf16* k_cache, const dh_bf16* vT_cache,
                         const int32_t* seq_slot, const int32_t* q_start, const int32_t* q_len,
                         const int32_t* kv_pos0, dh_bf16* y, float* lse, int n_seq, int max_q_len,
                         int n_head, int n_groups, int hs, int s_max, void* stream);

int64_t dh_attn_decode_work_bytes(int n_seq, int n_head, int hs, int s_max);
int dh_attn_decode_bf16(const dh_bf16* q, const dh_bf16* k_cache, const dh_bf16* vT_cache,
                        const int32_t* seq_slot, const int32_t* kv_len, dh_bf16* y, void* work,
                        int n_seq, int n_head, int n_groups, int hs, int s_max, void* stream);

int dh_attn_decode_fused_bf16(const float* qkv32, int n_part, int pairs, int n_seq, int qkv_dim, int n_ext,
                              const dh_bf16* lora_b, float lora_scale, int split0, int split1,
                              const dh_bf16* cos, const dh_bf16* sin, const int32_t* seq_slot,
                              const int32_t* kv_len, dh_bf16* k_cache, dh_bf16* vT_cache,
                              dh_bf16* y, int n_head, int n_groups, int hs, int s_max,
                              void* stream);


int dh_dropout_bf16(const dh_bf16* x, dh_bf16* y, dh_bf16* mask, int64_t n, float p, uint64_t seed, uint32_t call_id,
                    const uint64_t* step_dev, void* stream);
int dh_swiglu_fwd_bf16(const dh_bf16* g, const dh_bf16* u, dh_bf16* act, int64_t n, void* stream);
int dh_linear_mul_bf16(const dh_bf16* x, const dh_bf16* w, dh_bf16* y, int M, int N, int K,
                       const dh_bf16* mul, void* stream);
int dh_linear_swiglu_train_bf16(const dh_bf16* x, const dh_bf16* w1, const dh_bf16* w2, dh_bf16* act,
                                dh_bf16* g, dh_bf16* u, int M, int I, int K, void* stream);
int dh_swiglu_bwd_bf16(const dh_bf16* dact, const dh_bf16* g, const dh_bf16* u, dh_bf16* dgu, int rows,
                       int I, void* stream);
int dh_rmsnorm_bwd_bf16(const dh_bf16* dy, const dh_bf16* x, const dh_bf16* w, const dh_bf16* dres,
                        dh_bf16* dx, int rows, int d, float eps, void* stream);
int dh_qkv_rope_bwd_bf16(const dh_bf16* dq, const dh_bf16* dk, const dh_bf16* dv, const dh_bf16* cos,
                         const dh_bf16* sin, const int32_t* tok_pos, dh_bf16* dqkv, int n_tok,
                         int n_head, int n_groups, int hs, void* stream);
int64_t dh_tn_accum_work_bytes(int T, int M, int N);
int dh_tn_accum_f32(const dh_bf16* a, int lda, const dh_bf16* b, int ldb, float* out, int ldo, int T,
                    int M, int N, float scale, int accumulate, void* work, void* stream);
int dh_tn_accum_seg_f32(const dh_bf16* a, int lda, const dh_bf16* b, int ldb, float* out, int ldo, int T,
                        int M, int seg0, int seg1, float scale, int accumulate, void* work, void* stream);
int dh_rowdot_f32(const dh_bf16* a, const dh_bf16* b, float* out, int64_t rows, int hs, void* stream);
int dh_transpose_pad_bf16(const dh_bf16* src, dh_bf16* dst, const int32_t* tok_seq,
                          const int32_t* q_start, const int32_t* pad_start, int n_tok, int heads,
                          int hs, int n_pad, void* stream);
int dh_transpose_frag_bf16(const dh_bf16* src, dh_bf16* dst, const int32_t* pad_tok, int heads, int hs,
                           int n_pad, void* stream);
int dh_attn_bwd_transposes(int n_head, int n_groups, int hs, int n_pad);
int dh_attn_bwd_bf16(const dh_bf16* q, const dh_bf16* k, const dh_bf16* v, const dh_bf16* dout,
                     const dh_bf16* qT, const dh_bf16* doT, const dh_bf16* kT, const float* lse,
                     const float* dsum, const int32_t* q_start, const int32_t* q_len,
                     const int32_t* pad_start, dh_bf16* dq, dh_bf16* dk, dh_bf16* dv, int n_seq,
                     int max_q_len, int n_head, int n_groups, int hs, int n_pad, void* stream);


int dh_cross_entropy_fwd(const void* logits, int is_f32, const int64_t* targets, float* loss,
                         float* lse, int rows, int vocab, void* stream);
int dh_cross_entropy_bwd(const void* logits, int is_f32, const int64_t* targets, const float* lse,
                         const float* grad_row, void* dlogits, int rows, int vocab, void* stream);

int dh_im2col3_bf16(const dh_bf16* x, dh_bf16* out, int B, int T, int C, int ld, int relu, void* stream);
int dh_pool_head_bf16(const dh_bf16* h, const dh_bf16* w, const dh_bf16* bias, dh_bf16* out, int B, int T,
                      int H, int pool, void* stream);
int dh_pool_head_bwd_bf16(const dh_bf16* h, const dh_bf16* w, const float* dlogits, dh_bf16* dh, dh_bf16* pooled,
                          int B, int T, int H, int pool, void* stream);
int dh_col2im3_bf16(const dh_bf16* dcol, const dh_bf16* pre, const dh_bf16* mask, dh_bf16* dx, int B, int T, int C,
                    int ld, void* stream);

int dh_sample_bf16(const dh_bf16* logits, int vocab, int64_t* tokens, int tok_ld, int32_t* length,
                   int32_t* done, int n_seq, float temperature, int top_k, int64_t eos_id,
                   uint64_t seed, int step, void* stream);

int dh_sample_rows_bf16(const dh_bf16* logits, int vocab, int64_t* tokens, int tok_ld, int32_t* length,
                        int32_t* done, const int32_t* limit, const int32_t* row_seq, int n_rows, int n_seq,
                        int max_new_tokens, float temperature, int top_k, int64_t eos_id, uint64_t seed,
                        void* stream);


int dh_quant_rows_fp8(const dh_bf16* x, uint8_t* q, float* scale, int rows, int K, void* stream);
int dh_rmsnorm_quant_fp8(const dh_bf16* x, const dh_bf16* w, dh_bf16* xn_out, uint8_t* q, float* scale, int rows, int d,
                         float eps, const uint8_t* row_tail, void* stream);
int dh_linear_fp8(const uint8_t* xq, const float* x_scale, const uint8_t* wq, const float* w_scale, dh_bf16* y, int M, int N,
                  int K, int epilogue, const uint8_t* w2q, const float* w2_scale, const dh_bf16* vec_a, const dh_bf16* vec_b,
                  const dh_bf16* resid, void* stream);
int dh_linear_fp8_ex(const uint8_t* xq, const float* x_scale, const uint8_t* wq, const float* w_scale, dh_bf16* y, int M, int N,
                     int K, int epilogue, const uint8_t* w2q, const float* w2_scale, const dh_bf16* vec_a, const dh_bf16* vec_b,
                     const dh_bf16* resid, int kernel, void* stream);

int dh_linear_fp8_f32(const uint8_t* xq, const float* x_scale, const uint8_t* wq, const float* w_scale, float* y32, int M,
                      int N, int K, void* stream);


typedef struct dh_layer_weights {
    const dh_bf16* norm_1;
    const dh_bf16* norm_2;
    const dh_bf16* attn_w;
    const dh_bf16* attn_lora_a;
    const dh_bf16* attn_lora_b;
    const dh_bf16* proj_w;
    const dh_bf16* proj_lora_a;
    const dh_bf16* proj_lora_b;
    const dh_bf16* fc_1;
    const dh_bf16* fc_2;
    const dh_bf16* mlp_proj;
    const float* attn_ws;
    const float* proj_ws;
    const float* fc_1_ws;
    const float* fc_2_ws;
    const float* mlp_proj_ws;
} dh_layer_weights;

typedef struct dh_model_desc {
    int32_t n_layer, n_head, n_groups, head_size, n_embd, intermediate, vocab, block_size;
    float norm_eps;
    float lora_scale;
    const dh_bf16* wte;
    int32_t wte_rows;
    const dh_bf16* ln_f;
    const dh_bf16* rope_cos;
    const dh_bf16* rope_sin;
    const dh_bf16* lm_head;
    const dh_bf16* adapter_scale;
    const dh_bf16* adapter_bias;
    const dh_layer_weights* h_layers;
    const float* lm_head_ws;
} dh_model_desc;

typedef struct dh_engine dh_engine;

int dh_engine_create(const dh_model_desc* h_desc, int max_batch, int s_max, int max_tokens,
                     dh_engine** h_out);
void dh_engine_destroy(dh_engine* e);
int64_t dh_engine_device_bytes(const dh_engine* e);

int dh_engine_forward(dh_engine* e, const int64_t* ids, const int32_t* h_seq_len,
                      const int32_t* h_pos0, int n_seq, dh_bf16* logits_all,
                      dh_bf16* logits_last, void* stream);
int dh_engine_forward_at(dh_engine* e, const int64_t* ids, const int32_t* h_seq_len,
                         const int32_t* h_pos0, int n_seq, int slot_base, dh_bf16* logits_all,
                         dh_bf16* logits_last, void* stream);
int dh_engine_forward_slots(dh_engine* e, const int64_t* ids, const int32_t* h_seq_len,
                            const int32_t* h_pos0, const int32_t* h_slot, int n_seq, int prompt_phase,
                            dh_bf16* logits_all, dh_bf16* logits_last, void* stream);

int dh_engine_set_cpu_rsqrt_emulation(dh_engine* e, int vec_width, int whole_call);

int dh_engine_decode(dh_engine* e, int64_t* tokens, int tok_ld, int32_t* length, int32_t* done,
                     int n_seq, int n_steps, float temperature, int top_k, int64_t eos_id,
                     uint64_t seed, int first_step, void* stream);

int dh_engine_decode_rows(dh_engine* e, int64_t* tokens, int tok_ld, int32_t* length, int32_t* done,
                          const int32_t* limit, int n_seq, int max_new_tokens, const int32_t* row_seq,
                          const int32_t* row_slot, int n_rows, int n_steps, float temperature, int top_k,
                          int64_t eos_id, uint64_t seed, void* stream);

int dh_engine_read(dh_engine* e, int what, int layer, void* dst, int64_t n_bytes, void* stream);
int dh_engine_set_timing(dh_engine* e, int on);
int dh_engine_get_timing(dh_engine* e, int which, double* h_ms, int64_t* h_launches);

#ifdef __cplusplus
}
#endif
#endif
```

Baseline: 796.7 utterances/s.

## Add warp-specialized ring GEMM for decode QKV and proj with fused LoRA epilogue

Adds a new producer/consumer ring-buffer GEMM kernel in which loader waves stream weight and activation tiles into LDS slots, synchronised through LDS flags, while compute waves consume them. It writes bf16 QKV or proj+residual output directly with LoRA applied, replacing the split-K fp32 partial-sum path for decode when the row count is large enough. A bf16-row variant of the fused attention decode kernel and a norm-only kernel are added so the rest of the layer can take the direct outputs. This is meant to remove the fp32 partial buffer traffic and the reduction work, at the cost of spin-wait synchronisation risk and a different rounding order.

Result: no change. 804.4 utterances/s, median of 6 (+1.0%).

```diff
diff --git a/dualhyp_amd/_lib.py b/dualhyp_amd/_lib.py
--- a/dualhyp_amd/_lib.py
+++ b/dualhyp_amd/_lib.py
@@ -45,6 +45,10 @@
     "dh_linear_partial_pairs_bf16": (I, [P, P, P, P, I, I, I, I, I, P]),
     "dh_finish_norm_bf16": (I, [P, I, I, I, I, I, P, F, P, P, P, P, F, P, P]),
     "dh_attn_decode_fused_bf16": (I, [P, I, I, I, I, I, P, F, I, I, P, P, P, P, P, P, P, I, I, I, I, P]),
+    "dh_attn_decode_fused_rows_bf16": (I, [P, I, I, P, P, P, P, P, P, P, I, I, I, I, P]),
+    "dh_norm_only_bf16": (I, [P, P, P, I, I, F, P, P]),
+    "dh_linear_ring_qkv_bf16": (I, [P, P, P, P, F, I, I, P, I, I, I, I, P]),
+    "dh_linear_ring_proj_bf16": (I, [P, P, P, P, F, P, P, I, I, I, I, P]),
     "dh_attn_prefill_bf16": (I, [P, P, P, P, P, P, P, P, P, I, I, I, I, I, I, P]),
     "dh_dropout_bf16": (I, [P, P, P, I64, F, C.c_uint64, C.c_uint32, P, P]),
     "dh_swiglu_fwd_bf16": (I, [P, P, P, I64, P]),
diff --git a/dualhyp_amd/csrc/decode_fused.hip b/dualhyp_amd/csrc/decode_fused.hip
--- a/dualhyp_amd/csrc/decode_fused.hip
+++ b/dualhyp_amd/csrc/decode_fused.hip
@@ -5,13 +5,13 @@
 constexpr int DCOLS = 16;
 constexpr int MAXP = 16;
 
-template <int HS, int PMAX, int NW>
+template <int HS, int PMAX, int NW, bool ROWBF = false>
 __global__ __launch_bounds__(NW * 64, NW == 16 ? 1 : (NW == 6 ? 3 : (HS == 64 ? 4 : 2))) void attn_decode_fused_kernel(
     const float* __restrict__ qkv32, int n_part, int pairs, int n_seq, int ldq, int qkv_dim,
     const bf16_t* __restrict__ lora_b, float lora_scale, int split0, int split1,
     const bf16_t* __restrict__ cos, const bf16_t* __restrict__ sin, const int32_t* __restrict__ seq_slot,
     const int32_t* __restrict__ kv_len, bf16_t* __restrict__ k_cache, bf16_t* __restrict__ vT_cache,
-    bf16_t* __restrict__ y, int n_head, int n_groups, int s_max, float scale) {
+    bf16_t* __restrict__ y, int n_head, int n_groups, int s_max, float scale, const bf16_t* __restrict__ qkvb) {
     constexpr int KS = HS / 16, DT = HS / 32, HALF = HS / 2;
     extern __shared__ __attribute__((aligned(16))) char smem[];
     const int pair = blockIdx.x, seq = pair / n_groups, g = pair % n_groups;
@@ -67,11 +67,12 @@
         }
         return s;
     };
-    if (lora_b != nullptr && tid < 48) sXa[tid] = rbf(psum(qkv_dim + tid));
+    if (!ROWBF && lora_b != nullptr && tid < 48) sXa[tid] = rbf(psum(qkv_dim + tid));
     for (int i = tid; i < 16 * HS; i += NT_) sQ[i] = 0;
     __syncthreads();
 
     auto finish = [&](int c) -> float {
+        if (ROWBF) return bf2f(qkvb[(size_t)seq * qkv_dim + c]);
         float o = rbf(psum(c));
         if (lora_b != nullptr) {
             const int seg = (c >= split0) + (c >= split1);
@@ -346,6 +347,64 @@
     }
 }
 
+template <int MAXC>
+__global__ __launch_bounds__(256) void norm_only_kernel(const bf16_t* __restrict__ x, const bf16_t* __restrict__ w_norm,
+                                                        bf16_t* __restrict__ xn_out, int d, float eps, const uint8_t* __restrict__ row_tail) {
+    __shared__ float sRed[4];
+    const int row = blockIdx.x, tid = threadIdx.x, lane = tid & 63, wave = tid >> 6;
+    float v[MAXC][8];
+    float ss = 0.f;
+#pragma unroll
+    for (int i = 0; i < MAXC; ++i) {
+        const int c0 = (tid + i * 256) * 8;
+        if (c0 < d) {
+            const uint4 xr = *reinterpret_cast<const uint4*>(x + (size_t)row * d + c0);
+            const bf16_t* xp = reinterpret_cast<const bf16_t*>(&xr);
+#pragma unroll
+            for (int e = 0; e < 8; ++e) {
+                v[i][e] = bf2f(xp[e]);
+                ss += rbf(v[i][e] * v[i][e]);
+            }
+        }
+    }
+    ss = wave_sum(ss);
+    if (lane == 0) sRed[wave] = ss;
+    __syncthreads();
+    ss = sRed[0] + sRed[1] + sRed[2] + sRed[3];
+    const float ms = rbf(ss / (float)d);
+    const float t = rbf(ms + eps);
+    const bool tail = row_tail != nullptr && row_tail[row] != 0;
+    const float r = tail ? rbf(1.0f / rbf(sqrtf(t))) : rbf(1.0f / sqrtf(t));
+#pragma unroll
+    for (int i = 0; i < MAXC; ++i) {
+        const int c0 = (tid + i * 256) * 8;
+        if (c0 < d) {
+            const uint4 wu = *reinterpret_cast<const uint4*>(w_norm + c0);
+            const bf16_t* wp = reinterpret_cast<const bf16_t*>(&wu);
+            uint4 o;
+            bf16_t* op = reinterpret_cast<bf16_t*>(&o);
+#pragma unroll
+            for (int e = 0; e < 8; ++e) op[e] = f2bf(bf2f(wp[e]) * rbf(v[i][e] * r));
+            *reinterpret_cast<uint4*>(xn_out + (size_t)row * d + c0) = o;
+        }
+    }
+}
+
+}
+
+extern "C" int dh_norm_only_bf16(const dh_bf16* x, const dh_bf16* w_norm, dh_bf16* xn_out, int rows, int d, float eps,
+                                 const uint8_t* row_tail, void* stream) {
+    DH_CHECK(x && w_norm && xn_out, "dh_norm_only_bf16: null argument");
+    DH_CHECK(d % 8 == 0 && d <= 8192, "dh_norm_only_bf16: unsupported d=%d", d);
+    if (rows <= 0) return 0;
+    hipStream_t s = (hipStream_t)stream;
+#define LAUNCH(MAXC) hipLaunchKernelGGL((norm_only_kernel<MAXC>), dim3(rows), dim3(256), 0, s, x, w_norm, xn_out, d, eps, row_tail)
+    if (d <= 2048) { LAUNCH(1); }
+    else if (d <= 4096) { LAUNCH(2); }
+    else { LAUNCH(4); }
+#undef LAUNCH
+    DH_LAUNCH_CHECK();
+    return 0;
 }
 
 extern "C" int dh_attn_decode_fused_bf16(const float* qkv32, int n_part, int pairs, int n_seq, int qkv_dim, int n_ext,
@@ -366,7 +425,7 @@
 #define ATT_LAUNCH(HSV, PM)                                                                                           \
     hipLaunchKernelGGL((attn_decode_fused_kernel<HSV, PM, attn_fused_waves<HSV>()>), grid, dim3(64 * attn_fused_waves<HSV>()), attn_fused_lds<HSV>(), s, qkv32, n_part, pairs, n_seq,  \
                        qkv_dim + n_ext, qkv_dim, lora_b, lora_scale, split0, split1, cos, sin, seq_slot, kv_len, k_cache,  \
-                       vT_cache, y, n_head, n_groups, s_max, scale)
+                       vT_cache, y, n_head, n_groups, s_max, scale, nullptr)
     if (hs == 64) {
         DH_MAX_LDS_ONCE((attn_decode_fused_kernel<64, 2, attn_fused_waves<64>()>), attn_fused_lds<64>());
         DH_MAX_LDS_ONCE((attn_decode_fused_kernel<64, 8, attn_fused_waves<64>()>), attn_fused_lds<64>());
@@ -394,6 +453,33 @@
     return 0;
 }
 
+extern "C" int dh_attn_decode_fused_rows_bf16(const dh_bf16* qkv, int n_seq, int qkv_dim, const dh_bf16* cos, const dh_bf16* sin,
+                                              const int32_t* seq_slot, const int32_t* kv_len, dh_bf16* k_cache, dh_bf16* vT_cache,
+                                              dh_bf16* y, int n_head, int n_groups, int hs, int s_max, void* stream) {
+    DH_CHECK(qkv && cos && sin && seq_slot && kv_len && k_cache && vT_cache && y, "dh_attn_decode_fused_rows_bf16: null argument");
+    DH_CHECK(n_groups > 0 && n_head % n_groups == 0 && n_head / n_groups <= DCOLS, "dh_attn_decode_fused_rows_bf16: bad head counts");
+    DH_CHECK(hs == 64 || hs == 96 || hs == 128, "dh_attn_decode_fused_rows_bf16: head_size %d unsupported", hs);
+    DH_CHECK(s_max % 64 == 0, "dh_attn_decode_fused_rows_bf16: bad s_max");
+    DH_CHECK(qkv_dim == (n_head + 2 * n_groups) * hs, "dh_attn_decode_fused_rows_bf16: qkv_dim mismatch");
+    if (n_seq <= 0) return 0;
+    const float scale = 1.0f / sqrtf((float)hs);
+    hipStream_t s = (hipStream_t)stream;
+    dim3 grid(n_seq * n_groups);
+#define ATT_ROWS(HSV)                                                                                                              \
+    do {                                                                                                                           \
+        DH_MAX_LDS_ONCE((attn_decode_fused_kernel<HSV, 2, attn_fused_waves<HSV>(), true>), attn_fused_lds<HSV>());                 \
+        hipLaunchKernelGGL((attn_decode_fused_kernel<HSV, 2, attn_fused_waves<HSV>(), true>), grid, dim3(64 * attn_fused_waves<HSV>()), \
+                           attn_fused_lds<HSV>(), s, nullptr, 1, 0, n_seq, qkv_dim, qkv_dim, nullptr, 0.f, 0, 0, cos, sin, seq_slot, \
+                           kv_len, k_cache, vT_cache, y, n_head, n_groups, s_max, scale, qkv);                                     \
+    } while (0)
+    if (hs == 64) ATT_ROWS(64);
+    else if (hs == 96) ATT_ROWS(96);
+    else ATT_ROWS(128);
+#undef ATT_ROWS
+    DH_LAUNCH_CHECK();
+    return 0;
+}
+
 extern "C" int dh_finish_norm_bf16(const float* h32, int n_part, int pairs, int rows, int d, int n_ext, const dh_bf16* lora_b,
                                    float lora_scale, const dh_bf16* x_resid, const dh_bf16* w_norm, dh_bf16* x_out,
                                    dh_bf16* xn_out, float eps, const uint8_t* row_tail, void* stream) {
diff --git a/dualhyp_amd/csrc/engine.hip b/dualhyp_amd/csrc/engine.hip
--- a/dualhyp_amd/csrc/engine.hip
+++ b/dualhyp_amd/csrc/engine.hip
@@ -383,15 +383,33 @@
             return dh_linear_partial_bf16(xin, w, wext, e->part32, n_seq, N, ext, K, ks, s);
         };
         int np, pairs;
-        const int ext1 = W.attn_lora_a ? 48 : 0;
-        if ((rc = partial(e->xn, W.attn_w, W.attn_lora_a, e->qkv_dim, ext1, d, pick_ksplit((e->qkv_dim + ext1) / 16, d / 32), np, pairs))) return rc;
-        if ((rc = dh_attn_decode_fused_bf16(e->part32, np, pairs, n_seq, e->qkv_dim, ext1, W.attn_lora_b, D.lora_scale, d,
-                                            d + e->kv_dim, D.rope_cos, D.rope_sin, seq_slot, kv_len, kc, vtc, e->att, H, G,
-                                            hs, e->s_max, s))) return rc;
-        const int ext2 = W.proj_lora_a ? 16 : 0;
-        if ((rc = partial(e->att, W.proj_w, W.proj_lora_a, d, ext2, d, pick_ksplit((d + ext2) / 16, d / 32), np, pairs))) return rc;
+        const int ext1 = W.attn_lora_a ? 48 : 0, ks1 = pick_ksplit((e->qkv_dim + ext1) / 16, d / 32);
+        const int ext2 = W.proj_lora_a ? 16 : 0, ks2 = pick_ksplit((d + ext2) / 16, d / 32);
+        const int want = dh_ring_wanted(n_seq, d);
+        const bool ring_q = (want & 1) && dh_pairs_ok(n_seq, e->qkv_dim, ext1, d, ks1) && !dh_chain_ok(n_seq, e->qkv_dim, ext1, d, ks1) &&
+                            (W.attn_lora_a == nullptr) == (W.attn_lora_b == nullptr) && dh_ring_ok(n_seq, e->qkv_dim, d, ks1, d, d + e->kv_dim);
+        const bool ring_p = (want & 2) && dh_pairs_ok(n_seq, d, ext2, d, ks2) && !dh_chain_ok(n_seq, d, ext2, d, ks2) &&
+                            (W.proj_lora_a == nullptr) == (W.proj_lora_b == nullptr) && dh_ring_ok(n_seq, d, d, ks2, d, d);
+        if (ring_q) {
+            if ((rc = dh_linear_ring_qkv_bf16(e->xn, W.attn_w, W.attn_lora_a, W.attn_lora_b, D.lora_scale, d, d + e->kv_dim, e->qkv, n_seq,
+                                              e->qkv_dim, d, ks1, s))) return rc;
+            if ((rc = dh_attn_decode_fused_rows_bf16(e->qkv, n_seq, e->qkv_dim, D.rope_cos, D.rope_sin, seq_slot, kv_len, kc, vtc, e->att,
+                                                     H, G, hs, e->s_max, s))) return rc;
+        } else {
+            if ((rc = partial(e->xn, W.attn_w, W.attn_lora_a, e->qkv_dim, ext1, d, ks1, np, pairs))) return rc;
+            if ((rc = dh_attn_decode_fused_bf16(e->part32, np, pairs, n_seq, e->qkv_dim, ext1, W.attn_lora_b, D.lora_scale, d,
+                                                d + e->kv_dim, D.rope_cos, D.rope_sin, seq_slot, kv_len, kc, vtc, e->att, H, G,
+                                                hs, e->s_max, s))) return rc;
+        }
+        if (ring_p) {
+            if ((rc = dh_linear_ring_proj_bf16(e->att, W.proj_w, W.proj_lora_a, W.proj_lora_b, D.lora_scale, e->x, e->x, n_seq, d, d, ks2,
+                                               s))) return rc;
+            if ((rc = dh_norm_only_bf16(e->x, W.norm_2, e->xn, n_seq, d, D.norm_eps, rt, s))) return rc;
+        } else {
+        if ((rc = partial(e->att, W.proj_w, W.proj_lora_a, d, ext2, d, ks2, np, pairs))) return rc;
         if ((rc = dh_finish_norm_bf16(e->part32, np, pairs, n_seq, d, ext2, W.proj_lora_b, D.lora_scale, e->x, W.norm_2, e->x,
                                       e->xn, D.norm_eps, rt, s))) return rc;
+        }
         if ((rc = linear(e, e->xn, W.fc_1, e->act, n_seq, I, d, DH_EPI_SWIGLU, W.fc_2, nullptr, 0, nullptr, 0, 0, nullptr,
                          nullptr, nullptr, s, false))) return rc;
         if ((rc = partial(e->act, W.mlp_proj, nullptr, d, 0, I, pick_ksplit(d / 16, I / 32), np, pairs))) return rc;
diff --git a/dualhyp_amd/csrc/gemm.h b/dualhyp_amd/csrc/gemm.h
--- a/dualhyp_amd/csrc/gemm.h
+++ b/dualhyp_amd/csrc/gemm.h
@@ -54,6 +54,9 @@
                    int kps, hipStream_t s);
 extern int g_dt_min_rows, g_chain_min_rows;
 
+bool dh_ring_ok(int M, int N, int K, int ksplit, int split0, int split1);
+int dh_ring_wanted(int M, int K);
+
 bool dh_linear_is_big(int M, int N, int epilogue);
 
 int dh_linear_256(GemmArgs a, int epilogue, hipStream_t s);
diff --git a/dualhyp_amd/csrc/gemm_ring.hip b/dualhyp_amd/csrc/gemm_ring.hip
--- /dev/null
+++ b/dualhyp_amd/csrc/gemm_ring.hip
@@ -0,0 +1,347 @@
+#include "common.h"
+
+int g_ring = 3;
+int g_ring_min_rows = 640;
+int g_ring_max_k = 2048;
+int g_ring_nt = 0;
+int g_ring_depth = 2;
+int g_ring_cols = 0;
+
+namespace {
+
+constexpr int RM = 128;
+constexpr int BKR = 64;
+constexpr int SPIN_LIMIT = 1 << 20;
+
+__device__ __forceinline__ int swz7r(int row) { return (row >> 1) & 7; }
+
+struct RingArgs {
+    const bf16_t* x;
+    const bf16_t* w;
+    const bf16_t* a;
+    const bf16_t* lora_b;
+    const bf16_t* resid;
+    bf16_t* y;
+    float lora_scale;
+    int M, N, K, seg_kt;
+    int split0, split1;
+    int strips0, strips1;
+    int m_tiles;
+};
+
+template <bool WNT>
+__device__ __forceinline__ void ring_glds(const void* base_uniform, uint32_t lane_off, uint32_t lds) {
+    if (WNT) asm volatile("s_mov_b32 m0, %2\n\ts_nop 0\n\tglobal_load_lds_dwordx4 %0, %1 nt" ::"v"(lane_off), "s"(base_uniform), "s"(lds) : "memory", "m0");
+    else asm volatile("s_mov_b32 m0, %2\n\ts_nop 0\n\tglobal_load_lds_dwordx4 %0, %1" ::"v"(lane_off), "s"(base_uniform), "s"(lds) : "memory", "m0");
+}
+
+__device__ __forceinline__ int flag_load(const int* p) { return __hip_atomic_load(p, __ATOMIC_RELAXED, __HIP_MEMORY_SCOPE_WORKGROUP); }
+__device__ __forceinline__ void flag_store(int* p, int v) { __hip_atomic_store(p, v, __ATOMIC_RELAXED, __HIP_MEMORY_SCOPE_WORKGROUP); }
+
+__device__ __forceinline__ void wait_words(const int* words, int need, int lane, bool& dead) {
+    if (dead) return;
+    int spins = 0;
+    for (;;) {
+        const int v = lane < 4 ? flag_load(words + lane) : need;
+        if (__all(v >= need)) break;
+        if (++spins > SPIN_LIMIT) { dead = true; break; }
+        __builtin_amdgcn_s_sleep(1);
+    }
+    asm volatile("" ::: "memory");
+}
+
+template <int NT, bool LORA, bool WNT, int AHEAD>
+__global__ __launch_bounds__(512) void gemm_ring_kernel(RingArgs a) {
+    constexpr int NSLOT = AHEAD + 3;
+    constexpr int WT = NT + (LORA ? 1 : 0);
+    constexpr int WBYTES = WT * 16 * 128;
+    constexpr int SLOT = WBYTES + RM * 128;
+    constexpr int PIECES = SLOT / 1024;
+    constexpr int PER = (PIECES + 3) / 4;
+    extern __shared__ __attribute__((aligned(16))) char smem[];
+    int* full = reinterpret_cast<int*>(smem + NSLOT * SLOT);
+    int* free_ = full + NSLOT * 4;
+    int* bready = free_ + NSLOT * 4;
+    bf16_t* sB = reinterpret_cast<bf16_t*>(smem + NSLOT * SLOT + 2 * NSLOT * 16 + 16);
+    const int tid = threadIdx.x, lane = tid & 63, wave = __builtin_amdgcn_readfirstlane(tid >> 6);
+    if (tid < 2 * NSLOT * 4 + 4) full[tid] = 0;
+    __syncthreads();
+
+    int tile;
+    {
+        const int nwg = gridDim.x, bid = blockIdx.x, xcd = bid & 7, q = nwg >> 3, r = nwg & 7;
+        tile = (xcd < r ? xcd * (q + 1) : r * (q + 1) + (xcd - r) * q) + (bid >> 3);
+    }
+    const int tm = tile % a.m_tiles, tn = tile / a.m_tiles;
+    const int m0 = tm * RM;
+    int seg, n0, n_end;
+    if (tn < a.strips0) { seg = 0; n0 = tn * (NT * 16); n_end = a.split0; }
+    else if (tn < a.strips1) { seg = 1; n0 = a.split0 + (tn - a.strips0) * (NT * 16); n_end = a.split1; }
+    else { seg = 2; n0 = a.split1 + (tn - a.strips1) * (NT * 16); n_end = a.N; }
+    const int nk = a.K / BKR;
+
+    if (wave < 4) {
+        uint32_t off[PER];
+        uint32_t dst[PER];
+#pragma unroll
+        for (int j = 0; j < PER; ++j) {
+            int p = wave * PER + j;
+            p = p < PIECES ? p : PIECES - 1;
+            const int row = (p < WT * 2 ? p : p - WT * 2) * 8 + (lane >> 3);
+            const int chunk = (lane & 7) ^ swz7r(row);
+            if (p < WT * 2) {
+                if (LORA && p >= NT * 2) {
+                    off[j] = (uint32_t)(((size_t)(seg * 16 + row - NT * 16) * a.K + chunk * 8) * 2);
+                } else {
+                    int n = n0 + row;
+                    n = n < n_end ? n : n_end - 1;
+                    off[j] = (uint32_t)(((size_t)n * a.K + chunk * 8) * 2);
+                }
+            } else {
+                int m = m0 + row;
+                m = m < a.M ? m : a.M - 1;
+                off[j] = (uint32_t)(((size_t)m * a.K + chunk * 8) * 2);
+            }
+            dst[j] = (uint32_t)(uintptr_t)(__attribute__((address_space(3))) char*)smem + p * 1024;
+        }
+        bool dead = false;
+        int slot = 0, round = 0;
+        int pslot = 0, pround = 0;
+        auto publish = [&]() __attribute__((always_inline)) {
+            if (lane == 0) flag_store(full + pslot * 4 + wave, pround + 1);
+            if (++pslot == NSLOT) { pslot = 0; ++pround; }
+        };
+        for (int kt = 0; kt < nk; ++kt) {
+            if (round > 0) wait_words(free_ + slot * 4, round, lane, dead);
+#pragma unroll
+            for (int j = 0; j < PER; ++j) {
+                const int p = wave * PER + j < PIECES ? wave * PER + j : PIECES - 1;
+                const bf16_t* base = p < NT * 2 ? a.w : (p < WT * 2 ? a.a : a.x);
+                if (WNT && p < WT * 2) ring_glds<true>(base, off[j] + kt * (BKR * 2), dst[j] + slot * SLOT);
+                else ring_glds<false>(base, off[j] + kt * (BKR * 2), dst[j] + slot * SLOT);
+            }
+            if (kt >= AHEAD) {
+                asm volatile("s_waitcnt vmcnt(%0)" ::"n"(AHEAD * PER) : "memory");
+                publish();
+            }
+            if (++slot == NSLOT) { slot = 0; ++round; }
+        }
+        if (AHEAD >= 3 && nk >= 3) {
+            asm volatile("s_waitcnt vmcnt(%0)" ::"n"(2 * PER) : "memory");
+            publish();
+        }
+        if (nk >= 2) {
+            asm volatile("s_waitcnt vmcnt(%0)" ::"n"(PER) : "memory");
+            publish();
+        }
+        asm volatile("s_waitcnt vmcnt(0)" ::: "memory");
+        publish();
+        return;
+    }
+
+    const int cw = wave - 4;
+    const int frow = lane & 15, kg = lane >> 4;
+    const int sw = swz7r(frow);
+    f32x4 cur[WT][2], pairacc[WT][2], tot[WT][2];
+#pragma unroll
+    for (int i = 0; i < WT; ++i)
+#pragma unroll
+        for (int j = 0; j < 2; ++j) {
+            cur[i][j] = f32x4{0.f, 0.f, 0.f, 0.f};
+            pairacc[i][j] = f32x4{0.f, 0.f, 0.f, 0.f};
+            tot[i][j] = f32x4{0.f, 0.f, 0.f, 0.f};
+        }
+    bool dead = false;
+    if (LORA && cw == 0) {
+        for (int idx = lane; idx < NT * 32; idx += 64) {
+            int n = n0 + (idx >> 1);
+            n = n < n_end ? n : n_end - 1;
+            reinterpret_cast<uint4*>(sB)[idx] = reinterpret_cast<const uint4*>(a.lora_b + (size_t)n * 16)[idx & 1];
+        }
+        asm volatile("s_waitcnt lgkmcnt(0)" ::: "memory");
+        if (lane == 0) flag_store(bready, 1);
+    }
+    {
+        int slot = 0, round = 0, in_seg = 0, seg_idx = 0;
+        bf16x8 fa0[WT], fb0[2], fa1[WT], fb1[2];
+        auto read_half = [&](int sl, int ks, bf16x8 (&fa)[WT], bf16x8 (&fb)[2]) __attribute__((always_inline)) {
+            const char* sW = smem + sl * SLOT;
+            const char* sX = sW + WBYTES + cw * 32 * 128;
+            const int co = ((ks * 4 + kg) ^ sw) << 4;
+#pragma unroll
+            for (int i = 0; i < WT; ++i) fa[i] = *reinterpret_cast<const bf16x8*>(sW + (i * 16 + frow) * 128 + co);
+#pragma unroll
+            for (int j = 0; j < 2; ++j) fb[j] = *reinterpret_cast<const bf16x8*>(sX + (j * 16 + frow) * 128 + co);
+        };
+        auto mma = [&](const bf16x8 (&fa)[WT], const bf16x8 (&fb)[2]) __attribute__((always_inline)) {
+#pragma unroll
+            for (int i = 0; i < WT; ++i)
+#pragma unroll
+                for (int j = 0; j < 2; ++j) cur[i][j] = __builtin_amdgcn_mfma_f32_16x16x32_bf16(fa[i], fb[j], cur[i][j], 0, 0, 0);
+        };
+        wait_words(full, 1, lane, dead);
+        read_half(0, 0, fa0, fb0);
+        for (int kt = 0; kt < nk; ++kt) {
+            read_half(slot, 1, fa1, fb1);
+            mma(fa0, fb0);
+            asm volatile("s_waitcnt lgkmcnt(0)" ::: "memory");
+            if (lane == 0) flag_store(free_ + slot * 4 + cw, round + 1);
+            if (kt + 1 < nk) {
+                const int ns = slot + 1 == NSLOT ? 0 : slot + 1, nr = slot + 1 == NSLOT ? round + 1 : round;
+                wait_words(full + ns * 4, nr + 1, lane, dead);
+                read_half(ns, 0, fa0, fb0);
+            }
+            mma(fa1, fb1);
+            if (++in_seg == a.seg_kt || kt + 1 == nk) {
+                in_seg = 0;
+                const bool second = seg_idx & 1, last = kt + 1 == nk;
+                if (second) {
+#pragma unroll
+                    for (int i = 0; i < WT; ++i)
+#pragma unroll
+                        for (int j = 0; j < 2; ++j) tot[i][j] += pairacc[i][j] + cur[i][j];
+                } else if (last) {
+#pragma unroll
+                    for (int i = 0; i < WT; ++i)
+#pragma unroll
+                        for (int j = 0; j < 2; ++j) tot[i][j] += cur[i][j];
+                } else {
+#pragma unroll
+                    for (int i = 0; i < WT; ++i)
+#pragma unroll
+                        for (int j = 0; j < 2; ++j) pairacc[i][j] = cur[i][j];
+                }
+#pragma unroll
+                for (int i = 0; i < WT; ++i)
+#pragma unroll
+                    for (int j = 0; j < 2; ++j) cur[i][j] = f32x4{0.f, 0.f, 0.f, 0.f};
+                ++seg_idx;
+            }
+            if (++slot == NSLOT) { slot = 0; ++round; }
+        }
+    }
+
+    if (LORA && !dead) {
+        int spins = 0;
+        while (flag_load(bready) == 0 && ++spins <= SPIN_LIMIT) __builtin_amdgcn_s_sleep(1);
+        asm volatile("" ::: "memory");
+    }
+    uint2 rv[2][NT];
+    if (a.resid != nullptr) {
+#pragma unroll
+        for (int j = 0; j < 2; ++j)
+#pragma unroll
+            for (int i = 0; i < NT; ++i) {
+                const int m = m0 + cw * 32 + j * 16 + frow, n = n0 + i * 16 + kg * 4;
+                rv[j][i] = m < a.M && n < n_end ? *reinterpret_cast<const uint2*>(a.resid + (size_t)m * a.N + n) : make_uint2(0, 0);
+            }
+    }
+#pragma unroll
+    for (int j = 0; j < 2; ++j) {
+        const int m = m0 + cw * 32 + j * 16 + frow;
+        float xa[16];
+        if (LORA) {
+#pragma unroll
+            for (int q = 0; q < 4; ++q)
+#pragma unroll
+                for (int r = 0; r < 4; ++r) xa[q * 4 + r] = __shfl(rbf(tot[WT - 1][j][r]), q * 16 + frow, 64);
+        }
+        if (m >= a.M) continue;
+#pragma unroll
+        for (int i = 0; i < NT; ++i) {
+            const int n = n0 + i * 16 + kg * 4;
+            if (n >= n_end) continue;
+            float o[4];
+#pragma unroll
+            for (int r = 0; r < 4; ++r) {
+                o[r] = rbf(tot[i][j][r]);
+                if (LORA) {
+                    const uint4* b4 = reinterpret_cast<const uint4*>(sB + (i * 16 + kg * 4 + r) * 16);
+                    float l = 0.f;
+#pragma unroll
+                    for (int h = 0; h < 2; ++h) {
+                        const uint4 bv = b4[h];
+                        const bf16_t* bp = reinterpret_cast<const bf16_t*>(&bv);
+#pragma unroll
+                        for (int k = 0; k < 8; ++k) l = fmaf(xa[h * 8 + k], bf2f(bp[k]), l);
+                    }
+                    o[r] = rbf(o[r] + rbf(rbf(l) * a.lora_scale));
+                }
+            }
+            if (a.resid != nullptr) {
+                const bf16_t* rp = reinterpret_cast<const bf16_t*>(&rv[j][i]);
+#pragma unroll
+                for (int r = 0; r < 4; ++r) o[r] = bf2f(rp[r]) + o[r];
+            }
+            *reinterpret_cast<uint2*>(a.y + (size_t)m * a.N + n) = make_uint2(pack2bf(o[0], o[1]), pack2bf(o[2], o[3]));
+        }
+    }
+}
+
+template <int NT, bool LORA, bool WNT, int AHEAD>
+int launch_ring_t(const RingArgs& a, int wgs, hipStream_t s) {
+    constexpr int NSLOT = AHEAD + 3;
+    constexpr int lds = NSLOT * ((NT + (LORA ? 1 : 0)) * 2048 + RM * 128) + 2 * NSLOT * 4 * (int)sizeof(int) + 16 + 4 * 16 * 32;
+    DH_MAX_LDS_ONCE((gemm_ring_kernel<NT, LORA, WNT, AHEAD>), lds);
+    hipLaunchKernelGGL((gemm_ring_kernel<NT, LORA, WNT, AHEAD>), dim3(wgs), dim3(512), lds, s, a);
+    DH_LAUNCH_CHECK();
+    return 0;
+}
+
+int strips_of(int n, int nc) { return cdiv(n, nc); }
+
+int launch_ring(RingArgs a, hipStream_t s) {
+    const bool lora = a.a != nullptr;
+    a.m_tiles = cdiv(a.M, RM);
+    int best_nt = 0;
+    long best_cost = 0;
+    for (int nt = 3; nt <= 4; ++nt) {
+        if (g_ring_cols && g_ring_cols != nt * 16) continue;
+        const int nc = nt * 16;
+        const int strips = strips_of(a.split0, nc) + strips_of(a.split1 - a.split0, nc) + strips_of(a.N - a.split1, nc);
+        const long cost = (long)cdiv(strips * a.m_tiles, 256) * ((nt + (lora ? 1 : 0)) * 2048 + RM * 128);
+        if (!best_nt || cost < best_cost) { best_nt = nt; best_cost = cost; }
+    }
+    const int nc = best_nt * 16;
+    a.strips0 = strips_of(a.split0, nc);
+    a.strips1 = a.strips0 + strips_of(a.split1 - a.split0, nc);
+    const int wgs = (a.strips1 + strips_of(a.N - a.split1, nc)) * a.m_tiles;
+#define RING(NTV, LV)                                                                \
+    return g_ring_depth == 3 ? (g_ring_nt ? launch_ring_t<NTV, LV, true, 3>(a, wgs, s) : launch_ring_t<NTV, LV, false, 3>(a, wgs, s)) \
+                             : (g_ring_nt ? launch_ring_t<NTV, LV, true, 2>(a, wgs, s) : launch_ring_t<NTV, LV, false, 2>(a, wgs, s))
+    if (best_nt == 3) { if (lora) { RING(3, true); } else { RING(3, false); } }
+    if (lora) { RING(4, true); } else { RING(4, false); }
+#undef RING
+}
+
+}
+
+bool dh_ring_ok(int M, int N, int K, int ksplit, int split0, int split1) {
+    const int nks = K / 32, kps = ksplit > 0 ? (nks + ksplit - 1) / ksplit : 0;
+    return M >= 1 && K % 64 == 0 && K >= 64 && (kps == 8 || kps == 16) && ksplit * kps == nks && N % 16 == 0 && split0 % 16 == 0 &&
+           split1 % 16 == 0 && 0 < split0 && split0 <= split1 && split1 <= N && (size_t)N * K * 2 < (1ull << 32) &&
+           (size_t)M * K * 2 < (1ull << 32);
+}
+int dh_ring_wanted(int M, int K) {
+    return M >= g_ring_min_rows && K <= g_ring_max_k ? g_ring : 0;
+}
+
+extern "C" int dh_linear_ring_qkv_bf16(const dh_bf16* x, const dh_bf16* w, const dh_bf16* lora_a, const dh_bf16* lora_b, float lora_scale,
+                                       int split0, int split1, dh_bf16* qkv, int M, int N, int K, int ksplit, void* stream) {
+    DH_CHECK(x && w && qkv && (lora_a == nullptr) == (lora_b == nullptr), "dh_linear_ring_qkv_bf16: bad argument");
+    DH_CHECK(dh_ring_ok(M, N, K, ksplit, split0, split1),
+             "dh_linear_ring_qkv_bf16: unsupported shape M=%d N=%d K=%d ksplit=%d splits %d/%d (K %% 64 == 0, whole K-slices of 8 or 16 k-steps, "
+             "segments on 16 columns)", M, N, K, ksplit, split0, split1);
+    RingArgs a{x, w, lora_a, lora_b, nullptr, qkv, lora_scale, M, N, K, (K / 32 / ksplit) / 2, split0, split1, 0, 0, 0};
+    return launch_ring(a, (hipStream_t)stream);
+}
+
+extern "C" int dh_linear_ring_proj_bf16(const dh_bf16* x, const dh_bf16* w, const dh_bf16* lora_a, const dh_bf16* lora_b, float lora_scale,
+                                        const dh_bf16* x_resid, dh_bf16* x_out, int M, int N, int K, int ksplit, void* stream) {
+    DH_CHECK(x && w && x_resid && x_out && (lora_a == nullptr) == (lora_b == nullptr), "dh_linear_ring_proj_bf16: bad argument");
+    DH_CHECK(dh_ring_ok(M, N, K, ksplit, N, N),
+             "dh_linear_ring_proj_bf16: unsupported shape M=%d N=%d K=%d ksplit=%d (K %% 64 == 0, whole K-slices of 8 or 16 k-steps, N %% 16 == 0)",
+             M, N, K, ksplit);
+    RingArgs a{x, w, lora_a, lora_b, x_resid, x_out, lora_scale, M, N, K, (K / 32 / ksplit) / 2, N, N, 0, 0, 0};
+    return launch_ring(a, (hipStream_t)stream);
+}
diff --git a/dualhyp_amd/csrc/gemm_skinny.hip b/dualhyp_amd/csrc/gemm_skinny.hip
--- a/dualhyp_amd/csrc/gemm_skinny.hip
+++ b/dualhyp_amd/csrc/gemm_skinny.hip
@@ -667,6 +667,18 @@
     if (key == 25) { extern int g_w4_persist_qkv; g_w4_persist_qkv = value != 0; return 0; }
     if (key == 26) { extern int g_tn_mfma; g_tn_mfma = value != 0; return 0; }
     if (key == 31) { g_skinny_n = value != 0; return 0; }
+    if (key == 32 && value >= 0) {
+        extern int g_ring, g_ring_nt, g_ring_cols, g_ring_max_k, g_ring_depth, g_ring_min_rows;
+        if (value <= 1) g_ring = value ? 3 : 0;
+        else if (value == 4 || value == 5) g_ring = value == 4 ? 2 : 1;
+        else if (value <= 3) g_ring_nt = value == 2;
+        else if (value == 6 || value == 7) g_ring_depth = value - 4;
+        else if (value == 16 || value == 48 || value == 64) g_ring_cols = value == 16 ? 0 : value;
+        else if (value >= 256 && value < 1024) g_ring_min_rows = value;
+        else if (value >= 1024) g_ring_max_k = value;
+        else { dh_set_error("dh_set_tuning: key 32 takes 0 .. 7, 16, 48, 64, a row bound 256..1023 or a K bound >= 1024"); return 1; }
+        return 0;
+    }
     if (key == 30) { extern int g_w4_persist_lora; g_w4_persist_lora = value != 0; return 0; }
     if (key == 29) { extern int g_attn_bwd_dkdv_img; g_attn_bwd_dkdv_img = value != 0; return 0; }
     if (key == 28) { extern int g_tail_split; g_tail_split = value != 0; return 0; }
diff --git a/dualhyp_amd/ops.py b/dualhyp_amd/ops.py
--- a/dualhyp_amd/ops.py
+++ b/dualhyp_amd/ops.py
@@ -379,6 +379,47 @@
     return y
 
 
+def attn_decode_fused_rows(qkv: torch.Tensor, cos: torch.Tensor, sin: torch.Tensor, seq_slot: torch.Tensor, kv_len: torch.Tensor,
+                           k_cache: torch.Tensor, vT_cache: torch.Tensor, n_head: int) -> torch.Tensor:
+    k = _Keep()
+    qkv = _dev(qkv, name="qkv")
+    n_seq, qkv_dim = qkv.shape
+    n_groups, s_max, hs = k_cache.size(1), k_cache.size(2), k_cache.size(3)
+    y = torch.empty((n_seq, n_head * hs), dtype=torch.bfloat16, device=qkv.device)
+    i32 = torch.int32
+    check(_lib.load().dh_attn_decode_fused_rows_bf16(_p(qkv), n_seq, qkv_dim, k(cos), k(sin), k(seq_slot, i32), k(kv_len, i32),
+                                                     _p(k_cache), _p(vT_cache), _p(y), n_head, n_groups, hs, s_max, _stream()))
+    return y
+
+
+def norm_only(x: torch.Tensor, w_norm: torch.Tensor, eps: float, row_tail: Optional[torch.Tensor] = None) -> torch.Tensor:
+    k = _Keep()
+    x = _dev(x, name="x")
+    xn = torch.empty_like(x)
+    check(_lib.load().dh_norm_only_bf16(_p(x), k(w_norm), _p(xn), x.size(0), x.size(1), float(eps), _p(row_tail), _stream()))
+    return xn
+
+
+def linear_ring_qkv(x: torch.Tensor, w: torch.Tensor, lora_a: Optional[torch.Tensor], lora_b: Optional[torch.Tensor],
+                    lora_scale: float, splits: Tuple[int, int], ksplit: int) -> torch.Tensor:
+    x, w = _dev(x, name="x"), _dev(w, name="w")
+    M, K = x.shape
+    y = torch.empty((M, w.size(0)), dtype=torch.bfloat16, device=x.device)
+    check(_lib.load().dh_linear_ring_qkv_bf16(_p(x), _p(w), _p(lora_a), _p(lora_b), float(lora_scale), splits[0], splits[1], _p(y),
+                                              M, w.size(0), K, ksplit, _stream()))
+    return y
+
+
+def linear_ring_proj(x: torch.Tensor, w: torch.Tensor, lora_a: Optional[torch.Tensor], lora_b: Optional[torch.Tensor],
+                     lora_scale: float, x_resid: torch.Tensor, ksplit: int, out: Optional[torch.Tensor] = None) -> torch.Tensor:
+    x, w, x_resid = _dev(x, name="x"), _dev(w, name="w"), _dev(x_resid, name="x_resid")
+    M, K = x.shape
+    y = torch.empty_like(x_resid) if out is None else out
+    check(_lib.load().dh_linear_ring_proj_bf16(_p(x), _p(w), _p(lora_a), _p(lora_b), float(lora_scale), _p(x_resid), _p(y), M,
+                                               w.size(0), K, ksplit, _stream()))
+    return y
+
+
 def kcache_to_plain(kc: torch.Tensor) -> torch.Tensor:
     B, G, S, hs = kc.shape
     v = kc.reshape(B, G, S // 32, hs // 16, 2, 32, 8)
diff --git a/include/dualhyp_hip.h b/include/dualhyp_hip.h
--- a/include/dualhyp_hip.h
+++ b/include/dualhyp_hip.h
@@ -66,6 +66,15 @@
                         const dh_bf16* lora_b, float lora_scale, const dh_bf16* x_resid,
                         const dh_bf16* w_norm, dh_bf16* x_out, dh_bf16* xn_out, float eps,
                         const uint8_t* row_tail, void* stream);
+int dh_norm_only_bf16(const dh_bf16* x, const dh_bf16* w_norm, dh_bf16* xn_out, int rows, int d, float eps,
+                      const uint8_t* row_tail, void* stream);
+
+int dh_linear_ring_qkv_bf16(const dh_bf16* x, const dh_bf16* w, const dh_bf16* lora_a, const dh_bf16* lora_b,
+                            float lora_scale, int split0, int split1, dh_bf16* qkv, int M, int N, int K, int ksplit,
+                            void* stream);
+int dh_linear_ring_proj_bf16(const dh_bf16* x, const dh_bf16* w, const dh_bf16* lora_a, const dh_bf16* lora_b,
+                             float lora_scale, const dh_bf16* x_resid, dh_bf16* x_out, int M, int N, int K, int ksplit,
+                             void* stream);
 
 
 int dh_attn_prefill_bf16(const dh_bf16* q, const dh_bf16* k_cache, const dh_bf16* vT_cache,
@@ -84,6 +93,10 @@
                               const int32_t* kv_len, dh_bf16* k_cache, dh_bf16* vT_cache,
                               dh_bf16* y, int n_head, int n_groups, int hs, int s_max,
                               void* stream);
+int dh_attn_decode_fused_rows_bf16(const dh_bf16* qkv, int n_seq, int qkv_dim, const dh_bf16* cos, const dh_bf16* sin,
+                                   const int32_t* seq_slot, const int32_t* kv_len, dh_bf16* k_cache,
+                                   dh_bf16* vT_cache, dh_bf16* y, int n_head, int n_groups, int hs, int s_max,
+                                   void* stream);
 
 
 int dh_dropout_bf16(const dh_bf16* x, dh_bf16* y, dh_bf16* mask, int64_t n, float p, uint64_t seed, uint32_t call_id,
```
